# adelacvg/diff-vits

Hardware: AMD Instinct MI355X
Metric: mel_frames_per_sec_50step_dpmsolver (higher is better)
Workload: dtype bf16x3 (bf16 MFMA operands split hi+lo, 3 products, fp32 accumulate / fp32 activations); 1 GPU; B=8/GPU, C=80, T=1024, L=256, 50-step DPM-Solver++(2M) multistep, UNet1DConditionModel (128, 256, 384, 512), seeded random-init weights; global_batch=8, concurrent_sub_batches_per_gpu=1, rccl_world_size=1, parallelism=dp1 (batch-sharded, RCCL broadcast of conditioning + all-gather of mels)

## Files before the change

diff-vits_amd/csrc/engine.hip:

```cpp
#include "../../include/dvits_hip.h"
#include "dv_common.h"

#include <algorithm>
#include <atomic>
#include <cmath>
#include <cstdarg>
#include <cstdio>
#include <cstdlib>
#include <cstring>
#include <functional>
#include <map>
#include <memory>
#include <set>
#include <string>
#include <type_traits>
#include <vector>

static thread_local char g_err[1024] = "";
int dv_fail(int code, const char* fmt, ...) {
  va_list ap;
  va_start(ap, fmt);
  vsnprintf(g_err, sizeof(g_err), fmt, ap);
  va_end(ap);
  return code;
// ... 185 lines not shown
  u->slab = nullptr; u->slab_bytes = 0;
  u->step_ops.clear(); u->cond_ops.clear(); u->probes.clear(); u->step_meta.clear(); u->gemm_store.clear();
  u->pops.clear(); u->step_pop.clear(); u->pops_dev = nullptr; u->psync = nullptr; u->persist_on = false; u->p_begin = u->p_end = 0;
  u->prepared = false; u->cond_set = false; u->flops = 0;
  u->cond_segs.clear(); u->cond_segs_dev = nullptr; u->cond_chunks = 0; u->cond_sig = 0; u->row_cond.clear(); u->cond_gemms.clear();
}

extern "C" int dv_unet_create(const dv_unet_cfg* cfg, dv_unet** out) {
  if (!cfg || !out) return dv_fail(DV_ERR_INVALID, "dv_unet_create: null argument");
  if (cfg->n_levels < 2 || cfg->n_levels > 6) return dv_fail(DV_ERR_INVALID, "n_levels must be 2..6");
  for (int i = 0; i < cfg->n_levels; ++i)
    if (cfg->block_out_channels[i] % 32 != 0 || cfg->block_out_channels[i] <= 0)
      return dv_fail(DV_ERR_INVALID, "block_out_channels[%d]=%d must be a positive multiple of 32", i,
                     cfg->block_out_channels[i]);
  if (cfg->cross_attention_dim % 32 != 0) return dv_fail(DV_ERR_INVALID, "cross_attention_dim must be a multiple of 32");
  if (cfg->num_heads <= 0 || cfg->norm_num_groups <= 0 || cfg->norm_num_groups > 64)
    return dv_fail(DV_ERR_INVALID, "bad num_heads / norm_num_groups");
  for (int i = 0; i < cfg->n_levels; ++i) {
    int c = cfg->block_out_channels[i];
    if (c % cfg->num_heads != 0 || (c / cfg->num_heads) % 4 != 0 || c / cfg->num_heads > 64)
      return dv_fail(DV_ERR_INVALID, "head dim %d/%d must be a multiple of 4 and <= 64", c, cfg->num_heads);
    if (c % cfg->norm_num_groups != 0 || (c / cfg->norm_num_groups) % 4 != 0)
      return dv_fail(DV_ERR_INVALID, "channels per GroupNorm group must be a multiple of 4");
  }
  if (cfg->cross_attention_dim % cfg->add_embed_heads != 0 || cfg->cross_attention_dim / cfg->add_embed_heads > 8)
    return dv_fail(DV_ERR_INVALID, "add_embed_heads must divide cross_attention_dim with <= 8 dims per head");
  dv_unet* u = new dv_unet();
  u->cfg = *cfg;
  *out = u;
  return DV_OK;
}

extern "C" void dv_unet_destroy(dv_unet* u) {
  if (!u) return;
  (void)hipDeviceSynchronize();
  unet_release_prepared(u);
  if (u->gnx_status) (void)hipHostFree(u->gnx_status);
  for (auto& kv : u->w)
    if (kv.second.p) (void)hipFree(kv.second.p);
  delete u;
}

extern "C" int dv_unet_set_weight(dv_unet* u, const char* name, const void* dev_ptr, const int64_t* shape, int32_t ndim) {
  if (!u || !name || !dev_ptr || !shape || ndim < 1 || ndim > 4) return dv_fail(DV_ERR_INVALID, "dv_unet_set_weight: bad argument");
  size_t n = 1;
  std::vector<int64_t> sh(shape, shape + ndim);
  for (auto s : sh) n *= (size_t)s;
  RawW& r = u->w[name];
  if (r.numel != n) {
    if (r.p) (void)hipFree(r.p);
    r.p = nullptr;
    HIPCHK(hipMalloc((void**)&r.p, n * sizeof(float)));
  }
  r.shape = sh;
  r.numel = n;
  HIPCHK(hipMemcpy(r.p, dev_ptr, n * sizeof(float), hipMemcpyDeviceToDevice));
  u->weights_dirty = true;
  return DV_OK;
}

static bool autotune_on() {
  const char* e = getenv("DVITS_GEMM_AUTOTUNE");
  return e && (e[0] == '1' || e[0] == '2');
}

static int autotune_gemms(dv_unet* u, int precision) {
  u->tuned_gemms = u->tuned_changed = 0;
  if (!autotune_on() || u->gemm_store.empty()) return DV_OK;
  HIPCHK(hipDeviceSynchronize());
  hipStream_t st = nullptr;
  hipEvent_t e0, e1;
  HIPCHK(hipEventCreate(&e0)); HIPCHK(hipEventCreate(&e1));
  const size_t flush_bytes = 48u << 20;
  void* flush = nullptr;
  HIPCHK(hipMalloc(&flush, flush_bytes));
  auto time_one = [&](const GemmParams& t, float& best) -> bool {
    if (launch_gemm(t, precision, st) != hipSuccess) { (void)hipGetLastError(); return false; }
    best = 1e30f;
    for (int r = 0; r < 3; ++r) {
      if (hipMemsetAsync(flush, r, flush_bytes, st) != hipSuccess) return false;
      if (hipEventRecord(e0, st) != hipSuccess) return false;
      if (launch_gemm(t, precision, st) != hipSuccess) return false;
      if (hipEventRecord(e1, st) != hipSuccess || hipEventSynchronize(e1) != hipSuccess) return false;
      float ms = 0;
      if (hipEventElapsedTime(&ms, e0, e1) != hipSuccess) return false;
      best = ms < best ? ms : best;
    }
    return true;
  };
  for (auto& up : u->gemm_store) {
    GemmParams* gp = up.get();
    if (!gp->out && !gp->out_hi) continue;
    int cands[12];
    const int n = gemm_candidates(*gp, cands, 12);
    float best = 1e30f;
    int best_tile = gp->force_tile, best_split = gp->sk_split;
    const int heur_split = gp->sk_split;
    {
      float ms;
      if (time_one(*gp, ms)) best = ms * 0.97f;
    }
    for (int c = 0; c < n; ++c)
      for (int sp = 0; sp < (gp->sk_buf ? 2 : 1); ++sp) {
        GemmParams t = *gp;
        t.force_tile = cands[c];
        t.sk_split = sp ? (heur_split > 2 ? heur_split : 2) : 0;
        float ms;
        if (time_one(t, ms) && ms < best) { best = ms; best_tile = cands[c]; best_split = t.sk_split; }
      }
    if (best_tile != gp->force_tile || best_split != heur_split) u->tuned_changed++;
    gp->force_tile = best_tile;
    gp->sk_split = best_split;
    u->tuned_gemms++;
  }
  if (const char* e = getenv("DVITS_GEMM_AUTOTUNE"))
    if (e[0] == '2') fprintf(stderr, "[dvits] GEMM tuner: %d of %d GEMMs moved off the heuristic tile\n", u->tuned_changed, u->tuned_gemms);
  (void)hipFree(flush);
  (void)hipEventDestroy(e0); (void)hipEventDestroy(e1);
  HIPCHK(hipDeviceSynchronize());
  return DV_OK;
}

struct Builder {
  dv_unet* u;
  Arena arena;
  bool dry;
  int B, T, L, prec;
  std::string err;
  hipStream_t pack_stream = nullptr;
  bool fuse_ln = [] { const char* e = getenv("DVITS_FUSE_LN"); return !(e && e[0] == '0'); }();
  bool merge_ff = [] { const char* e = getenv("DVITS_MERGE_FF"); return !(e && e[0] == '0'); }();

  const RawW* raw(const std::string& name) {
    auto it = u->w.find(name);
    if (it == u->w.end()) { if (err.empty()) err = "missing weight: " + name; return nullptr; }
    return &it->second;
  }
  const float* W(const std::string& name) { const RawW* r = raw(name); return r ? r->p : nullptr; }
  bool has(const std::string& name) { return u->w.count(name) != 0; }

  float* alloc(size_t floats) {
    size_t off = arena.alloc(floats * sizeof(float));
    return dry ? reinterpret_cast<float*>(0x1000 + off) : reinterpret_cast<float*>(u->slab + off);
  }
  void release(const void* p) {
    if (u->keep_intermediates) return;
    size_t off = dry ? (reinterpret_cast<size_t>(p) - 0x1000) : (size_t)(reinterpret_cast<const char*>(p) - u->slab);
    arena.release(off);
  }
  const char* cur_kind = "misc";
  const GemmParams* cur_gp = nullptr;
  double cur_flops = 0;
  std::string cur_desc;
  void emit(std::vector<OpFn>& ops, OpFn f, const PersistOp* pop = nullptr) {
    if (dry) return;
    ops.push_back(std::move(f));
    if (&ops == &u->step_ops) {
      u->step_meta.push_back({cur_kind, cur_flops, cur_desc, cur_gp});
      if (pop) { u->step_pop.push_back((int)u->pops.size()); u->pops.push_back(*pop); }
      else u->step_pop.push_back(-1);
    }
    cur_kind = "misc"; cur_flops = 0; cur_desc.clear(); cur_gp = nullptr;
  }
  void emit_launch(std::vector<OpFn>& ops, const char* kind, double flops, std::string desc, OpFn f, const PersistOp* pop = nullptr) {
    cur_kind = kind; cur_flops = flops; cur_desc = std::move(desc);
    if (!dry) u->flops += flops;
    emit(ops, std::move(f), pop);
  }
  static std::string strf(const char* fmt, ...) {
    char buf[128];
    va_list ap;
    va_start(ap, fmt);
    vsnprintf(buf, sizeof(buf), fmt, ap);
    va_end(ap);
    return buf;
  }
  bool persist_gemm(const GemmParams& gin, PersistOp& po) {
    if (prec != DV_PREC_BF16X3 || gin.epi == EPI_STORE_NCT || !gin.w_lo) return false;
    bool k64 = true;
    for (int s2 = 0; s2 < gin.nseg; ++s2) k64 = k64 && gin.seg[s2].c0 % 64 == 0 && gin.seg[s2].c1 % 64 == 0;
    int cfg, bm, bk;
    if (gin.epi == EPI_GEGLU) { if (!k64) return false; cfg = 1; bm = 128; bk = 64; }
    else {
      const bool big = gin.T_out % 128 == 0 && (gin.T_out / 128) * ((gin.N + 127) / 128) >= 24;
      if (big || !k64) { cfg = 0; bm = 128; bk = 32; } else { cfg = 2; bm = 64; bk = 64; }
    }
    if (gin.T_out % bm != 0 || gin.M != B * gin.T_out) return false;
    if (gin.T_out < 1 || (unsigned long long)(gin.M > 0 ? gin.M : 1) * (unsigned long long)gin.T_out >= (1ull << 32)) return false;
    po = PersistOp{};
    po.type = POP_GEMM; po.cfg = cfg; po.g = gin;
    po.g.tout_magic = gemm_tout_magic(gin.T_out);
    if (po.g.Tv_out <= 0) po.g.Tv_out = po.g.T_out;
    if (po.g.Tv_in <= 0) po.g.Tv_in = po.g.T_in;
    for (int s2 = 0; s2 < gin.nseg; ++s2) po.g.seg[s2].nkt = gin.seg[s2].taps * (gin.seg[s2].c0 + gin.seg[s2].c1) / bk;
    return true;
  }
  void probe(const std::string& name, const float* p, int T_, int C_) {
    if (!dry && u->keep_intermediates) u->probes.push_back(Probe{name, const_cast<float*>(p), T_, C_, T_ > 1 ? pitch(T_) : T_});
  }
  void probe_rows(const std::string& name, const float* p, int T_, int C_) {
    if (!dry && u->keep_intermediates) u->probes.push_back(Probe{name, const_cast<float*>(p), T_, C_, T_});
  }

  struct Piece { std::string w; int kind, C, taps, c_pad, k_off, n_off; std::string kscale; int geglu; };
  struct BiasPiece { std::string bias, bias2, foldW, foldBeta; int N, C, n_off, geglu; };

  const PackedW* pack(const std::string& key, int N, int Kp, const std::vector<Piece>& pieces,
                      const std::vector<BiasPiece>& biases) {
    if (dry) { static PackedW dummy; return &dummy; }
    auto it = u->packed.find(key);
    if (it != u->packed.end()) return &it->second;
    PackedW pw;
    pw.N = N; pw.Kp = Kp; pw.N_pad = rup(N, 128);
    const size_t elems = (size_t)pw.N_pad * Kp;
    if (hipMalloc((void**)&pw.hi, elems * 2) != hipSuccess) { err = "hipMalloc(packed weights) failed"; return nullptr; }
    u->owned_w.push_back(pw.hi);
    (void)hipMemsetAsync(pw.hi, 0, elems * 2, pack_stream);
    if (prec == DV_PREC_BF16X3) {
      if (hipMalloc((void**)&pw.lo, elems * 2) != hipSuccess) { err = "hipMalloc(packed weights) failed"; return nullptr; }
      u->owned_w.push_back(pw.lo);
      (void)hipMemsetAsync(pw.lo, 0, elems * 2, pack_stream);
    }
    for (const Piece& pc : pieces) {
      const RawW* r = raw(pc.w);
      if (!r) return nullptr;
      PackSpec s{};
      s.src = r->p; s.N = (int)r->shape[0]; s.kind = pc.kind; s.C = pc.C; s.taps = pc.taps; s.c_pad = pc.c_pad;
      s.k_off = pc.k_off; s.n_off = pc.n_off; s.geglu = pc.geglu;
      s.kscale = pc.kscale.empty() ? nullptr : W(pc.kscale);
      if ((size_t)s.N * s.C * s.taps != r->numel) { err = "weight shape mismatch: " + pc.w; return nullptr; }
      if (launch_pack_weight(s, pw.hi, pw.lo, Kp, pack_stream) != hipSuccess) { err = "pack_weight launch failed"; return nullptr; }
      if (s.kscale) {
        if (!pw.u) {
          if (hipMalloc((void**)&pw.u, (size_t)pw.N_pad * 4) != hipSuccess) { err = "hipMalloc(u) failed"; return nullptr; }
          u->owned_w.push_back(pw.u);
          (void)hipMemsetAsync(pw.u, 0, (size_t)pw.N_pad * 4, pack_stream);
        }
        if (launch_fold_bias(r->p, nullptr, s.kscale, pw.u, s.N, s.C, pc.n_off, pc.geglu, pack_stream) != hipSuccess) {
          err = "fold(u) launch failed"; return nullptr;
        }
      }
    }
    if (!biases.empty()) {
      if (hipMalloc((void**)&pw.bias, (size_t)pw.N_pad * 4) != hipSuccess) { err = "hipMalloc(bias) failed"; return nullptr; }
      u->owned_w.push_back(pw.bias);
      (void)hipMemsetAsync(pw.bias, 0, (size_t)pw.N_pad * 4, pack_stream);
      for (const BiasPiece& bp : biases) {
        const float* b1 = bp.bias.empty() ? nullptr : W(bp.bias);
        const float* fw = bp.foldW.empty() ? nullptr : W(bp.foldW);
        const float* fb = bp.foldBeta.empty() ? nullptr : W(bp.foldBeta);
        if (launch_fold_bias(fw, b1, fb, pw.bias, bp.N, bp.C, bp.n_off, bp.geglu, pack_stream) != hipSuccess) {
          err = "fold_bias launch failed"; return nullptr;
        }
        if (!bp.bias2.empty()) {
          static const float one_one[8] = {1.f, 1.f, 0, 0, 0, 0, 0, 0};
          float* dcoef = nullptr;
          if (hipMalloc((void**)&dcoef, sizeof(one_one)) != hipSuccess) { err = "hipMalloc failed"; return nullptr; }
          u->owned_w.push_back(dcoef);
          (void)hipMemcpyAsync(dcoef, one_one, sizeof(one_one), hipMemcpyHostToDevice, pack_stream);
          (void)launch_lincomb(pw.bias + bp.n_off, pw.bias + bp.n_off, W(bp.bias2), nullptr, nullptr, nullptr, dcoef, bp.N,
                               pack_stream);
        }
      }
    }
    u->packed[key] = pw;
    return &u->packed[key];
  }

  struct Planes { bf16_t* hi = nullptr; bf16_t* lo = nullptr; };
  Planes alloc_planes(size_t elems) {
    Planes pl;
    pl.hi = reinterpret_cast<bf16_t*>(alloc((elems + 1) / 2));
    if (prec == DV_PREC_BF16X3) pl.lo = reinterpret_cast<bf16_t*>(alloc((elems + 1) / 2));
    return pl;
  }
  void release(const Planes& pl) { if (pl.hi) release((const void*)pl.hi); if (pl.lo) release((const void*)pl.lo); }
  void alloc_stat(Act& a, bool want16 = false) {
    if (a.Tp % 32 != 0) {
      if (B == 1) a.stat = alloc((size_t)((a.Tp + 31) / 32) * a.C * 2);
      return;
    }
    if (want16 || stat16_everywhere()) a.stat16 = alloc((size_t)(B * a.Tp / 32) * (a.C / 16) * 2);
    else a.stat = alloc((size_t)(B * a.Tp / 32) * a.C * 2);
  }
  bool pad_on = [] { const char* e = getenv("DVITS_PAD_T"); return !(e && e[0] == '0'); }();
  int pitch(int Tl) const { return (pad_on && Tl % 32 != 0 && stat16_everywhere()) ? rup(Tl, 32) : Tl; }
  bool stat16_everywhere() const {
    const char* e16 = getenv("DVITS_STAT16");
    if ((e16 && e16[0] == '0') || arena.exact) return false;
    const int G = u->cfg.norm_num_groups;
    for (int i = 0; i < u->cfg.n_levels; ++i)
      if (u->cfg.block_out_channels[i] % G != 0 || (u->cfg.block_out_channels[i] / G) % 16 != 0) return false;
    return true;
  }
  void stat_out(GemmParams& g, const Act& a) { g.stats = a.stat; g.stats16 = a.stat16; }
  bool chain_on = [] { const char* e = getenv("DVITS_CHAIN"); return !(e && e[0] == '0'); }();
  int chain_min_rows = [] { const char* e = getenv("DVITS_CHAIN_MIN_ROWS"); return e ? atoi(e) : 128; }();
  bool chain_ok(int Tn, int C) const {
    const int G = u->cfg.norm_num_groups;
    return chain_on && fuse_ln && !arena.exact && prec == DV_PREC_BF16X3 && (C == 128 || C == 256 || C == 384) && Tn % 32 == 0 &&
           B * Tn >= chain_min_rows &&
           G > 0 && G <= 64 && (G & (G - 1)) == 0 && C % G == 0 && (C / G) % 16 == 0 && (Tn / 32) * (C / 16) <= (C / 128) * 2048;
  }
  bool frag(const PackedW* cw) {
    if (dry) return true;
    PackedW* w = const_cast<PackedW*>(cw);
    if (w->fhi) return true;
    const size_t elems = (size_t)w->N_pad * w->Kp;
    if (!w->lo || hipMalloc((void**)&w->fhi, elems * 2) != hipSuccess || hipMalloc((void**)&w->flo, elems * 2) != hipSuccess) {
      err = "hipMalloc(fragment-major weights) failed"; return false;
    }
    u->owned_w.push_back(w->fhi); u->owned_w.push_back(w->flo);
    if (launch_relayout_frag(w->hi, w->fhi, w->N_pad, w->Kp, pack_stream) != hipSuccess ||
        launch_relayout_frag(w->lo, w->flo, w->N_pad, w->Kp, pack_stream) != hipSuccess) { err = "relayout launch failed"; return false; }
    return true;
  }
  static double chain_flops(const ChainParams& cp) { return 2.0 * (double)cp.M * cp.C * cp.C * (1 + cp.passes); }
  void chain(std::vector<OpFn>& ops, const ChainParams& cp, const char* what, double extra_flops = 0.0) {
    const int pr = prec;
    emit_launch(ops, "chain", chain_flops(cp) + extra_flops, strf("%s M=%d C=%d N2=%d", what, cp.M, cp.C, cp.passes * cp.C),
                [cp, pr](hipStream_t st) { return launch_chain2(cp, pr, st); });
  }
  bool sk_fused = [] { const char* e = getenv("DVITS_SPLITK_FUSED"); return !(e && e[0] == '0'); }();
  bool gnx_on = [] { const char* e = getenv("DVITS_GNX"); return !(e && e[0] == '0') && !getenv("HSA_CU_MASK") && !getenv("ROC_GLOBAL_CU_MASK"); }();
  size_t gnx_used = 0;
  int gnx_spin = [] { const char* e = getenv("DVITS_GNX_SPIN"); const int v = e ? atoi(e) : 0; return v != 0 ? v : (1 << 18); }();
  int n_cu = [] { int d = 0, n = 0; if (hipGetDevice(&d) != hipSuccess || hipDeviceGetAttribute(&n, hipDeviceAttributeMultiprocessorCount, d) != hipSuccess) n = 0;
                  const char* e = getenv("DVITS_CU_BUDGET"); const int b = e ? atoi(e) : 0; return b > 0 && b < n ? b : n; }();
  bool gnx_cat_on = [] { const char* e = getenv("DVITS_GNX_CONCAT"); return !(e && e[0] == '0'); }();
  bool handover_ok() const { return gnx_on && u->exclusive && !arena.exact && n_cu > 0; }
  struct Handover { unsigned long long* flags; unsigned* status; };
  Handover handover(size_t n) {
    Handover h{dry ? reinterpret_cast<unsigned long long*>(0x1000) : u->gnx_pool + gnx_used,
               dry ? reinterpret_cast<unsigned*>(0x1000) : u->gnx_status};
    gnx_used += (n + 1) & ~(size_t)1;
    if (!dry) { u->gnx_words = gnx_used; u->gnx_ops++; }
    return h;
  }
  bool gnx_setup(GemmParams& g, const std::string& pre, float eps, const float* tscale, const float* tshift, int ld_t, bool silu,
                 Planes* y, const Act* skip = nullptr, Planes* sk_y = nullptr, Planes* sk_raw = nullptr) {
    if (!handover_ok() || autotune_on() || !g.stats16) return false;
    if (skip && (!gnx_cat_on || !skip->p || !skip->stat16 || skip->Tp != g.T_out || tscale)) return false;
    GemmParams t = g;
    t.B = B;
    t.gnx = GnxParams{};
    t.gnx.groups = u->cfg.norm_num_groups;
    t.gnx.sk_c = skip ? skip->C : 0;
    int k_pad = 0;
    for (int s2 = 0; s2 < t.nseg; ++s2) k_pad += t.seg[s2].taps * (t.seg[s2].c0 + t.seg[s2].c1);
    t.c3_route = conv3_route(t);
    t.sk_split = t.c3_route ? gemm_conv3_split(t, n_cu) : gemm_splitk_plan(t.M, t.N, k_pad, t.epi);
    if (t.sk_split >= 2) {
      if (!sk_fused || ((t.M + 31) / 32) * ((t.N + 31) / 32) > 4096) return false;
      t.sk_buf = reinterpret_cast<float*>(0x1000); t.sk_ticket = reinterpret_cast<unsigned*>(0x1000);
    }
    const int nw = gemm_gnx_plan(t, n_cu);
    if (nw <= 0 || gnx_used + (size_t)nw > dv_unet::GNX_POOL) return false;
    g.gnx = t.gnx;
    gnx_fill(g.gnx, nw, g.M, g.N, pre, eps, tscale, tshift, ld_t, silu, y, skip, sk_y, sk_raw);
    return true;
  }
  void gnx_fill(GnxParams& gx, int nw, int M, int N, const std::string& pre, float eps, const float* tscale, const float* tshift, int ld_t,
                bool silu, Planes* y, const Act* skip, Planes* sk_y, Planes* sk_raw) {
    gx.gamma = W(pre + ".weight"); gx.beta = W(pre + ".bias"); gx.eps = eps;
    gx.tscale = tscale; gx.tshift = tshift; gx.ld_t = ld_t; gx.silu = silu ? 1 : 0;
    gx.spin_max = gnx_spin;
    const Handover h = handover((size_t)nw);
    gx.xchg = h.flags; gx.status = h.status;
    *y = alloc_planes((size_t)M * N);
    gx.y_hi = y->hi; gx.y_lo = y->lo;
    if (skip) {
      gx.sk_x = skip->p; gx.sk_stat16 = skip->stat16;
      *sk_y = alloc_planes((size_t)M * skip->C);
      gx.sk_y_hi = sk_y->hi; gx.sk_y_lo = sk_y->lo;
      if (sk_raw) { *sk_raw = alloc_planes((size_t)M * skip->C); gx.sk_raw_hi = sk_raw->hi; gx.sk_raw_lo = sk_raw->lo; }
    }
  }

  struct NextNorm { std::string pre; bool raw = false; bool set = false; Act skip; float eps = 0.f; bool silu = true; } next_norm;
  void announce_norm(const std::string& pre, bool raw_planes, const Act& skip = Act{}) {
    next_norm.pre = pre; next_norm.raw = raw_planes; next_norm.skip = skip; next_norm.set = true;
    next_norm.eps = u->cfg.norm_eps; next_norm.silu = true;
  }
  void announce_transformer_norm(const std::string& tp, int Tp, int C) {
    if (chain_ok(Tp, C)) return;
    announce_norm(tp + "norm", false);
    next_norm.eps = 1e-6f; next_norm.silu = false;
  }
  bool gnx_offer(GemmParams& g, const NextNorm& nn, Planes* y, Planes* sy, Planes* sr) {
    return gnx_setup(g, nn.pre, nn.eps, nullptr, nullptr, 0, nn.silu, y, nn.skip.C > 0 ? &nn.skip : nullptr, sy, nn.raw ? sr : nullptr);
  }
  static int ff_gnx_plan(const ChainFFParams& fp, int n_cu) { return chain_ff_gnx_plan(fp, n_cu); }
  static int ff_gnx_plan(const FFSplitParams& fp, int n_cu) { return ff_split_gnx_plan(fp, n_cu); }
  template <class FF> bool gnx_offer(FF& fp, const NextNorm& nn, Planes* y, Planes* sy, Planes* sr) {
    const bool cat = nn.skip.C > 0;
    if (!handover_ok() || !gnx_ff_on || !fp.stats16) return false;
    if (cat && (!gnx_cat_on || !nn.skip.p || !nn.skip.stat16 || nn.skip.Tp != fp.T)) return false;
    fp.gnx = GnxParams{};
    fp.gnx.groups = u->cfg.norm_num_groups;
    fp.gnx.sk_c = cat ? nn.skip.C : 0;
    const int nw = ff_gnx_plan(fp, n_cu);
    if (nw <= 0 || gnx_used + (size_t)nw > dv_unet::GNX_POOL) { fp.gnx = GnxParams{}; return false; }
    gnx_fill(fp.gnx, nw, fp.M, fp.C, nn.pre, nn.eps, nullptr, nullptr, 0, nn.silu, y, cat ? &nn.skip : nullptr, sy, nn.raw ? sr : nullptr);
    return true;
  }
  template <class P> void offer_next(P& prod, Act& out) {
    if (!next_norm.set) return;
    const NextNorm nn = next_norm;
    next_norm.set = false;
    Planes y, sy, sr;
    if (!gnx_offer(prod, nn, &y, &sy, &sr)) return;
    const bool cat = nn.skip.C > 0;
    out.n_hi = y.hi; out.n_lo = y.lo; out.n_pre = nn.pre;
    if (cat) { out.sn_hi = sy.hi; out.sn_lo = sy.lo; out.sr_hi = sr.hi; out.sr_lo = sr.lo; }
    const bool fp32_unread = cat && nn.raw && !u->keep_intermediates;
    if (nn.raw && !prod.out_hi) out_planes(prod, out);
    if (fp32_unread && cat_drop_fp32) prod.out = nullptr;
  }
  template <class P> void out_planes(P& prod, Act& out) {
    Planes pl = alloc_planes((size_t)prod.M * out.C);
    out.pl_hi = pl.hi; out.pl_lo = pl.lo; prod.out_hi = pl.hi; prod.out_lo = pl.lo;
  }
  bool ff_split_on = [] { const char* e = getenv("DVITS_FF_SPLIT"); return !(e && e[0] == '0'); }();
  bool chain_ff_on = [] { const char* e = getenv("DVITS_CHAIN_FF"); return !(e && e[0] == '0'); }();
  bool chain_split_on = [] { const char* e = getenv("DVITS_CHAIN_SPLIT"); return !(e && e[0] == '0'); }();
  bool chain_xsplit_on = [] { const char* e = getenv("DVITS_CHAIN_XSPLIT"); return !(e && e[0] == '0'); }();
  bool qkv_split_on = [] { const char* e = getenv("DVITS_QKV_SPLIT"); return !(e && e[0] == '0'); }();
  int qkv_split_min_wg = [] { const char* e = getenv("DVITS_QKV_SPLIT_MIN_WG"); return e ? atoi(e) : 96; }();
  int qkv_split_min_c = [] { const char* e = getenv("DVITS_QKV_SPLIT_MIN_C"); return e ? atoi(e) : 256; }();
  bool qkv_xa_on = [] { const char* e = getenv("DVITS_QKV_XA"); return !(e && e[0] == '0'); }();
  int qkv_xa_min_c = [] { const char* e = getenv("DVITS_QKV_XA_MIN_C"); return e ? atoi(e) : 256; }();
  int ff_split_min_wg = [] { const char* e = getenv("DVITS_FF_SPLIT_MIN_WG"); return e ? atoi(e) : 96; }();
  bool gnx_ff_on = [] { const char* e = getenv("DVITS_GNX_FF"); return !(e && e[0] == '0'); }();
  bool cat_drop_fp32 = [] { const char* e = getenv("DVITS_GNX_CONCAT_KEEP_FP32"); return !(e && e[0] == '1'); }();

  int conv3_min_tiles = [] { const char* e = getenv("DVITS_CONV3_MIN_TILES"); return e ? atoi(e) : 64; }();
  int conv3_route(const GemmParams& g) const {
    if (arena.exact || autotune_on() || prec != DV_PREC_BF16X3) return 0;
    GemmParams t = g;
    t.B = B;
    if (gemm_conv3_up_ok(t)) {
      const int tu = gemm_conv3_row_tiles(t, 128) * (t.N / 64);
      return tu >= (conv3_min_tiles < 64 ? conv3_min_tiles : 96) ? 2 : 0;
    }
    if (!gemm_conv3_shape_ok(t)) return 0;
    return gemm_conv3_row_tiles(t, 64) * (t.N / 64) >= conv3_min_tiles ? 1 : 0;
  }
  bool conv3_takes(const GemmParams& g) const { return conv3_route(g) != 0; }
  void gemm(std::vector<OpFn>& ops, GemmParams g, const PackedW* pw, int k_real) {
    g.w_hi = pw->hi; g.w_lo = pw->lo; g.Kp = pw->Kp; g.N_pad = pw->N_pad;
    if (!g.bias) g.bias = pw->bias;
    g.B = B;
    g.zero_page = u->zero_page;
    const int p = prec;
    const int route = conv3_route(g);
    const bool c3 = route != 0 && (dry || g.Kp == gemm_conv3_k(g)) && frag(pw);
    g.c3_route = c3 ? route : 0;
    if (c3) { g.wf_hi = dry ? reinterpret_cast<const bf16_t*>(0x1000) : pw->fhi; g.wf_lo = dry ? reinterpret_cast<const bf16_t*>(0x1000) : pw->flo; }
    cur_kind = "gemm"; cur_flops = 2.0 * (double)g.M * (double)g.N * (double)k_real;
    {
      char buf[128];
      snprintf(buf, sizeof(buf), "M=%d N=%d K=%d taps=%d nseg=%d epi=%d stride=%d up=%d%s%s%s", g.M, g.N, k_real, g.seg[0].taps,
               g.nseg, g.epi, g.stride, g.up_mode, (g.stats || g.stats16) ? " +stats" : "", c3 ? " resident" : "",
               g.gnx.xchg ? " +gnx" : "");
      cur_desc = buf;
    }
    u->flops += dry ? 0.0 : cur_flops;
    int k_pad = 0;
    for (int s2 = 0; s2 < g.nseg; ++s2) k_pad += g.seg[s2].taps * (g.seg[s2].c0 + g.seg[s2].c1);
    g.sk_split = arena.exact ? 0 : (c3 ? gemm_conv3_split(g, n_cu) : gemm_splitk_plan(g.M, g.N, k_pad, g.epi));
    const bool offer = !arena.exact && autotune_on() && gemm_splitk_plan(64, 64, 1 << 20, EPI_STORE) != 0 && k_pad >= 768 && (g.epi == EPI_STORE || g.epi == EPI_RESIDUAL) &&
                       ((g.M + 63) / 64) * ((g.N + 63) / 64) <= 256;
    if (g.sk_split >= 2 || offer) {
      g.sk_buf = alloc((c3 && g.sk_split == 2 ? gemm_conv3_split_bytes(g) : gemm_splitk_bytes(g.M, g.N, g.sk_split > 2 ? g.sk_split : 2)) / sizeof(float));
      g.sk_ticket = (sk_fused && ((g.M + 31) / 32) * ((g.N + 31) / 32) <= 4096) ? u->sk_tickets : nullptr;
    }
    PersistOp po;
    const bool pok = !dry && persist_gemm(g, po);
    if (dry) emit(ops, OpFn{}, nullptr);
    else {
      u->gemm_store.emplace_back(new GemmParams(g));
      const GemmParams* gp = u->gemm_store.back().get();
      cur_gp = gp;
      if (&ops == &u->cond_ops) u->cond_gemms.push_back(gp);
      dv_unet* uu = u;
      emit(ops, [gp, p, uu](hipStream_t st) {
        if (!uu->io.tp_base || !gp->gnx.xchg || !gp->gnx.tscale) return launch_gemm(*gp, p, st);
        GemmParams g2 = *gp;
        g2.gnx.tscale = uu->io.tp_base + (gp->gnx.tscale - uu->temb.tproj_arena);
        g2.gnx.tshift = uu->io.tp_base + (gp->gnx.tshift - uu->temb.tproj_arena);
        return launch_gemm(g2, p, st);
      }, pok ? &po : nullptr);
    }
    if (g.sk_buf) release((const void*)g.sk_buf);
  }

  static GemmSeg seg(Planes a0, int c0, Planes a1, int c1, int taps, int pad) {
    GemmSeg s{};
    s.a0_hi = a0.hi; s.a0_lo = a0.lo; s.a1_hi = a1.hi; s.a1_lo = a1.lo;
    s.c0 = c0; s.c1 = c1; s.taps = taps; s.pad = pad;
    return s;
  }

  Planes norm_apply(std::vector<OpFn>& ops, Act a0, Act a1, const std::string& pre, float eps, const float* tscale,
                    const float* tshift, int ld_t, bool silu, Planes* raw_out) {
    const int G = u->cfg.norm_num_groups, C = a0.C + a1.C, Tn = a0.T, Tp = a0.Tp;
    GnApplyParams gp{};
    gp.a0 = a0.p; gp.a1 = a1.p; gp.c0 = a0.C; gp.c1 = a1.C;
    gp.gamma = W(pre + ".weight"); gp.beta = W(pre + ".bias"); gp.eps = eps; gp.groups = G;
    gp.tscale = tscale; gp.tshift = tshift; gp.ld_t = ld_t; gp.silu = silu ? 1 : 0;
    gp.B = B; gp.T = Tp; gp.Tv = Tn;
    float* sc = nullptr; float* sh = nullptr;
    const bool fast16 = a0.stat16 && (a1.C == 0 || a1.stat16) && ((a0.C + a1.C) / G) % 16 == 0 && a0.C % 16 == 0;
    const bool fast = fast16 || (a0.stat && (a1.C == 0 || a1.stat));
    if (fast16) { gp.st16_0 = a0.stat16; gp.st16_1 = a1.stat16; }
    else if (fast) { gp.slab0 = a0.stat; gp.slab1 = a1.stat; }
    else {
      const int nchunk = std::max(1, std::min(64, (Tn + 63) / 64));
      double* part = reinterpret_cast<double*>(alloc((size_t)B * nchunk * G * 2 * 2));
      sc = alloc((size_t)B * C); sh = alloc((size_t)B * C);
      const int Bn = B;
      const float* gamma = gp.gamma; const float* beta = gp.beta;
      cur_kind = "gn_partial";
      emit(ops, [=](hipStream_t st) { return launch_gn_partial(a0.p, a0.C, a1.p, a1.C, part, Bn, Tn, G, nchunk, st); });
      cur_kind = "gn_finalize";
      dv_unet* uu = u;
      emit(ops, [=](hipStream_t st) {
        const float* ts = tscale; const float* tb = tshift;
        if (uu->io.tp_base && ts) {
          ts = uu->io.tp_base + (tscale - uu->temb.tproj_arena);
          tb = uu->io.tp_base + (tshift - uu->temb.tproj_arena);
        }
        return launch_gn_finalize(part, nchunk, gamma, beta, ts, tb, ld_t, sc, sh, nullptr, nullptr, Bn, Tn, C, G, eps, st);
      });
      release(part);
      gp.scale_in = sc; gp.shift_in = sh;
    }
    Planes out = alloc_planes((size_t)B * Tp * C);
    gp.out_hi = out.hi; gp.out_lo = out.lo;
    if (raw_out) { *raw_out = alloc_planes((size_t)B * Tp * C); gp.raw_hi = raw_out->hi; gp.raw_lo = raw_out->lo; }
    cur_kind = "gn_apply";
    {
      char buf[96];
      snprintf(buf, sizeof(buf), "T=%d C=%d%s%s", Tn, C, fast16 ? " blockstats" : (fast ? " slab" : " table"), raw_out ? " +raw" : "");
      cur_desc = buf;
    }
    PersistOp po{};
    if (fast) {
      po.type = POP_GN; po.gn = gp;
      po.gn_chunks = std::max(1, std::min(Tp / 4, 64 / G));
      po.gn_rpb = (Tp + po.gn_chunks - 1) / po.gn_chunks;
      po.gn_chunks = (Tp + po.gn_rpb - 1) / po.gn_rpb;
    }
    {
      dv_unet* uu = u;
      emit(ops, [gp, uu](hipStream_t st) {
        if (!uu->io.tp_base || !gp.tscale) return launch_gn_apply(gp, st);
        GnApplyParams g2 = gp;
        g2.tscale = uu->io.tp_base + (gp.tscale - uu->temb.tproj_arena);
        g2.tshift = uu->io.tp_base + (gp.tshift - uu->temb.tproj_arena);
        return launch_gn_apply(g2, st);
      }, (fast && !fast16) ? &po : nullptr);
    }
    if (sc) { release(sc); release(sh); }
    return out;
  }

  Planes ln_apply(std::vector<OpFn>& ops, const float* x, int M, int C) {
    Planes out = alloc_planes((size_t)M * C);
    cur_kind = "ln_apply";
    emit(ops, [=](hipStream_t st) { return launch_ln_apply(x, out.hi, out.lo, M, C, 1e-5f, st); });
    return out;
  }

  Planes split(std::vector<OpFn>& ops, const float* x, size_t n) {
    Planes out = alloc_planes(n);
    cur_kind = "split";
    PersistOp po{};
    po.type = POP_SPLIT; po.sp_in = x; po.sp_hi = out.hi; po.sp_lo = out.lo; po.n4_per_item = (int64_t)(n / 4 / (size_t)B);
    emit(ops, [=](hipStream_t st) { return launch_split(x, out.hi, out.lo, (int64_t)n, st); }, (n % (4 * (size_t)B) == 0) ? &po : nullptr);
    return out;
  }

  GemmParams gp_base(int Tn, int M, int N) {
    GemmParams g{};
    g.nseg = 1; g.T_out = g.T_in = pitch(Tn); g.Tv_out = g.Tv_in = g.T_virt = Tn; g.stride = 1; g.up_mode = UP_NONE;
    g.M = M; g.N = N; g.epi = EPI_STORE; g.ldo = N; g.ldres = N;
    return g;
  }
  GemmParams gp_rows(int rows, int M, int N) {
    GemmParams g = gp_base(rows, M, N);
    g.T_out = g.T_in = rows;
    return g;
  }

  std::map<std::string, int> tproj_off;
  int tproj_total = 0;
  float* tproj = nullptr;

  Act resnet(std::vector<OpFn>& ops, const std::string& p, Act x0, Act x1, int cout, bool want_planes = false,
             bool stat16_out = false) {
    const int cin = x0.C + x1.C, Tn = x0.T, Tp = x0.Tp, M = B * Tp;
    const float eps = u->cfg.norm_eps;
    const bool shortcut = has(p + "conv_shortcut.weight");
    const PackedW* w1 = pack(p + "conv1", cout, 3 * cin, {{p + "conv1.weight", 1, cin, 3, cin, 0, 0, "", 0}},
                             {{p + "conv1.bias", "", "", "", cout, 0, 0, 0}});
    if (!w1) return Act{};
    Act h{};
    h.p = alloc((size_t)M * cout); h.C = cout; h.T = Tn; h.Tp = Tp; alloc_stat(h);
    Planes raw, raw1;
    bool raw_made = false;
    const int toff = tproj_off[p];
    Planes n2x;
    bool gnx1 = false;
    {
      GemmParams g = gp_base(Tn, M, cout);
      g.out = h.p; stat_out(g, h);
      {
        Planes n1, n1b;
        if (x0.n_hi && x0.n_pre == p + "norm1" && (!shortcut || x0.pl_hi) && (x1.C == 0 || (x0.sn_hi && (!shortcut || x0.sr_hi)))) {
          n1.hi = x0.n_hi; n1.lo = x0.n_lo;
          if (shortcut) { raw.hi = x0.pl_hi; raw.lo = x0.pl_lo; }
          if (x1.C) {
            n1b.hi = x0.sn_hi; n1b.lo = x0.sn_lo;
            if (shortcut) { raw1.hi = x0.sr_hi; raw1.lo = x0.sr_lo; }
          }
          g.seg[0] = x1.C ? seg(n1, x0.C, n1b, x1.C, 3, 1) : seg(n1, cin, Planes{}, 0, 3, 1);
        } else {
          if (x0.n_hi) { Planes stale; stale.hi = x0.n_hi; stale.lo = x0.n_lo; release(stale); }
          if (x0.sn_hi) { Planes stale; stale.hi = x0.sn_hi; stale.lo = x0.sn_lo; release(stale); }
          if (x0.sr_hi) { Planes stale; stale.hi = x0.sr_hi; stale.lo = x0.sr_lo; release(stale); }
          n1 = norm_apply(ops, x0, x1, p + "norm1", eps, nullptr, nullptr, 0, true, shortcut ? &raw : nullptr);
          g.seg[0] = seg(n1, cin, Planes{}, 0, 3, 1);
        }
        raw_made = shortcut;
        gnx1 = gnx_setup(g, p + "norm2", eps, tproj + toff, tproj + toff + cout, tproj_total, true, &n2x);
        if (gnx1 && !u->keep_intermediates) g.out = nullptr;
        gemm(ops, g, w1, 3 * cin);
        release(n1);
        if (n1b.hi) release(n1b);
      }
    }
    probe(p + "conv1", h.p, Tn, cout);

    const int K2 = 3 * cout + (shortcut ? cin : 0);
    std::vector<Piece> pcs = {{p + "conv2.weight", 1, cout, 3, cout, 0, 0, "", 0}};
    std::vector<BiasPiece> bps = {{p + "conv2.bias", shortcut ? p + "conv_shortcut.bias" : "", "", "", cout, 0, 0, 0}};
    if (shortcut) pcs.push_back({p + "conv_shortcut.weight", 1, cin, 1, cin, 3 * cout, 0, "", 0});
    const PackedW* w2 = pack(p + "conv2", cout, K2, pcs, bps);
    if (!w2) return Act{};
    Act out{};
    out.p = alloc((size_t)M * cout); out.C = cout; out.T = Tn; out.Tp = Tp; alloc_stat(out, stat16_out);
    {
      GemmParams g = gp_base(Tn, M, cout);
      if (!shortcut) { g.epi = EPI_RESIDUAL; g.res = x0.p; g.ldres = cout; }
      g.out = out.p; stat_out(g, out);
      if (want_planes) out_planes(g, out);
      const bool offered = next_norm.set;
      {
        Planes n2 = gnx1 ? n2x : norm_apply(ops, h, Act{}, p + "norm2", eps, tproj + toff, tproj + toff + cout, tproj_total, true, nullptr);
        g.seg[0] = seg(n2, cout, Planes{}, 0, 3, 1);
        g.nseg = 1;
        if (shortcut) { g.seg[1] = raw1.hi ? seg(raw, x0.C, raw1, x1.C, 1, 0) : seg(raw, cin, Planes{}, 0, 1, 0); g.nseg = 2; }
        if (offered) offer_next(g, out);
        gemm(ops, g, w2, K2);
        release(n2);
      }
    }
    release_act(h);
    if (raw_made) release(raw);
    if (raw1.hi) release(raw1);
    probe(p.substr(0, p.size() - 1), out.p, Tn, cout);
    return out;
  }

  std::map<std::string, float*> cross_kv;
  std::set<std::string> kv_read;
  float* mask_bias = nullptr;
  struct XFrag { bf16_t* kf_hi = nullptr; bf16_t* kf_lo = nullptr; bf16_t* vf_hi = nullptr; bf16_t* vf_lo = nullptr; };
  std::map<std::string, XFrag> cross_frag;
  float* xbias = nullptr;
  bool xa_on = [] { const char* e = getenv("DVITS_CHAIN_XATTN"); return !(e && e[0] == '0'); }();
  bool xa_ok(int Tn, int C) const {
    const int H = u->cfg.num_heads;
    return xa_on && chain_ok(Tn, C) && H == 8 && C % H == 0 && (C / H == 16 || C / H == 32);
  }

  Planes attention(std::vector<OpFn>& ops, const float* q, int ldq, const float* k, const float* v, int ldkv, const float* bias,
                   int Tq, int Tk, int C, int Tk_pitch = 0) {
    Planes o = alloc_planes((size_t)B * Tq * C);
    AttnParams a{};
    a.Tk_pitch = Tk_pitch;
    a.q = q; a.k = k; a.v = v; a.bias = bias; a.o = nullptr; a.o_hi = o.hi; a.o_lo = o.lo;
    a.ldq = ldq; a.ldk = ldkv; a.ldv = ldkv; a.ldo = C;
    a.B = B; a.H = u->cfg.num_heads; a.Tq = Tq; a.Tk = Tk; a.d = C / u->cfg.num_heads;
    a.scale = 1.0f / sqrtf((float)a.d);
    a.nsplit = prec == DV_PREC_BF16X3 ? 3 : 1;
    PersistOp po{};
    po.type = POP_ATTN; po.cfg = (a.d + 15) / 16 * 16; po.a = a;
    emit_launch(ops, "attn", 4.0 * B * a.H * (double)Tq * Tk * a.d, strf("Tq=%d Tk=%d d=%d H=%d", Tq, Tk, a.d, a.H),
                [a](hipStream_t st) { return launch_attention(a, st); }, (prec == DV_PREC_BF16X3 && a.d % 4 == 0 && a.d <= 64) ? &po : nullptr);
    return o;
  }

  Planes attention_frag(std::vector<OpFn>& ops, AttnFragParams a, int Tq, int Tk, int C) {
    Planes o = alloc_planes((size_t)B * Tq * C);
    a.o = nullptr; a.o_hi = o.hi; a.o_lo = o.lo; a.ldo = C;
    a.B = B; a.H = u->cfg.num_heads; a.Tq = Tq; a.Tk = Tk; a.d = C / u->cfg.num_heads;
    a.scale = 1.0f / sqrtf((float)a.d);
    a.nsplit = prec == DV_PREC_BF16X3 ? 3 : 1;
    emit_launch(ops, "attn", 4.0 * B * a.H * (double)Tq * Tk * a.d, strf("Tq=%d Tk=%d d=%d H=%d frag", Tq, Tk, a.d, a.H),
                [a](hipStream_t st) { return launch_attention_frag(a, st); });
    return o;
  }
  bool attn_frag_on = [] { const char* e = getenv("DVITS_ATTN_FRAG"); return !(e && e[0] == '0'); }();
  Planes cross_attention_frag(std::vector<OpFn>& ops, const std::string& p, const float* q2, int Tn, int C) {
    const XFrag& xf = cross_frag[p];
    const int H = u->cfg.num_heads, dh = C / H, nT = (L + 31) / 32, KSq = dh / 16, NBv = (dh + 31) / 32;
    AttnFragParams a{};
    a.q = q2; a.ldq = C;
    a.kf_hi = xf.kf_hi; a.kf_lo = xf.kf_lo; a.vf_hi = xf.vf_hi; a.vf_lo = xf.vf_lo;
    a.k_b = H * nT * KSq; a.k_h = nT * KSq; a.k_t = KSq;
    a.v_b = H * nT * 2 * NBv; a.v_h = nT * 2 * NBv; a.v_t = 2 * NBv; a.v_kb = NBv; a.v_nb = 1; a.self_layout = 0;
    a.bias = xbias; a.bias_ld = nT * 32;
    return attention_frag(ops, a, Tn, L, C);
  }

  struct LnIn { Planes pl; float* stat = nullptr; };
  LnIn ln_planes(int M, int C) {
    LnIn in;
    in.pl = alloc_planes((size_t)M * C);
    in.stat = alloc((size_t)M * (C / 32) * 2);
    return in;
  }
  LnIn ln_produce(GemmParams& g, int M, int C) {
    if (!fuse_ln) return LnIn{};
    LnIn in = ln_planes(M, C);
    g.out_hi = in.pl.hi; g.out_lo = in.pl.lo; g.rowstat_out = in.stat;
    return in;
  }
  void ln_consume(std::vector<OpFn>& ops, GemmParams& g, LnIn& in, const float* x32, const PackedW* w, int M, int C) {
    if (!fuse_ln) in.pl = ln_apply(ops, x32, M, C);
    else { g.ln_stat = in.stat; g.ln_nblk = C / 32; g.ln_u = w->u; g.ln_eps = 1e-5f; }
    g.seg[0] = seg(in.pl, C, Planes{}, 0, 1, 0);
  }
  void ln_release(LnIn& in) { release(in.pl); if (in.stat) release(in.stat); }

  bool qkv_split(std::vector<OpFn>& ops, ChainParams cp, std::string desc, double extra_flops = 0.0) {
    if (!qkv_split_supported(cp, prec)) return false;
    const Handover h = handover((size_t)qkv_split_flags(cp));
    cp.nsplit = 1; cp.qs_flags = h.flags; cp.qs_status = h.status; cp.qs_spin = gnx_spin;
    const int pr = prec;
    emit_launch(ops, "chain", chain_flops(cp) + extra_flops, std::move(desc), [cp, pr](hipStream_t st) { return launch_qkv_split(cp, pr, st); });
    return true;
  }

  struct Xf {
    std::string p, tb;
    Act x;
    int C, Tn, Tp, M;
    const PackedW *w_in, *w_qkv, *w_o1, *w_q2, *w_o2, *w_gg, *w_ff, *w_out;
    bool merged_ffproj;
  };

  Act transformer(std::vector<OpFn>& ops, const std::string& p, Act x, bool want_planes = false) {
    const int C = x.C;
    const std::string tb = p + "transformer_blocks.0.";
    Xf b{p, tb, x, C, x.T, x.Tp, B * x.Tp};
    b.w_in = pack(p + "proj_in", C, C, {{p + "proj_in.weight", 1, C, 1, C, 0, 0, "", 0}},
                  {{p + "proj_in.bias", "", "", "", C, 0, 0, 0}});
    b.w_qkv = pack(tb + "qkv1", 3 * C, C,
                   {{tb + "attn1.to_q.weight", 0, C, 1, C, 0, 0, tb + "norm1.weight", 0},
                    {tb + "attn1.to_k.weight", 0, C, 1, C, 0, C, tb + "norm1.weight", 0},
                    {tb + "attn1.to_v.weight", 0, C, 1, C, 0, 2 * C, tb + "norm1.weight", 0}},
                   {{"", "", tb + "attn1.to_q.weight", tb + "norm1.bias", C, C, 0, 0},
                    {"", "", tb + "attn1.to_k.weight", tb + "norm1.bias", C, C, C, 0},
                    {"", "", tb + "attn1.to_v.weight", tb + "norm1.bias", C, C, 2 * C, 0}});
    b.w_o1 = pack(tb + "out1", C, C, {{tb + "attn1.to_out.0.weight", 0, C, 1, C, 0, 0, "", 0}},
                  {{tb + "attn1.to_out.0.bias", "", "", "", C, 0, 0, 0}});
    b.w_q2 = pack(tb + "q2", C, C, {{tb + "attn2.to_q.weight", 0, C, 1, C, 0, 0, tb + "norm2.weight", 0}},
                  {{"", "", tb + "attn2.to_q.weight", tb + "norm2.bias", C, C, 0, 0}});
    b.w_o2 = pack(tb + "out2", C, C, {{tb + "attn2.to_out.0.weight", 0, C, 1, C, 0, 0, "", 0}},
                  {{tb + "attn2.to_out.0.bias", "", "", "", C, 0, 0, 0}});
    b.w_gg = pack(tb + "geglu", 8 * C, C, {{tb + "ff.net.0.proj.weight", 0, C, 1, C, 0, 0, tb + "norm3.weight", 1}},
                  {{tb + "ff.net.0.proj.bias", "", tb + "ff.net.0.proj.weight", tb + "norm3.bias", 8 * C, C, 0, 1}});
    b.merged_ffproj = merge_ff && fuse_ln && !u->keep_intermediates;
    b.w_ff = b.merged_ffproj ? b.w_gg : pack(tb + "ffout", C, 4 * C, {{tb + "ff.net.2.weight", 0, 4 * C, 1, 4 * C, 0, 0, "", 0}},
                                             {{tb + "ff.net.2.bias", "", "", "", C, 0, 0, 0}});
    b.w_out = b.merged_ffproj ? b.w_gg : pack(p + "proj_out", C, C, {{p + "proj_out.weight", 1, C, 1, C, 0, 0, "", 0}},
                                              {{p + "proj_out.bias", "", "", "", C, 0, 0, 0}});
    if (!b.w_in || !b.w_qkv || !b.w_o1 || !b.w_q2 || !b.w_o2 || !b.w_gg || !b.w_ff || !b.w_out) return Act{};

    float* h3 = nullptr;
    LnIn l3;
    if (chain_ok(b.Tp, C) && x.stat16) {
      if (!(frag(b.w_in) && frag(b.w_qkv) && frag(b.w_o1) && frag(b.w_q2))) return Act{};
      float* h = nullptr;
      const Planes ao = xf_head(ops, b, h);
      if (!xf_tail(ops, b, h, ao, h3, l3)) return Act{};
    } else h3 = xf_attention_gemms(ops, b, l3);
    return xf_ff(ops, b, h3, l3, want_planes);
  }

  Planes xf_head(std::vector<OpFn>& ops, const Xf& b, float*& h) {
    const int C = b.C, Tn = b.Tn, Tp = b.Tp, M = b.M;
    h = alloc((size_t)M * C);
    const int dh = C / u->cfg.num_heads;
    const bool sa_frag = attn_frag_on && !arena.exact && C % u->cfg.num_heads == 0 && dh % 16 == 0 && dh <= 64;
    float* qkv = alloc((size_t)M * (sa_frag ? 1 : 3) * C);
    Planes kf, vf;
    if (sa_frag) { kf = alloc_planes((size_t)M * C); vf = alloc_planes((size_t)M * C); }
    ChainParams cp{};
    cp.M = M; cp.C = C; cp.T = Tp; cp.Tv = Tn; cp.amode = 1;
    cp.x = b.x.p; cp.stat16 = b.x.stat16; cp.gamma = W(b.p + "norm.weight"); cp.beta = W(b.p + "norm.bias"); cp.gn_eps = 1e-6f;
    cp.groups = u->cfg.norm_num_groups;
    cp.w1_hi = b.w_in->fhi; cp.w1_lo = b.w_in->flo; cp.Kp1 = b.w_in->Kp; cp.b1 = b.w_in->bias; cp.res = nullptr; cp.out1 = h;
    cp.w2_hi = b.w_qkv->fhi; cp.w2_lo = b.w_qkv->flo; cp.Kp2 = b.w_qkv->Kp; cp.b2 = b.w_qkv->bias; cp.u2 = b.w_qkv->u;
    cp.passes = 3; cp.out2 = qkv; cp.ldo2 = sa_frag ? C : 3 * C; cp.ln_eps = 1e-5f;
    if (sa_frag) { cp.sa_kf_hi = kf.hi; cp.sa_kf_lo = kf.lo; cp.sa_vf_hi = vf.hi; cp.sa_vf_lo = vf.lo; }
    {
      const int rbs = M / 32, cus = n_cu > 0 ? n_cu : 256;
      cp.nsplit = !chain_split_on ? 1 : (rbs * 3 <= cus ? 3 : (rbs * 2 <= cus ? 2 : 1));
    }
    const int n_qflags = qkv_split_flags(cp);
    const bool split = qkv_split_on && C >= qkv_split_min_c && sa_frag && handover_ok() && !autotune_on() &&
                       n_qflags <= n_cu && n_qflags >= qkv_split_min_wg && gnx_used + (size_t)n_qflags <= dv_unet::GNX_POOL &&
                       qkv_split(ops, cp, strf("norm+proj_in+LN+q|Kfrag|Vfrag (%d wg / 64 rows) M=%d C=%d N2=%d", C / 64, M, C, 3 * C));
    if (!split) chain(ops, cp, sa_frag ? "norm+proj_in+LN+q|Kfrag|Vfrag" : "norm+proj_in+LN+qkv");
    probe(b.p + "proj_in", h, Tn, C);
    Planes ao;
    if (sa_frag) {
      AttnFragParams a{};
      a.q = qkv; a.ldq = C;
      a.kf_hi = kf.hi; a.kf_lo = kf.lo; a.vf_hi = vf.hi; a.vf_lo = vf.lo;
      const int nT = Tp / 32;
      a.k_b = nT * (C / 16); a.k_h = dh / 16; a.k_t = C / 16;
      a.v_b = nT * (C / 32) * 2; a.v_h = 0; a.v_t = (C / 32) * 2; a.v_kb = 1; a.v_nb = 2; a.self_layout = 1;
      a.bias = nullptr; a.bias_ld = 0;
      ao = attention_frag(ops, a, Tp, Tn, C);
      release(kf); release(vf);
    } else ao = attention(ops, qkv, 3 * C, qkv + C, qkv + 2 * C, 3 * C, nullptr, Tp, Tn, C, Tp);
    release(qkv);
    return ao;
  }

  bool xf_tail(std::vector<OpFn>& ops, const Xf& b, float* h, Planes ao, float*& h3, LnIn& l3) {
    const int C = b.C, M = b.M;
    if (xa_ok(b.Tp, C) && cross_frag.count(b.p)) {
      if (!frag(b.w_o2)) return false;
      float* h2 = alloc((size_t)M * C);
      h3 = alloc((size_t)M * C);
      l3 = ln_planes(M, C);
      xf_xattn_chain(ops, b, h, ao, h2, h3, l3);
      release(ao); release(h);
      probe(b.tb + "attn1", h2, b.Tn, C);
      release(h2);
      probe(b.tb + "attn2", h3, b.Tn, C);
      return true;
    }
    float* h2 = alloc((size_t)M * C);
    float* q2 = alloc((size_t)M * C);
    ChainParams cp = tail_chain(b, h, ao, h2);
    cp.out2 = q2;
    {
      const int rbs = M / 32, cus = n_cu > 0 ? n_cu : 256, nsg = C / 128;
      cp.nsplit = (chain_split_on && nsg >= 2 && rbs * nsg <= cus) ? nsg : 1;
    }
    const int n_qflags = qkv_split_flags(cp);
    const bool split = qkv_split_on && C >= qkv_split_min_c && handover_ok() && !autotune_on() &&
                       n_qflags <= n_cu && n_qflags >= qkv_split_min_wg && gnx_used + (size_t)n_qflags <= dv_unet::GNX_POOL &&
                       qkv_split(ops, cp, strf("to_out+res+LN+to_q (%d wg / 64 rows) M=%d C=%d N2=%d", C / 64, M, C, C));
    if (!split) chain(ops, cp, "to_out+res+LN+to_q");
    release(ao); release(h);
    probe(b.tb + "attn1", h2, b.Tn, C);
    h3 = cross_attention_out(ops, b, q2, h2, l3);
    return true;
  }
  ChainParams tail_chain(const Xf& b, float* h, Planes ao, float* h2) {
    ChainParams cp{};
    cp.M = b.M; cp.C = b.C; cp.T = b.Tp; cp.Tv = b.Tn; cp.amode = 0;
    cp.a_hi = ao.hi; cp.a_lo = ao.lo;
    cp.w1_hi = b.w_o1->fhi; cp.w1_lo = b.w_o1->flo; cp.Kp1 = b.w_o1->Kp; cp.b1 = b.w_o1->bias; cp.res = h; cp.out1 = h2;
    cp.w2_hi = b.w_q2->fhi; cp.w2_lo = b.w_q2->flo; cp.Kp2 = b.w_q2->Kp; cp.b2 = b.w_q2->bias; cp.u2 = b.w_q2->u;
    cp.passes = 1; cp.out2 = nullptr; cp.ldo2 = b.C; cp.ln_eps = 1e-5f;
    return cp;
  }
  void xf_xattn_chain(std::vector<OpFn>& ops, const Xf& b, float* h, Planes ao, float* h2, float* h3, const LnIn& l3) {
    const int C = b.C, Tp = b.Tp, M = b.M;
    const XFrag& xf = cross_frag[b.p];
    ChainParams cp = tail_chain(b, h, ao, h2);
    cp.xa_kf_hi = xf.kf_hi; cp.xa_kf_lo = xf.kf_lo; cp.xa_vf_hi = xf.vf_hi; cp.xa_vf_lo = xf.vf_lo; cp.xa_bias = xbias;
    cp.xa_nT = (L + 31) / 32; cp.xa_d = C / u->cfg.num_heads;
    cp.xa_qscale = (1.0f / sqrtf((float)cp.xa_d)) * 1.44269504088896340736f;
    cp.w3_hi = b.w_o2->fhi; cp.w3_lo = b.w_o2->flo; cp.b3 = b.w_o2->bias;
    cp.out3 = h3; cp.out3_hi = l3.pl.hi; cp.out3_lo = l3.pl.lo; cp.rowstat3 = l3.stat;
    {
      const int rbs = M / 32, cus = n_cu > 0 ? n_cu : 256;
      if (chain_xsplit_on && C == 256 && rbs * 2 <= cus && rbs <= 4096 && (dry || u->sk_tickets)) {
        cp.nsplit = 2;
        cp.xs_buf = alloc((size_t)rbs * 2 * C * 32);
        cp.xs_ticket = dry ? reinterpret_cast<unsigned*>(0x1000) : u->sk_tickets;
      }
    }
    ChainParams cq = cp;
    cq.nsplit = 1; cq.xs_buf = nullptr; cq.xs_ticket = nullptr;
    const double xattn_flops = 4.0 * B * u->cfg.num_heads * (double)Tp * L * cp.xa_d + 2.0 * (double)M * C * C;
    const int n_wg = (M / 64) * (C / 64);
    bool split_xa = qkv_split_on && qkv_xa_on && C >= qkv_xa_min_c && handover_ok() && !autotune_on() &&
                    Tp % 64 == 0 && (M / 64) % 8 == 0 && n_wg <= n_cu && n_wg >= qkv_split_min_wg && u->cfg.num_heads == 8 &&
                    gnx_used + (size_t)2 * n_wg <= dv_unet::GNX_POOL;
    Planes oxa;
    if (split_xa) {
      oxa = alloc_planes((size_t)M * C);
      cq.qs_o_hi = oxa.hi; cq.qs_o_lo = oxa.lo;
      split_xa = qkv_split(ops, cq, strf("to_out+res+LN+to_q+xattn+to_out+res (%d wg / 64 rows) M=%d C=%d", C / 64, M, C), xattn_flops);
      if (!split_xa) release(oxa);
    }
    if (!split_xa)
      chain(ops, cp, cp.nsplit == 2 ? "to_out+res+LN+to_q+xattn(2 wg)+to_out+res" : "to_out+res+LN+to_q+xattn+to_out+res", xattn_flops);
    if (cp.xs_buf) release(cp.xs_buf);
    if (split_xa) release(oxa);
  }

  float* xf_attention_gemms(std::vector<OpFn>& ops, const Xf& b, LnIn& l3) {
    const int C = b.C, Tn = b.Tn, Tp = b.Tp, M = b.M;
    float* h = alloc((size_t)M * C);
    LnIn l1;
    {
      GemmParams g = gp_base(Tn, M, C);
      g.out = h; l1 = ln_produce(g, M, C);
      Planes gn;
      if (b.x.n_hi && b.x.n_pre == b.p + "norm") { gn.hi = b.x.n_hi; gn.lo = b.x.n_lo; }
      else gn = norm_apply(ops, b.x, Act{}, b.p + "norm", 1e-6f, nullptr, nullptr, 0, false, nullptr);
      g.seg[0] = seg(gn, C, Planes{}, 0, 1, 0);
      gemm(ops, g, b.w_in, C);
      release(gn);
    }
    probe(b.p + "proj_in", h, Tn, C);

    float* qkv = alloc((size_t)M * 3 * C);
    {
      GemmParams g = gp_base(Tn, M, 3 * C);
      g.out = qkv; ln_consume(ops, g, l1, h, b.w_qkv, M, C); gemm(ops, g, b.w_qkv, C);
    }
    ln_release(l1);
    Planes ao = attention(ops, qkv, 3 * C, qkv + C, qkv + 2 * C, 3 * C, nullptr, Tp, Tn, C, Tp);
    release(qkv);
    float* h2 = alloc((size_t)M * C);
    LnIn l2;
    {
      GemmParams g = gp_base(Tn, M, C); g.seg[0] = seg(ao, C, Planes{}, 0, 1, 0);
      g.epi = EPI_RESIDUAL; g.res = h; g.out = h2; l2 = ln_produce(g, M, C);
      gemm(ops, g, b.w_o1, C);
    }
    release(ao); release(h);
    probe(b.tb + "attn1", h2, Tn, C);

    float* q2 = alloc((size_t)M * C);
    {
      GemmParams g = gp_base(Tn, M, C);
      g.out = q2; ln_consume(ops, g, l2, h2, b.w_q2, M, C); gemm(ops, g, b.w_q2, C);
    }
    ln_release(l2);
    return cross_attention_out(ops, b, q2, h2, l3);
  }
  float* cross_attention_out(std::vector<OpFn>& ops, const Xf& b, float* q2, float* h2, LnIn& l3) {
    const int C = b.C, Tp = b.Tp, M = b.M;
    float* kv = cross_kv[b.p];
    Planes ao;
    if (attn_frag_on && !arena.exact && cross_frag.count(b.p)) ao = cross_attention_frag(ops, b.p, q2, Tp, C);
    else { ao = attention(ops, q2, C, kv, kv + C, 2 * C, mask_bias, Tp, L, C); kv_read.insert(b.p); }
    release(q2);
    float* h3 = alloc((size_t)M * C);
    {
      GemmParams g = gp_base(b.Tn, M, C); g.seg[0] = seg(ao, C, Planes{}, 0, 1, 0);
      g.epi = EPI_RESIDUAL; g.res = h2; g.out = h3; l3 = ln_produce(g, M, C);
      gemm(ops, g, b.w_o2, C);
    }
    release(ao); release(h2);
    probe(b.tb + "attn2", h3, b.Tn, C);
    return h3;
  }

  Act xf_ff(std::vector<OpFn>& ops, const Xf& b, float* h3, LnIn& l3, bool want_planes) {
    const int C = b.C, Tp = b.Tp, M = b.M;
    const bool one_launch = b.merged_ffproj && chain_on && !arena.exact && l3.stat && b.x.stat16;
    ChainFFParams cf{};
    cf.M = M; cf.C = C; cf.T = Tp; cf.Tv = b.Tn;
    FFSplitParams fs{};
    fs.M = M; fs.C = C; fs.T = Tp; fs.Tv = b.Tn; fs.nspl = C == 256 ? 4 : 8;
    fs.rows = ff_split_rows(C, M, Tp, fs.nspl, n_cu);
    const int ff_wg = (M / fs.rows) * fs.nspl;
    const size_t n_flags = (size_t)ff_wg * 8;
    if (one_launch && chain_ff_on && chain_ff_supported(cf, prec)) return ff_launch(ops, b, cf, h3, l3, want_planes);
    else if (one_launch && ff_split_on && handover_ok() && !autotune_on() && (C == 256 || C == 384 || C == 512) &&
             ff_split_supported(fs, prec) && (ff_wg <= n_cu || gemm_handover_rounds()) && ff_wg >= ff_split_min_wg &&
             gnx_used + n_flags <= dv_unet::GNX_POOL)
      return ff_launch(ops, b, fs, h3, l3, want_planes);
    else return xf_ff_gemms(ops, b, h3, l3, want_planes);
  }
  const PackedW* ffproj_weight(const Xf& b) {
    const int C = b.C;
    const std::string &p = b.p, &tb = b.tb;
    const std::string mw = tb + "__ffproj.weight", mb = tb + "__ffproj.bias";
    if (!dry && !u->packed.count(p + "ffproj")) {
      const float* Wo = W(p + "proj_out.weight"); const float* W2 = W(tb + "ff.net.2.weight");
      const float* bo = W(p + "proj_out.bias"); const float* b2 = W(tb + "ff.net.2.bias");
      float* dw = derived(mw, {C, 4 * C});
      float* db = derived(mb, {C});
      if (!Wo || !W2 || !bo || !b2 || !dw || !db) return nullptr;
      (void)launch_matmul_f32(Wo, W2, dw, C, C, 4 * C, pack_stream);
      (void)launch_fold_bias(Wo, bo, b2, db, C, C, 0, 0, pack_stream);
    }
    return pack(p + "ffproj", C, 5 * C, {{p + "proj_out.weight", 1, C, 1, C, 0, 0, "", 0}, {mw, 0, 4 * C, 1, 4 * C, C, 0, "", 0}},
                {{mb, "", "", "", C, 0, 0, 0}});
  }
  template <class FF> Act ff_launch(std::vector<OpFn>& ops, const Xf& b, FF fp, float* h3, LnIn& l3, bool want_planes) {
    constexpr bool split = std::is_same<FF, FFSplitParams>::value;
    const int C = b.C, M = b.M;
    const PackedW* w_m = ffproj_weight(b);
    if (!w_m || !frag(b.w_gg) || !frag(w_m)) return Act{};
    Act out{};
    out.p = alloc((size_t)M * C); out.C = C; out.T = b.Tn; out.Tp = b.Tp; alloc_stat(out, true);
    fp.a_hi = l3.pl.hi; fp.a_lo = l3.pl.lo; fp.rowstat = l3.stat; fp.ln_eps = 1e-5f;
    fp.wg_hi = b.w_gg->fhi; fp.wg_lo = b.w_gg->flo; fp.bg = b.w_gg->bias; fp.ug = b.w_gg->u;
    fp.wm_hi = w_m->fhi; fp.wm_lo = w_m->flo; fp.bm = w_m->bias;
    fp.res = b.x.p; fp.out = out.p; fp.stats16 = out.stat16;
    if constexpr (split) {
      const Handover ho = handover((size_t)(M / fp.rows) * fp.nspl * 8);
      fp.flags = ho.flags; fp.status = ho.status; fp.spin_max = gnx_spin;
      fp.xbuf = alloc(ff_split_xbuf_floats(M, C, fp.nspl, fp.rows));
    }
    if (want_planes) out_planes(fp, out);
    offer_next(fp, out);
    const double flops = 2.0 * (double)M * C * (8.0 * C + 5.0 * C);
    const char* gnx = fp.gnx.xchg ? "+gnx" : "";
    const int pr = prec;
    if constexpr (split) {
      emit_launch(ops, "chain", flops, strf("LN+GEGLU+ffproj+res%s (%d wg / %d rows) M=%d C=%d", gnx, fp.nspl, fp.rows, M, C),
                  [fp, pr](hipStream_t st) { return launch_ff_split(fp, pr, st); });
      release(fp.xbuf);
    } else {
      emit_launch(ops, "chain", flops, strf("LN+GEGLU+ffproj+res%s M=%d C=%d", gnx, M, C),
                  [fp, pr](hipStream_t st) { return launch_chain_ff(fp, pr, st); });
    }
    ln_release(l3);
    release(h3);
    probe(b.p.substr(0, b.p.size() - 1), out.p, b.Tn, C);
    return out;
  }
  Act xf_ff_gemms(std::vector<OpFn>& ops, const Xf& b, float* h3, LnIn& l3, bool want_planes) {
    const int C = b.C, Tn = b.Tn, Tp = b.Tp, M = b.M;
    Planes gg = alloc_planes((size_t)M * 4 * C);
    {
      GemmParams g = gp_base(Tn, M, 8 * C);
      g.epi = EPI_GEGLU; g.out_hi = gg.hi; g.out_lo = gg.lo; g.ldo = 4 * C; ln_consume(ops, g, l3, h3, b.w_gg, M, C); gemm(ops, g, b.w_gg, C);
    }
    if (b.merged_ffproj) {
      const PackedW* w_m = ffproj_weight(b);
      if (!w_m) return Act{};
      Act out{};
      out.p = alloc((size_t)M * C); out.C = C; out.T = Tn; out.Tp = Tp; alloc_stat(out);
      {
        GemmParams g = gp_base(Tn, M, C);
        g.seg[0] = seg(l3.pl, C, Planes{}, 0, 1, 0);
        g.seg[1] = seg(gg, 4 * C, Planes{}, 0, 1, 0); g.nseg = 2;
        g.epi = EPI_RESIDUAL; g.res = b.x.p; g.out = out.p; stat_out(g, out);
        if (want_planes) out_planes(g, out);
        offer_next(g, out);
        gemm(ops, g, w_m, 5 * C);
      }
      ln_release(l3);
      release(gg); release(h3);
      probe(b.p.substr(0, b.p.size() - 1), out.p, Tn, C);
      return out;
    }
    ln_release(l3);
    Planes h4 = alloc_planes((size_t)M * C);
    float* h4f = u->keep_intermediates ? alloc((size_t)M * C) : nullptr;
    {
      GemmParams g = gp_base(Tn, M, C); g.seg[0] = seg(gg, 4 * C, Planes{}, 0, 1, 0);
      g.epi = EPI_RESIDUAL; g.res = h3; g.out = h4f; g.out_hi = h4.hi; g.out_lo = h4.lo; gemm(ops, g, b.w_ff, 4 * C);
    }
    release(gg); release(h3);
    if (h4f) probe(b.tb + "ff", h4f, Tn, C);

    Act out{};
    out.p = alloc((size_t)M * C); out.C = C; out.T = Tn; out.Tp = Tp; alloc_stat(out);
    {
      GemmParams g = gp_base(Tn, M, C); g.seg[0] = seg(h4, C, Planes{}, 0, 1, 0);
      g.epi = EPI_RESIDUAL; g.res = b.x.p; g.out = out.p; stat_out(g, out);
      if (want_planes) out_planes(g, out);
      offer_next(g, out);
      gemm(ops, g, b.w_out, C);
    }
    release(h4);
    probe(b.p.substr(0, b.p.size() - 1), out.p, Tn, C);
    return out;
  }

  Act resample(std::vector<OpFn>& ops, const std::string& p, Act x, bool down, int T_target) {
    const int C = x.C;
    const PackedW* w = pack(p + "conv", C, 3 * C, {{p + "conv.weight", 1, C, 3, C, 0, 0, "", 0}},
                            {{p + "conv.bias", "", "", "", C, 0, 0, 0}});
    if (!w) return Act{};
    Planes xs;
    if (x.pl_hi) { xs.hi = x.pl_hi; xs.lo = x.pl_lo; }
    else xs = split(ops, x.p, (size_t)B * x.Tp * C);
    GemmParams g = gp_base(x.T, 0, C);
    g.seg[0] = seg(xs, C, Planes{}, 0, 3, 1);
    g.T_in = x.Tp; g.Tv_in = x.T;
    int T_new;
    if (down) { g.T_virt = x.T; g.stride = 2; g.up_mode = UP_NONE; T_new = (x.T + 2 - 3) / 2 + 1; }
    else {
      g.stride = 1; T_new = g.T_virt = T_target;
      if (u->force_up && T_target != 2 * x.T) { g.up_mode = UP_SIZE; g.up_scale = (float)x.T / (float)T_target; }
      else g.up_mode = UP_X2;
    }
    g.Tv_out = T_new; g.T_out = pitch(T_new);
    Act out{};
    out.p = alloc((size_t)B * g.T_out * C); out.C = C; out.T = T_new; out.Tp = g.T_out; alloc_stat(out);
    g.M = B * g.T_out; g.out = out.p; stat_out(g, out);
    offer_next(g, out);
    gemm(ops, g, w, 3 * C);
    release(xs);
    probe(p.substr(0, p.size() - 1), out.p, T_new, C);
    return out;
  }

  void release_act(const Act& a) { if (a.p) release(a.p); if (a.stat) release(a.stat); if (a.stat16) release(a.stat16); }

  int build() {
    const dv_unet_cfg& c = u->cfg;
    const int n = c.n_levels, lpb = c.layers_per_block, E = c.block_out_channels[0] * 4, D = c.cross_attention_dim;
    const int C0 = c.block_out_channels[0];
    std::vector<OpFn>& S = u->step_ops;
    std::vector<OpFn>& K = u->cond_ops;
    dv_unet* uu = u;
    const int Bn = B, Ln = L, Tn = T;

    std::vector<std::pair<std::string, int>> resnets;
    for (int i = 0; i < n; ++i)
      for (int j = 0; j < lpb; ++j) resnets.push_back({"down_blocks." + std::to_string(i) + ".resnets." + std::to_string(j) + ".", c.block_out_channels[i]});
    resnets.push_back({"mid_block.resnets.0.", c.block_out_channels[n - 1]});
    resnets.push_back({"mid_block.resnets.1.", c.block_out_channels[n - 1]});
    for (int i = 0; i < n; ++i)
      for (int j = 0; j < lpb + 1; ++j) resnets.push_back({"up_blocks." + std::to_string(i) + ".resnets." + std::to_string(j) + ".", c.block_out_channels[n - 1 - i]});
    tproj_total = 0;
    for (auto& r : resnets) { tproj_off[r.first] = tproj_total; tproj_total += 2 * r.second; }

    float* Wt = nullptr; float* bt = nullptr;
    if (!dry) {
      if (hipMalloc((void**)&Wt, (size_t)tproj_total * E * 4) != hipSuccess || hipMalloc((void**)&bt, (size_t)tproj_total * 4) != hipSuccess)
        return dv_fail(DV_ERR_HIP, "hipMalloc(time_emb_proj table) failed");
      u->owned.push_back(Wt); u->owned.push_back(bt);
      for (auto& r : resnets) {
        const RawW* w = raw(r.first + "time_emb_proj.weight");
        const RawW* b = raw(r.first + "time_emb_proj.bias");
        if (!w || !b) break;
        if (w->numel != (size_t)2 * r.second * E) { err = "shape mismatch: " + r.first + "time_emb_proj.weight"; break; }
        (void)hipMemcpyAsync(Wt + (size_t)tproj_off[r.first] * E, w->p, w->numel * 4, hipMemcpyDeviceToDevice, pack_stream);
        (void)hipMemcpyAsync(bt + tproj_off[r.first], b->p, b->numel * 4, hipMemcpyDeviceToDevice, pack_stream);
      }
      if (!u->zero_page) {
        void* z = nullptr;
        if (hipMalloc(&z, DV_ZERO_PAGE_BYTES) != hipSuccess) return dv_fail(DV_ERR_HIP, "hipMalloc(zero page) failed");
        (void)hipMemsetAsync(z, 0, DV_ZERO_PAGE_BYTES, pack_stream);
        u->owned.push_back(z);
        u->zero_page = reinterpret_cast<bf16_t*>(z);
      }
      if (!u->gnx_pool) {
        void* z = nullptr;
        if (hipMalloc(&z, dv_unet::GNX_POOL * 8) != hipSuccess) return dv_fail(DV_ERR_HIP, "hipMalloc(GroupNorm exchange words) failed");
        (void)hipMemsetAsync(z, 0xff, dv_unet::GNX_POOL * 8, pack_stream);
        u->owned.push_back(z);
        u->gnx_pool = reinterpret_cast<unsigned long long*>(z);
      }
      if (!u->gnx_status) {
        if (hipHostMalloc((void**)&u->gnx_status, 64, hipHostMallocMapped) != hipSuccess) return dv_fail(DV_ERR_HIP, "hipHostMalloc(status word) failed");
        *u->gnx_status = 0;
      }
      if (!u->sk_tickets) {
        void* z = nullptr;
        if (hipMalloc(&z, 4096 * sizeof(unsigned)) != hipSuccess) return dv_fail(DV_ERR_HIP, "hipMalloc(split-K tickets) failed");
        (void)hipMemsetAsync(z, 0, 4096 * sizeof(unsigned), pack_stream);
        u->owned.push_back(z);
        u->sk_tickets = reinterpret_cast<unsigned*>(z);
      }
    }

    float* aug_emb = alloc((size_t)B * E);
    mask_bias = alloc((size_t)B * L);
    std::vector<std::pair<std::string, int>> xformers;
    for (int i = 0; i < n - 1; ++i)
      for (int j = 0; j < lpb; ++j) xformers.push_back({"down_blocks." + std::to_string(i) + ".attentions." + std::to_string(j) + ".", c.block_out_channels[i]});
    xformers.push_back({"mid_block.attentions.0.", c.block_out_channels[n - 1]});
    for (int i = 1; i < n; ++i)
      for (int j = 0; j < lpb + 1; ++j) xformers.push_back({"up_blocks." + std::to_string(i) + ".attentions." + std::to_string(j) + ".", c.block_out_channels[n - 1 - i]});
    for (auto& x : xformers) cross_kv[x.first] = alloc((size_t)B * L * 2 * x.second);
    {
      const int H = c.num_heads, nT = (L + 31) / 32;
      xbias = alloc((size_t)B * nT * 32);
      int lvl_T = T;
      std::map<int, int> T_of_C;
      for (int i = 0; i < n; ++i) { T_of_C[c.block_out_channels[i]] = pitch(lvl_T); lvl_T = (lvl_T + 2 - 3) / 2 + 1; }
      for (auto& x : xformers) {
        const int C = x.second;
        const bool frag_attn = attn_frag_on && !arena.exact && prec == DV_PREC_BF16X3 && C % H == 0 && (C / H) % 16 == 0 && C / H <= 64;
        if (!xa_ok(T_of_C[C], C) && !frag_attn) continue;
        const int d = C / H, KSq = d / 16, NBv = (d + 31) / 32;
        const size_t kel = (size_t)B * H * nT * KSq * 64 * 8, vel = (size_t)B * H * nT * 2 * NBv * 64 * 8;
        XFrag xf;
        xf.kf_hi = reinterpret_cast<bf16_t*>(alloc((kel + 1) / 2)); xf.kf_lo = reinterpret_cast<bf16_t*>(alloc((kel + 1) / 2));
        xf.vf_hi = reinterpret_cast<bf16_t*>(alloc((vel + 1) / 2)); xf.vf_lo = reinterpret_cast<bf16_t*>(alloc((vel + 1) / 2));
        cross_frag[x.first] = xf;
      }
    }

    {
      float* mb = mask_bias;
      emit(K, [=](hipStream_t st) {
        return uu->io.mask ? launch_copy_f32(uu->io.mask, mb, (int64_t)Bn * Ln, st) : launch_fill_f32(mb, 0.f, (int64_t)Bn * Ln, st);
      });
      const std::string a = "add_embedding.";
      float* seq = alloc((size_t)B * (L + 1) * D);
      const float* n1w = W(a + "norm1.weight"); const float* n1b = W(a + "norm1.bias");
      emit(K, [=](hipStream_t st) { return launch_layernorm_rows_into(uu->io.enc, n1w, n1b, seq, Bn * Ln, D, 1e-5f, Ln, Ln + 1, 1, st); });
      const float* pos = W(a + "pool.positional_embedding");
      emit(K, [=](hipStream_t st) { return launch_mean_token(seq, pos, Bn, Ln, D, st); });
      const PackedW* wkv = pack(a + "pool.kv", 2 * D, D,
                                {{a + "pool.k_proj.weight", 0, D, 1, D, 0, 0, "", 0}, {a + "pool.v_proj.weight", 0, D, 1, D, 0, D, "", 0}},
                                {{a + "pool.k_proj.bias", "", "", "", D, 0, 0, 0}, {a + "pool.v_proj.bias", "", "", "", D, 0, D, 0}});
      if (!wkv) return dv_fail(DV_ERR_MISSING_WEIGHT, "%s", err.c_str());
      Planes seqs = split(K, seq, (size_t)B * (L + 1) * D);
      float* kvp = alloc((size_t)B * (L + 1) * 2 * D);
      {
        GemmParams g = gp_rows(L + 1, B * (L + 1), 2 * D);
        g.seg[0] = seg(seqs, D, Planes{}, 0, 1, 0);
        g.out = kvp;
        gemm(K, g, wkv, D);
      }
      float* qp = alloc((size_t)B * D);
      const float* wq = W(a + "pool.q_proj.weight"); const float* bq = W(a + "pool.q_proj.bias");
      emit(K, [=](hipStream_t st) { return launch_small_linear(seq, (Ln + 1) * D, wq, bq, nullptr, qp, D, Bn, D, D, 0, 0, st); });
      float* pooled = alloc((size_t)B * D);
      const int heads = c.add_embed_heads;
      emit(K, [=](hipStream_t st) { return launch_pool_attn(qp, kvp, pooled, Bn, Ln + 1, D, heads, st); });
      float* pe = alloc((size_t)B * E);
      const float* wp = W(a + "proj.weight"); const float* bp = W(a + "proj.bias");
      emit(K, [=](hipStream_t st) { return launch_small_linear(pooled, D, wp, bp, nullptr, pe, E, Bn, D, E, 0, 0, st); });
      const float* n2w = W(a + "norm2.weight"); const float* n2b = W(a + "norm2.bias");
      emit(K, [=](hipStream_t st) { return launch_layernorm_rows(pe, n2w, n2b, aug_emb, Bn, E, 1e-5f, st); });
      release(seq); release(seqs); release(kvp); release(qp); release(pooled); release(pe);
      Planes encs = alloc_planes((size_t)B * L * D);
      emit(K, [=](hipStream_t st) { return launch_split(uu->io.enc, encs.hi, encs.lo, (int64_t)Bn * Ln * D, st); });
      for (auto& x : xformers) {
        const std::string tb = x.first + "transformer_blocks.0.";
        const int C = x.second;
        const PackedW* w = pack(tb + "kv2", 2 * C, D,
                                {{tb + "attn2.to_k.weight", 0, D, 1, D, 0, 0, "", 0}, {tb + "attn2.to_v.weight", 0, D, 1, D, 0, C, "", 0}}, {});
        if (!w) return dv_fail(DV_ERR_MISSING_WEIGHT, "%s", err.c_str());
        GemmParams g = gp_rows(L, B * L, 2 * C);
        g.seg[0] = seg(encs, D, Planes{}, 0, 1, 0);
        g.out = cross_kv[x.first];
        gemm(K, g, w, D);
        if (cross_frag.count(x.first)) {
          const XFrag xf = cross_frag[x.first];
          const float* kvp2 = cross_kv[x.first];
          const int H = c.num_heads;
          emit(K, [=](hipStream_t st) { return launch_kv_frag(kvp2, xf.kf_hi, xf.kf_lo, xf.vf_hi, xf.vf_lo, Bn, Ln, C, H, st); });
        }
      }
      {
        float* xb = xbias; const float* mbp = mask_bias; const int nT = (L + 31) / 32;
        emit(K, [=](hipStream_t st) { return launch_xbias(mbp, xb, Bn, Ln, nT, st); });
      }
      release(encs);
    }

    u->flops = 0;
    tproj = alloc((size_t)B * tproj_total);
    float* emb = alloc((size_t)B * E);
    {
      float* tsin = alloc((size_t)B * C0);
      float* h1 = alloc((size_t)B * E);
      const int temb_begin = (int)S.size();
      emit(S, [=](hipStream_t st) { return launch_timestep_sincos(uu->io.t, tsin, Bn, C0, st); });
      const float* w1 = W("time_embedding.linear_1.weight"); const float* b1 = W("time_embedding.linear_1.bias");
      const float* w2 = W("time_embedding.linear_2.weight"); const float* b2 = W("time_embedding.linear_2.bias");
      if (Bn <= 16) {
        float* w1T = nullptr; float* w2T = nullptr;
        if (!dry) {
          if (hipMalloc((void**)&w1T, (size_t)E * C0 * 4) != hipSuccess || hipMalloc((void**)&w2T, (size_t)E * E * 4) != hipSuccess)
            return dv_fail(DV_ERR_HIP, "hipMalloc(time_embedding^T) failed");
          u->owned.push_back(w1T); u->owned.push_back(w2T);
          (void)launch_transpose_f32(w1, w1T, E, C0, pack_stream);
          (void)launch_transpose_f32(w2, w2T, E, E, pack_stream);
        }
        emit(S, [=](hipStream_t st) { return launch_small_linear_t(tsin, C0, w1T, b1, nullptr, h1, E, Bn, C0, E, 0, 1, st); });
        emit(S, [=](hipStream_t st) { return launch_small_linear_t(h1, E, w2T, b2, aug_emb, emb, E, Bn, E, E, 0, 0, st); });
        if (!dry) { u->temb.w1T = w1T; u->temb.w2T = w2T; u->temb.b1 = b1; u->temb.b2 = b2; u->temb.aug_emb = aug_emb; }
      } else {
        emit(S, [=](hipStream_t st) { return launch_small_linear(tsin, C0, w1, b1, nullptr, h1, E, Bn, C0, E, 0, 1, st); });
        emit(S, [=](hipStream_t st) { return launch_small_linear(h1, E, w2, b2, aug_emb, emb, E, Bn, E, E, 0, 0, st); });
      }
      float* tp = tproj; const int tt = tproj_total;
      if (Bn <= 16) {
        float* WtT = nullptr;
        if (!dry) {
          if (hipMalloc((void**)&WtT, (size_t)tt * E * 4) != hipSuccess) return dv_fail(DV_ERR_HIP, "hipMalloc(time_emb_proj^T) failed");
          u->owned.push_back(WtT);
          (void)launch_transpose_f32(Wt, WtT, tt, E, pack_stream);
        }
        emit(S, [=](hipStream_t st) { return launch_small_linear_t(emb, E, WtT, bt, nullptr, tp, tt, Bn, E, tt, 1, 0, st); });
        if (!dry && !arena.exact) {
          u->temb.WtT = WtT; u->temb.bt = bt; u->temb.C0 = C0; u->temb.E = E; u->temb.tt = tt; u->temb.tproj_arena = tp;
          u->temb.begin = temb_begin; u->temb.end = (int)S.size(); u->temb.ok = true;
        }
      } else {
        emit(S, [=](hipStream_t st) { return launch_small_linear(emb, E, Wt, bt, nullptr, tp, tt, Bn, E, tt, 1, 0, st); });
      }
      release(tsin); release(h1);
      probe("emb", emb, 1, E);
    }
    const int cin = c.in_channels, cpad = cin > 64 ? rup(cin, 64) : rup(cin, 32);
    const int Tp0 = pitch(T);
    Planes xin = alloc_planes((size_t)B * Tp0 * cpad);
    emit(S, [=](hipStream_t st) {
      return launch_pack_input(uu->io.x, uu->io.cx, uu->io.cond, cin - uu->io.cx, xin.hi, xin.lo, cpad, Bn, Tn, st, uu->gnx_pool, uu->gnx_words, Tp0);
    });
    const PackedW* wci = pack("conv_in", C0, 3 * cpad, {{"conv_in.weight", 1, cin, 3, cpad, 0, 0, "", 0}},
                              {{"conv_in.bias", "", "", "", C0, 0, 0, 0}});
    if (!wci) return dv_fail(DV_ERR_MISSING_WEIGHT, "%s", err.c_str());
    Act h{};
    h.p = alloc((size_t)B * Tp0 * C0); h.C = C0; h.T = T; h.Tp = Tp0; alloc_stat(h);
    {
      GemmParams g = gp_base(T, B * Tp0, C0);
      g.seg[0] = seg(xin, cpad, Planes{}, 0, 3, 1);
      g.out = h.p; stat_out(g, h);
      announce_norm("down_blocks.0.resnets.0.norm1", has("down_blocks.0.resnets.0.conv_shortcut.weight"));
      offer_next(g, h);
      gemm(S, g, wci, 3 * cin);
    }
    release(xin);
    probe("conv_in", h.p, T, C0);

    auto skip_of = [](Act a) { a.pl_hi = a.pl_lo = a.n_hi = a.n_lo = a.sn_hi = a.sn_lo = a.sr_hi = a.sr_lo = nullptr; a.n_pre.clear(); return a; };
    auto announce_resnet = [&](const std::string& rp) { announce_norm(rp + "norm1", has(rp + "conv_shortcut.weight")); };
    std::vector<Act> skips{skip_of(h)};
    auto announce_up = [&](int i, int j) {
      const std::string rp = "up_blocks." + std::to_string(i) + ".resnets." + std::to_string(j) + ".";
      if (!skips.empty()) announce_norm(rp + "norm1", has(rp + "conv_shortcut.weight"), skips.back());
    };
    for (int i = 0; i < n; ++i) {
      const std::string bp = "down_blocks." + std::to_string(i) + ".";
      const bool attn = i < n - 1;
      for (int j = 0; j < lpb; ++j) {
        const bool feeds_resampler = i < n - 1 && j == lpb - 1;
        const std::string next_rp = j + 1 < lpb ? bp + "resnets." + std::to_string(j + 1) + "." : (i == n - 1 ? std::string("mid_block.resnets.0.") : std::string());
        if (!attn && !next_rp.empty()) announce_resnet(next_rp);
        if (attn) announce_transformer_norm(bp + "attentions." + std::to_string(j) + ".", h.Tp, c.block_out_channels[i]);
        Act r = resnet(S, bp + "resnets." + std::to_string(j) + ".", h, Act{}, c.block_out_channels[i], feeds_resampler && !attn,
                       attn && chain_ok(h.Tp, c.block_out_channels[i]));
        next_norm.set = false;
        if (!r.p) return dv_fail(DV_ERR_MISSING_WEIGHT, "%s", err.c_str());
        if (attn) {
          if (!next_rp.empty()) announce_resnet(next_rp);
          Act a = transformer(S, bp + "attentions." + std::to_string(j) + ".", r, feeds_resampler);
          next_norm.set = false;
          if (!a.p) return dv_fail(DV_ERR_MISSING_WEIGHT, "%s", err.c_str());
          release_act(r);
          r = a;
        }
        h = r;
        skips.push_back(skip_of(h));
      }
      if (i < n - 1) {
        announce_resnet("down_blocks." + std::to_string(i + 1) + ".resnets.0.");
        h = resample(S, bp + "downsamplers.0.", h, true, 0);
        next_norm.set = false;
        if (!h.p) return dv_fail(DV_ERR_MISSING_WEIGHT, "%s", err.c_str());
        skips.push_back(skip_of(h));
      }
    }
    {
      announce_transformer_norm("mid_block.attentions.0.", h.Tp, h.C);
      Act r0 = resnet(S, "mid_block.resnets.0.", h, Act{}, h.C, false, chain_ok(h.Tp, h.C));
      next_norm.set = false;
      if (!r0.p) return dv_fail(DV_ERR_MISSING_WEIGHT, "%s", err.c_str());
      announce_resnet("mid_block.resnets.1.");
      Act a = transformer(S, "mid_block.attentions.0.", r0);
      next_norm.set = false;
      if (!a.p) return dv_fail(DV_ERR_MISSING_WEIGHT, "%s", err.c_str());
      release_act(r0);
      announce_up(0, 0);
      h = resnet(S, "mid_block.resnets.1.", a, Act{}, a.C);
      next_norm.set = false;
      if (!h.p) return dv_fail(DV_ERR_MISSING_WEIGHT, "%s", err.c_str());
      release_act(a);
    }
    for (int i = 0; i < n; ++i) {
      const std::string bp = "up_blocks." + std::to_string(i) + ".";
      const bool attn = i > 0, last = i == n - 1;
      const int cout = c.block_out_channels[n - 1 - i];
      for (int j = 0; j < lpb + 1; ++j) {
        Act sk = skips.back();
        skips.pop_back();
        const bool feeds_resampler = !last && j == lpb;
        const bool final_op = last && j == lpb;
        if (final_op && !attn) announce_norm("conv_norm_out", false);
        if (j < lpb && !attn) announce_up(i, j + 1);
        if (attn) announce_transformer_norm(bp + "attentions." + std::to_string(j) + ".", h.Tp, cout);
        Act r = resnet(S, bp + "resnets." + std::to_string(j) + ".", h, sk, cout, feeds_resampler && !attn, attn && chain_ok(h.Tp, cout));
        next_norm.set = false;
        if (!r.p) return dv_fail(DV_ERR_MISSING_WEIGHT, "%s", err.c_str());
        release_act(h);
        release_act(sk);
        if (attn) {
          if (final_op) announce_norm("conv_norm_out", false);
          if (j < lpb) announce_up(i, j + 1);
          Act a = transformer(S, bp + "attentions." + std::to_string(j) + ".", r, feeds_resampler);
          next_norm.set = false;
          if (!a.p) return dv_fail(DV_ERR_MISSING_WEIGHT, "%s", err.c_str());
          release_act(r);
          r = a;
        }
        h = r;
      }
      if (!last) {
        announce_up(i + 1, 0);
        Act up = resample(S, bp + "upsamplers.0.", h, false, skips.back().T);
        next_norm.set = false;
        if (!up.p) return dv_fail(DV_ERR_MISSING_WEIGHT, "%s", err.c_str());
        release_act(h);
        h = up;
      }
    }
    {
      const int co = c.out_channels;
      const PackedW* wo = pack("conv_out", co, 3 * C0, {{"conv_out.weight", 1, C0, 3, C0, 0, 0, "", 0}},
                               {{"conv_out.bias", "", "", "", co, 0, 0, 0}});
      if (!wo) return dv_fail(DV_ERR_MISSING_WEIGHT, "%s", err.c_str());
      GemmParams g = gp_base(T, B * Tp0, co);
      Planes nf;
      if (h.n_hi && h.n_pre == "conv_norm_out") {
        nf.hi = h.n_hi; nf.lo = h.n_lo;
        g.seg[0] = seg(nf, C0, Planes{}, 0, 3, 1);
      } else {
        nf = norm_apply(S, h, Act{}, "conv_norm_out", c.norm_eps, nullptr, nullptr, 0, true, nullptr);
        g.seg[0] = seg(nf, C0, Planes{}, 0, 3, 1);
      }
      g.epi = EPI_STORE_NCT; g.ldo = co;
      g.w_hi = wo->hi; g.w_lo = wo->lo; g.Kp = wo->Kp; g.N_pad = wo->N_pad; g.bias = wo->bias; g.B = B;
      g.zero_page = u->zero_page;
      const int pr = prec;
      emit_launch(S, "gemm", 2.0 * g.M * (double)co * 3 * C0, "conv_out (NCT store)",
                  [g, pr, uu](hipStream_t st) { GemmParams gg = g; gg.out = uu->io.y; return launch_gemm(gg, pr, st); });
      if (nf.hi) release(nf);
      release_act(h);
    }
    if (!err.empty()) return dv_fail(DV_ERR_MISSING_WEIGHT, "%s", err.c_str());
    if (!dry) {
      const int H = c.num_heads, nT = (L + 31) / 32;
      auto add = [&](int kind, int idx, const void* base, size_t bytes) {
        u->cond_segs.push_back(dv_unet::CondSeg{kind, idx, const_cast<char*>(static_cast<const char*>(base)), bytes});
      };
      add(1, 0, aug_emb, (size_t)E * 4);
      if (!kv_read.empty()) add(2, 0, mask_bias, (size_t)L * 4);
      if (!cross_frag.empty()) add(3, 0, xbias, (size_t)nT * 32 * 4);
      for (int i = 0; i < (int)xformers.size(); ++i) {
        const std::string& p = xformers[i].first;
        const int C = xformers[i].second;
        if (kv_read.count(p)) add(4, i, cross_kv[p], (size_t)L * 2 * C * 4);
        if (cross_frag.count(p)) {
          const XFrag& xf = cross_frag[p];
          const int d = C / H, KSq = d / 16, NBv = (d + 31) / 32;
          const size_t kb = (size_t)H * nT * KSq * 64 * 8 * sizeof(bf16_t), vb = (size_t)H * nT * 2 * NBv * 64 * 8 * sizeof(bf16_t);
          add(5, i, xf.kf_hi, kb); add(6, i, xf.kf_lo, kb); add(7, i, xf.vf_hi, vb); add(8, i, xf.vf_lo, vb);
        }
      }
    }
    return DV_OK;
  }

  float* derived(const std::string& name, const std::vector<int64_t>& shape) {
    if (dry) return nullptr;
    size_t n = 1;
    for (auto v : shape) n *= (size_t)v;
    RawW& r = u->w[name];
    if (r.numel != n) {
      if (r.p) (void)hipFree(r.p);
      r.p = nullptr;
      if (hipMalloc((void**)&r.p, n * 4) != hipSuccess) { err = "hipMalloc(derived weight) failed"; return nullptr; }
    }
    r.shape = shape; r.numel = n;
    return r.p;
  }

  void const_vec(const std::string& name, int n, float value) {
    if (dry || u->w.count(name)) return;
    RawW r;
    if (hipMalloc((void**)&r.p, (size_t)n * 4) != hipSuccess) { err = "hipMalloc(const) failed"; return; }
    r.shape = {n}; r.numel = (size_t)n;
    (void)launch_fill_f32(r.p, value, n, pack_stream);
    u->w[name] = r;
  }

  int build_penc() {
    const dv_penc_cfg& c = u->pcfg;
    const int H = c.hidden_channels, Cin = c.in_channels, Cout = c.out_channels, Ln = T, M = B * Ln, Bn = B;
    const int cpad = rup(Cin, 32), KS9 = c.ffn_kernel;
    std::vector<OpFn>& S = u->step_ops;
    dv_unet* uu = u;
    if (!dry && !u->zero_page) {
      void* z = nullptr;
      if (hipMalloc(&z, DV_ZERO_PAGE_BYTES) != hipSuccess) return dv_fail(DV_ERR_HIP, "hipMalloc(zero page) failed");
      (void)hipMemsetAsync(z, 0, DV_ZERO_PAGE_BYTES, pack_stream);
      u->owned.push_back(z);
      u->zero_page = reinterpret_cast<bf16_t*>(z);
    }

    float* keep = alloc((size_t)M);
    float* kbias = alloc((size_t)M);
    emit(S, [=](hipStream_t st) { return launch_copy_f32(uu->io.mask, keep, (int64_t)Bn * Ln, st); });
    Planes p0 = alloc_planes((size_t)M * cpad);
    {
      const float* g0 = W("pre.layer_norm.weight"); const float* b0 = W("pre.layer_norm.bias");
      emit(S, [=](hipStream_t st) {
        return launch_prompt_pre(uu->io.x, keep, g0, b0, p0.hi, p0.lo, kbias, Bn, Cin, Ln, cpad, 1e-5f, st);
      });
    }
    const PackedW* w_pre = pack("pre", H, cpad, {{"pre.conv.weight", 0, Cin, 1, cpad, 0, 0, "", 0}},
                                {{"pre.conv.bias", "", "", "", H, 0, 0, 0}});
    if (!w_pre) return dv_fail(DV_ERR_MISSING_WEIGHT, "%s", err.c_str());
    float* x = alloc((size_t)M * H);
    LnIn lin;
    {
      GemmParams g = gp_rows(Ln, M, H); g.seg[0] = seg(p0, cpad, Planes{}, 0, 1, 0);
      g.out = x; g.rowmask = keep; lin = ln_produce(g, M, H); gemm(S, g, w_pre, Cin);
    }
    release(p0);
    probe_rows("pre", x, Ln, H);

    const_vec("__const.ffn_scale", 4 * H, 1.0f / sqrtf((float)KS9));
    for (int i = 0; i < c.n_layers; ++i) {
      const std::string p = "layers." + std::to_string(i) + ".op.";
      const PackedW* w_qkv = pack(p + "qkv", 3 * H, H, {{p + "self_attn.in_proj_weight", 0, H, 1, H, 0, 0, p + "layer_norm1.weight", 0}},
                                  {{"", "", p + "self_attn.in_proj_weight", p + "layer_norm1.bias", 3 * H, H, 0, 0}});
      const PackedW* w_o = pack(p + "out", H, H, {{p + "self_attn.out_proj.weight", 0, H, 1, H, 0, 0, "", 0}}, {});
      std::vector<Piece> f1;
      for (int j = 0; j < KS9; ++j) f1.push_back({p + "ffn.ffn_1." + std::to_string(j) + ".weight", 0, H, 1, H, H * j, 0, "", 0});
      const PackedW* w_f1 = pack(p + "ffn1", 4 * H, KS9 * H, f1, {{p + "ffn.ffn_1.0.bias", "", "", "", 4 * H, 0, 0, 0}});
      const PackedW* w_f2 = pack(p + "ffn2", H, 4 * H, {{p + "ffn.ffn_2.weight", 0, 4 * H, 1, 4 * H, 0, 0, "__const.ffn_scale", 0}},
                                 {{p + "ffn.ffn_2.bias", "", "", "", H, 0, 0, 0}});
      if (!w_qkv || !w_o || !w_f1 || !w_f2) return dv_fail(DV_ERR_MISSING_WEIGHT, "%s", err.c_str());

      float* qkv = alloc((size_t)M * 3 * H);
      {
        GemmParams g = gp_rows(Ln, M, 3 * H);
        g.out = qkv; ln_consume(S, g, lin, x, w_qkv, M, H); gemm(S, g, w_qkv, H);
      }
      ln_release(lin);
      Planes ao = attention(S, qkv, 3 * H, qkv + H, qkv + 2 * H, 3 * H, kbias, Ln, Ln, H);
      release(qkv);
      float* x2 = alloc((size_t)M * H);
      {
        GemmParams g = gp_rows(Ln, M, H); g.seg[0] = seg(ao, H, Planes{}, 0, 1, 0);
        g.epi = EPI_RESIDUAL; g.res = x; g.out = x2; g.rowmask = keep; gemm(S, g, w_o, H);
      }
      release(ao); release(x);
      probe_rows("layer" + std::to_string(i) + ".attn", x2, Ln, H);

      Planes n2 = alloc_planes((size_t)M * H);
      {
        const float* g2 = W(p + "layer_norm2.weight"); const float* b2 = W(p + "layer_norm2.bias");
        const float* xin = x2;
        cur_kind = "ln_apply";
        emit(S, [=](hipStream_t st) { return launch_ln_affine(xin, g2, b2, nullptr, nullptr, n2.hi, n2.lo, Bn * Ln, H, 1e-5f, st); });
      }
      Planes hh = alloc_planes((size_t)M * 4 * H);
      {
        GemmParams g = gp_rows(Ln, M, 4 * H);
        g.seg[0] = seg(n2, H, Planes{}, 0, 1, 0);
        if (KS9 > 1) { g.seg[1] = seg(n2, H, Planes{}, 0, KS9 - 1, (KS9 - 1) / 2 - 1); g.nseg = 2; }
        g.relu = 1; g.out_hi = hh.hi; g.out_lo = hh.lo;
        gemm(S, g, w_f1, KS9 * H);
      }
      release(n2);
      if (!dry && u->keep_intermediates)
        u->probes.push_back(Probe{"layer" + std::to_string(i) + ".ffn1", nullptr, Ln, 4 * H, Ln, hh.hi, hh.lo, 1.0f / sqrtf((float)KS9)});
      float* x3 = alloc((size_t)M * H);
      {
        GemmParams g = gp_rows(Ln, M, H); g.seg[0] = seg(hh, 4 * H, Planes{}, 0, 1, 0);
        g.epi = EPI_RESIDUAL; g.res = x2; g.out = x3; g.rowmask = keep; lin = ln_produce(g, M, H); gemm(S, g, w_f2, 4 * H);
      }
      release(hh); release(x2);
      x = x3;
      probe_rows("layer" + std::to_string(i), x, Ln, H);
    }

    const PackedW* w_op = pack("out_proj", Cout, H, {{"out_proj.conv.weight", 0, H, 1, H, 0, 0, "out_proj.layer_norm.weight", 0}},
                               {{"out_proj.conv.bias", "", "out_proj.conv.weight", "out_proj.layer_norm.bias", Cout, H, 0, 0}});
    if (!w_op) return dv_fail(DV_ERR_MISSING_WEIGHT, "%s", err.c_str());
    float* z = alloc((size_t)M * Cout);
    {
      GemmParams g = gp_rows(Ln, M, Cout);
      g.out = z; g.rowmask = keep; ln_consume(S, g, lin, x, w_op, M, H); gemm(S, g, w_op, H);
    }
    ln_release(lin); release(x);
    probe_rows("out_proj", z, Ln, Cout);
    if (has("layer_norm.weight")) {
      const float* gl = W("layer_norm.weight"); const float* bl = W("layer_norm.bias");
      cur_kind = "ln_apply";
      emit(S, [=](hipStream_t st) { return launch_ln_affine(z, gl, bl, keep, uu->io.y, nullptr, nullptr, Bn * Ln, Cout, 1e-5f, st); });
    } else {
      emit(S, [=](hipStream_t st) { return launch_copy_f32(z, uu->io.y, (int64_t)Bn * Ln * Cout, st); });
    }
    release(z);
    if (!err.empty()) return dv_fail(DV_ERR_MISSING_WEIGHT, "%s", err.c_str());
    return DV_OK;
  }
};

static int cond_table_finish(dv_unet* u);
extern "C" int dv_unet_prepare(dv_unet* u, int32_t B, int32_t T, int32_t L, int32_t precision, int32_t force_upsample_size) {
  if (!u) return dv_fail(DV_ERR_INVALID, "dv_unet_prepare: null handle");
  if (B <= 0 || T <= 0 || L <= 0) return dv_fail(DV_ERR_INVALID, "dv_unet_prepare: B, T, L must be positive");
  if (precision != DV_PREC_BF16X3 && precision != DV_PREC_BF16) return dv_fail(DV_ERR_INVALID, "unknown precision %d", precision);
  {
    int t = T;
    for (int i = 0; i < u->cfg.n_levels - 1; ++i) t = (t + 2 - 3) / 2 + 1;
    if (t < 1) return dv_fail(DV_ERR_INVALID, "T=%d too short for %d levels", T, u->cfg.n_levels);
  }
  HIPCHK(hipDeviceSynchronize());
  HIPCHK(gemm_init());
  gemm_env_refresh();
  HIPCHK(attn_init());
  HIPCHK(chain_init());
  HIPCHK(ff_split_init());
  HIPCHK(qkv_split_init());
  unet_release_prepared(u, !u->weights_dirty && u->packed_prec == precision);
  u->packed_prec = precision;
  u->B = B; u->T = T; u->L = L; u->precision = precision; u->force_up = force_upsample_size;
  const char* keep = getenv("DVITS_KEEP_INTERMEDIATES");
  u->keep_intermediates = keep && keep[0] == '1';

  const bool persist_env = [] { const char* e = getenv("DVITS_PERSIST"); return e && e[0] == '1'; }();
  size_t need = 0;
  {
    Builder b{};
    b.u = u; b.dry = true; b.B = B; b.T = T; b.L = L; b.prec = precision;
    b.arena.reuse = !u->keep_intermediates;
    b.arena.exact = persist_env;
    int rc = b.build();
    if (rc != DV_OK) return rc;
    need = b.arena.high;
  }
  HIPCHK(hipMalloc((void**)&u->slab, need + 256));
  u->slab_bytes = need;
  {
    Builder b{};
    b.u = u; b.dry = false; b.B = B; b.T = T; b.L = L; b.prec = precision;
    b.arena.reuse = !u->keep_intermediates;
    b.arena.exact = persist_env;
    int rc = b.build();
    if (rc != DV_OK) { unet_release_prepared(u); return rc; }
  }
  if (!persist_env) {
    int rc = autotune_gemms(u, precision);
    if (rc != DV_OK) { unet_release_prepared(u); return rc; }
  }
  {
    const char* pe = getenv("DVITS_PERSIST");
    const int n = (int)u->step_ops.size();
    int best0 = 0, best1 = 0;
    for (int i = 0; i < n;) {
      if (u->step_pop[i] < 0) { ++i; continue; }
      int j = i;
      while (j < n && u->step_pop[j] >= 0) ++j;
      if (j - i > best1 - best0) { best0 = i; best1 = j; }
      i = j;
    }
    if (pe && pe[0] == '1' && best1 - best0 >= 8 && persist_init() == hipSuccess) {
      const int np = best1 - best0;
      HIPCHK(hipMalloc((void**)&u->pops_dev, (size_t)np * sizeof(PersistOp)));
      u->owned.push_back(u->pops_dev);
      HIPCHK(hipMemcpy(u->pops_dev, u->pops.data() + u->step_pop[best0], (size_t)np * sizeof(PersistOp), hipMemcpyHostToDevice));
      HIPCHK(hipMalloc((void**)&u->psync, sizeof(PersistSync)));
      u->owned.push_back(u->psync);
      HIPCHK(hipMemset(u->psync, 0, sizeof(PersistSync)));
      u->p_begin = best0; u->p_end = best1; u->persist_on = true;
    }
  }
  if (int rc = cond_table_finish(u)) { unet_release_prepared(u); return rc; }
  HIPCHK(hipDeviceSynchronize());
  u->prepared = true;
  u->weights_dirty = false;
  u->generation = ++g_generation;
  return DV_OK;
}

struct dv_penc { dv_unet core; };

extern "C" int dv_penc_create(const dv_penc_cfg* cfg, dv_penc** out) {
  if (!cfg || !out) return dv_fail(DV_ERR_INVALID, "dv_penc_create: null argument");
  if (cfg->in_channels <= 0 || cfg->in_channels > 512) return dv_fail(DV_ERR_INVALID, "in_channels must be 1..512");
  if (cfg->hidden_channels <= 0 || cfg->hidden_channels % 32 != 0 || cfg->hidden_channels > 512)
    return dv_fail(DV_ERR_INVALID, "hidden_channels must be a positive multiple of 32, <= 512");
  if (cfg->out_channels <= 0 || cfg->out_channels % 4 != 0 || cfg->out_channels > 2048)
    return dv_fail(DV_ERR_INVALID, "out_channels must be a positive multiple of 4");
  if (cfg->n_layers < 0 || cfg->n_layers > 64) return dv_fail(DV_ERR_INVALID, "n_layers out of range");
  if (cfg->num_heads <= 0 || cfg->hidden_channels % cfg->num_heads != 0 || (cfg->hidden_channels / cfg->num_heads) % 4 != 0 ||
      cfg->hidden_channels / cfg->num_heads > 64)
    return dv_fail(DV_ERR_INVALID, "head dim must be a multiple of 4 and <= 64");
  if (cfg->ffn_kernel < 1 || cfg->ffn_kernel % 2 != 1) return dv_fail(DV_ERR_INVALID, "ffn_kernel must be odd ('SAME' padding)");
  dv_penc* p = new dv_penc();
// ... 681 lines not shown
```

diff-vits_amd/csrc/kernels_qkv.hip:

```cpp
#include "dv_common.h"
#include "dv_device.h"

#include <cstdlib>
#include <type_traits>

typedef __attribute__((ext_vector_type(8))) __bf16 bf16x8;
typedef __attribute__((ext_vector_type(16))) float f32x16;

#ifdef DV_GEMM_TRACE
__device__ unsigned long long g_qkv_trace[1024 * 16];
__device__ int g_qkv_sel = 0;
#define DV_QTRACE(i) do { if (threadIdx.x == 0 && blockIdx.x < 1024 && (g_qkv_sel == 0 || g_qkv_sel == C)) g_qkv_trace[blockIdx.x * 16 + (i)] = __builtin_amdgcn_s_memtime(); } while (0)
extern "C" int dv_debug_qkv_trace_select(int c) {
  hipError_t e = hipMemcpyToSymbol(HIP_SYMBOL(g_qkv_sel), &c, sizeof(c));
  void* d = nullptr;
  if (e == hipSuccess) e = hipGetSymbolAddress(&d, HIP_SYMBOL(g_qkv_trace));
  return (int)(e != hipSuccess ? e : hipMemset(d, 0, sizeof(g_qkv_trace)));
}
extern "C" int dv_debug_qkv_trace(unsigned long long* host, int n_wg) {
  return (int)hipMemcpyFromSymbol(host, HIP_SYMBOL(g_qkv_trace), (size_t)n_wg * 16 * sizeof(unsigned long long));
}
#else
#define DV_QTRACE(i) do {} while (0)
#endif

namespace {

constexpr int NWV = 8, NT = 64 * NWV, BM = 64, BN = 64;
constexpr int CHP = BM * 128;
__device__ __forceinline__ int swz(int row) { return (row >> 1) & 7; }
__device__ __forceinline__ unsigned pk(float lo, float hi) { return dv_cvt_pk_bf16(lo, hi); }
struct BFrag { bf16x8 h, l; };

template <int C>
struct QGeom {
  static constexpr int NSPL = C / BN;
  static constexpr int KS = C / 16, U = KS / 4;
  static constexpr int DEPTH = U < 6 ? U : 6;
  static constexpr int A_CH = C / 64, A_PL = A_CH * CHP;
  static constexpr bool ONE = 2 * A_PL + 65536 + 8192 <= 160 * 1024;
  static constexpr int RED = ONE ? 65536 : 32768;
  static constexpr int SMEM = 2 * A_PL + RED;
  static constexpr int D3 = 3 * U < 9 ? 3 * U : 9;
  static constexpr int JT = C / 32;
  static constexpr int ENT_MAX = RED / 8;
  static_assert(C % 128 == 0 && KS % 4 == 0 && SMEM + 8192 <= 160 * 1024, "geometry");
};

template <int C, int MODE>
__global__ __launch_bounds__(NT) void k_qkv_split(const ChainParams p) {
  using G = QGeom<C>;
  extern __shared__ __attribute__((aligned(1024))) char smem[];
  char* const a_reg = smem;
  char* const red_reg = smem + 2 * G::A_PL;
  __shared__ __attribute__((aligned(16))) float s_gscale[C], s_gshift[C];
  __shared__ __attribute__((aligned(16))) float2 s_ln[BM];
  asm volatile("" ::"s"(p.M), "s"(p.gamma), "s"(p.w1_lo), "s"(p.out1), "s"(p.u2), "s"(p.sa_kf_hi), "s"(p.sa_vf_lo), "s"(p.qs_flags));
  DV_QTRACE(0);
  const int tid = threadIdx.x, lane = tid & 63, wave = __builtin_amdgcn_readfirstlane(tid >> 6);
  const int l31 = lane & 31, lh = lane >> 5;
  const int cf = wave & 1, kq = wave >> 1;
  const int fg = wave >> 1;
  const bool xl = p.qs_xcd != 0;
  int rb, s;
  if (xl) { const int x = (int)blockIdx.x & 7, i = (int)blockIdx.x >> 3, rbl = i / G::NSPL; s = i - rbl * G::NSPL; rb = rbl * 8 + x; }
  else { rb = (int)blockIdx.x / G::NSPL; s = (int)blockIdx.x - rb * G::NSPL; }
  const int m0 = rb * BM;
  unsigned xcc = 0;
  asm volatile("s_getreg_b32 %0, hwreg(HW_REG_XCC_ID)" : "=s"(xcc));
  xcc &= 0xfu;
  const int r_row = tid >> 3, r_e8 = tid & 7;

  auto load_unit = [&](const bf16_t* wf_hi, const bf16_t* wf_lo, int nf, int j) {
    const size_t e = ((size_t)(nf * G::KS + kq * G::U + j) * 64 + lane) * 8;
    BFrag f;
    f.h = *reinterpret_cast<const bf16x8*>(wf_hi + e);
    f.l = *reinterpret_cast<const bf16x8*>(wf_lo + e);
    return f;
  };
  BFrag bq[G::DEPTH];
  auto job_prologue = [&](const bf16_t* wf_hi, const bf16_t* wf_lo, int nf) __attribute__((always_inline)) {
#pragma unroll
    for (int j = 0; j < G::DEPTH; ++j) bq[j] = load_unit(wf_hi, wf_lo, nf, j);
    __builtin_amdgcn_sched_barrier(0);
  };
  f32x16 acc[2];
  auto job_loop = [&](const bf16_t* wf_hi, const bf16_t* wf_lo, int nf, auto swap_tag) __attribute__((always_inline)) {
    constexpr bool SWAP = decltype(swap_tag)::value;
#pragma unroll
    for (int rf = 0; rf < 2; ++rf)
#pragma unroll
      for (int r = 0; r < 16; ++r) acc[rf][r] = 0.f;
    auto read_a = [&](int u, bf16x8 (&h)[2], bf16x8 (&l)[2]) {
      const int c16 = (kq * G::U + u) * 2 + lh;
#pragma unroll
      for (int rf = 0; rf < 2; ++rf) {
        const int row = rf * 32 + l31;
        const int off = (c16 >> 3) * CHP + row * 128 + (((c16 & 7) ^ swz(row)) << 4);
        h[rf] = *reinterpret_cast<const bf16x8*>(a_reg + off);
        l[rf] = *reinterpret_cast<const bf16x8*>(a_reg + G::A_PL + off);
      }
    };
    bf16x8 ah[2][2], al[2][2];
    read_a(0, ah[0], al[0]);
#pragma unroll
    for (int u = 0; u < G::U; ++u) {
      const int cur = u & 1;
      if (u + 1 < G::U) read_a(u + 1, ah[cur ^ 1], al[cur ^ 1]);
      const BFrag f = bq[u % G::DEPTH];
      if (SWAP) {
        acc[0] = __builtin_amdgcn_mfma_f32_32x32x16_bf16(al[cur][0], f.h, acc[0], 0, 0, 0);
        acc[1] = __builtin_amdgcn_mfma_f32_32x32x16_bf16(al[cur][1], f.h, acc[1], 0, 0, 0);
        acc[0] = __builtin_amdgcn_mfma_f32_32x32x16_bf16(ah[cur][0], f.l, acc[0], 0, 0, 0);
        acc[1] = __builtin_amdgcn_mfma_f32_32x32x16_bf16(ah[cur][1], f.l, acc[1], 0, 0, 0);
        acc[0] = __builtin_amdgcn_mfma_f32_32x32x16_bf16(ah[cur][0], f.h, acc[0], 0, 0, 0);
        acc[1] = __builtin_amdgcn_mfma_f32_32x32x16_bf16(ah[cur][1], f.h, acc[1], 0, 0, 0);
      } else {
        acc[0] = __builtin_amdgcn_mfma_f32_32x32x16_bf16(f.h, al[cur][0], acc[0], 0, 0, 0);
        acc[1] = __builtin_amdgcn_mfma_f32_32x32x16_bf16(f.h, al[cur][1], acc[1], 0, 0, 0);
        acc[0] = __builtin_amdgcn_mfma_f32_32x32x16_bf16(f.l, ah[cur][0], acc[0], 0, 0, 0);
        acc[1] = __builtin_amdgcn_mfma_f32_32x32x16_bf16(f.l, ah[cur][1], acc[1], 0, 0, 0);
        acc[0] = __builtin_amdgcn_mfma_f32_32x32x16_bf16(f.h, ah[cur][0], acc[0], 0, 0, 0);
        acc[1] = __builtin_amdgcn_mfma_f32_32x32x16_bf16(f.h, ah[cur][1], acc[1], 0, 0, 0);
      }
      __builtin_amdgcn_sched_barrier(0);
      if (u + G::DEPTH < G::U) bq[u % G::DEPTH] = load_unit(wf_hi, wf_lo, nf, u + G::DEPTH);
      __builtin_amdgcn_sched_barrier(0);
    }
  };
  float4* const red4 = reinterpret_cast<float4*>(red_reg);
  auto pieces = [&](const f32x16& a0, const f32x16& a1, float4 (&v)[2]) __attribute__((always_inline)) {
    if constexpr (G::ONE) {
      __syncthreads();
#pragma unroll
      for (int g = 0; g < 4; ++g) {
        red4[((((cf * 4 + kq) * 2 + 0) * 4 + g) << 6) + lane] = make_float4(a0[4 * g], a0[4 * g + 1], a0[4 * g + 2], a0[4 * g + 3]);
        red4[((((cf * 4 + kq) * 2 + 1) * 4 + g) << 6) + lane] = make_float4(a1[4 * g], a1[4 * g + 1], a1[4 * g + 2], a1[4 * g + 3]);
      }
      __syncthreads();
#pragma unroll
      for (int rf = 0; rf < 2; ++rf) {
        float4 t = red4[((((cf * 4 + 0) * 2 + rf) * 4 + fg) << 6) + lane];
#pragma unroll
        for (int k = 1; k < 4; ++k) {
          const float4 w = red4[((((cf * 4 + k) * 2 + rf) * 4 + fg) << 6) + lane];
          t.x += w.x; t.y += w.y; t.z += w.z; t.w += w.w;
        }
        v[rf] = t;
      }
    } else {
#pragma unroll
      for (int rf = 0; rf < 2; ++rf) {
        __syncthreads();
#pragma unroll
        for (int g = 0; g < 4; ++g)
          red4[(((cf * 4 + kq) * 4 + g) << 6) + lane] = rf == 0 ? make_float4(a0[4 * g], a0[4 * g + 1], a0[4 * g + 2], a0[4 * g + 3])
                                                                 : make_float4(a1[4 * g], a1[4 * g + 1], a1[4 * g + 2], a1[4 * g + 3]);
        __syncthreads();
        float4 t = red4[(((cf * 4 + 0) * 4 + fg) << 6) + lane];
#pragma unroll
        for (int k = 1; k < 4; ++k) {
          const float4 w = red4[(((cf * 4 + k) * 4 + fg) << 6) + lane];
          t.x += w.x; t.y += w.y; t.z += w.z; t.w += w.w;
        }
        v[rf] = t;
      }
    }
  };
  auto put_planes = [&](int j, float v0, float v1, float v2, float v3) __attribute__((always_inline)) {
    const int ch = 4 * (r_e8 + 8 * j);
    uint2 hw, lw;
    hw.x = pk(v0, v1); hw.y = pk(v2, v3);
    lw.x = pk(v0 - __uint_as_float(hw.x << 16), v1 - __uint_as_float(hw.x & 0xffff0000u));
    lw.y = pk(v2 - __uint_as_float(hw.y << 16), v3 - __uint_as_float(hw.y & 0xffff0000u));
    const int off = (ch >> 6) * CHP + r_row * 128 + ((((ch & 63) >> 3) ^ swz(r_row)) << 4) + ((ch & 7) >> 2) * 8;
    *reinterpret_cast<uint2*>(a_reg + off) = hw;
    *reinterpret_cast<uint2*>(a_reg + G::A_PL + off) = lw;
  };

  float4 rv[G::JT];
  const float4 b1v = *reinterpret_cast<const float4*>(p.b1 + s * BN + cf * 32 + 8 * fg + 4 * lh);
  float4 rres[2];
  float4 h2v[2];
  if constexpr (MODE >= 1) {
    const int ncol_ = s * BN + cf * 32 + 8 * fg + 4 * lh;
#pragma unroll
    for (int rf = 0; rf < 2; ++rf)
      rres[rf] = p.res ? *reinterpret_cast<const float4*>(p.res + (size_t)(m0 + rf * 32 + l31) * C + ncol_) : make_float4(0.f, 0.f, 0.f, 0.f);
    const unsigned a_base = (unsigned)(size_t)a_reg;
    const int d_row = wave * 8 + (lane >> 3), d_slot = lane & 7;
#pragma unroll
    for (int c = 0; c < G::A_CH; ++c) {
      const size_t e = (size_t)(m0 + d_row) * C + c * 64 + ((d_slot ^ swz(d_row)) << 3);
      const unsigned dst = a_base + (unsigned)(c * CHP + wave * 1024);
      glds16(p.a_hi + e, dst);
      glds16(p.a_lo + e, dst + G::A_PL);
    }
    job_prologue(p.w1_hi, p.w1_lo, s * 2 + cf);
    DV_QTRACE(10);
    wait_vmcnt<2 * G::DEPTH>();
  } else {
  const int T = p.T, b_item = m0 / T, Tv = p.Tv > 0 ? p.Tv : T;
  {
    const float* xr = p.x + (size_t)(m0 + r_row) * C + 4 * r_e8;
#pragma unroll
    for (int j = 0; j < G::JT; ++j) rv[j] = *reinterpret_cast<const float4*>(xr + 32 * j);
  }
  job_prologue(p.w1_hi, p.w1_lo, s * 2 + cf);
  DV_QTRACE(10);
  {
    const int Gn = p.groups, cg = C / Gn, nvb = cg >> 4, RB = T >> 5, nblk = C >> 4, n_ent = RB * nblk;
    const int cc = min(tid, C - 1);
    const float pg = p.gamma[cc], pb = p.beta[cc];
    float2* s_ent = reinterpret_cast<float2*>(red_reg);
    for (int e0 = 0; e0 < n_ent; e0 += 2 * NT) {
      float2 ev[2];
#pragma unroll
      for (int k = 0; k < 2; ++k) {
        const int e = min(e0 + k * NT + tid, n_ent - 1);
        ev[k] = reinterpret_cast<const float2*>(p.stat16)[(size_t)b_item * n_ent + e];
      }
#pragma unroll
      for (int k = 0; k < 2; ++k) {
        const int e = e0 + k * NT + tid;
        if (e < n_ent) s_ent[e] = ev[k];
      }
    }
    __syncthreads();
    DV_QTRACE(11);
    const int lpg = 64 / Gn, g = lane / lpg, sub = lane - g * lpg;
    const double inv_last = 1.0 / (double)(16 * min(32, Tv - 32 * (RB - 1)));
    double s1 = 0, q = 0;
    for (int i0 = sub; i0 < RB * nvb; i0 += 4 * lpg) {
#pragma unroll
      for (int k = 0; k < 4; ++k) {
        const int i = i0 + k * lpg, rbk = i / nvb;
        const float2 v = s_ent[min(rbk * nblk + g * nvb + (i - rbk * nvb), n_ent - 1)];
        if (i < RB * nvb) { s1 += (double)v.x; q += (double)v.y + (double)v.x * (double)v.x * (rbk == RB - 1 ? inv_last : (1.0 / 512.0)); }
      }
    }
    for (int o = lpg >> 1; o > 0; o >>= 1) { s1 += __shfl_xor(s1, o); q += __shfl_xor(q, o); }
    const double n = (double)cg * (double)Tv, mean_d = s1 / n;
    double var = q / n - mean_d * mean_d;
    var = var > 0 ? var : 0;
    const float mean = (float)mean_d, rstd = 1.0f / sqrtf((float)var + p.gn_eps);
    const int src_lane = cc / cg * lpg;
    const float gm = __shfl(mean, src_lane), gr = __shfl(rstd, src_lane);
    if (tid < C) { const float a = gr * pg; s_gscale[tid] = a; s_gshift[tid] = pb - gm * a; }
    __syncthreads();
    DV_QTRACE(12);
  }
#pragma unroll
  for (int j = 0; j < G::JT; ++j) {
    const int ch = 4 * (r_e8 + 8 * j);
    const float4 sc = *reinterpret_cast<const float4*>(s_gscale + ch);
    const float4 sh = *reinterpret_cast<const float4*>(s_gshift + ch);
    put_planes(j, fmaf(rv[j].x, sc.x, sh.x), fmaf(rv[j].y, sc.y, sh.y), fmaf(rv[j].z, sc.z, sh.z), fmaf(rv[j].w, sc.w, sh.w));
  }
  }
  DV_QTRACE(1);
  __syncthreads();
  DV_QTRACE(2);

  job_loop(p.w1_hi, p.w1_lo, s * 2 + cf, std::false_type{});
  DV_QTRACE(3);
  const int ncol = s * BN + cf * 32 + 8 * fg + 4 * lh;
  {
    const float4 b4 = b1v;
    float4 pv[2];
    pieces(acc[0], acc[1], pv);
#pragma unroll
    for (int rf = 0; rf < 2; ++rf) {
      float4 v = pv[rf];
      v.x += b4.x; v.y += b4.y; v.z += b4.z; v.w += b4.w;
      if constexpr (MODE >= 1) {
        const float4 r4 = rf == 0 ? rres[0] : rres[1];
        v.x += r4.x; v.y += r4.y; v.z += r4.z; v.w += r4.w;
        if (rf == 0) h2v[0] = v; else h2v[1] = v;
      }
      float4* const dst = reinterpret_cast<float4*>(p.out1 + (size_t)(m0 + rf * 32 + l31) * C + ncol);
      if (xl) *dst = v; else st_handover16(dst, v);
    }
  }
  asm volatile("s_waitcnt vmcnt(0)" ::: "memory");
  __syncthreads();
  if (tid == 0) {
    const unsigned long long fv = 1ull + xcc;
    if (xl) *reinterpret_cast<volatile unsigned long long*>(p.qs_flags + (size_t)rb * G::NSPL + s) = fv;
    else __hip_atomic_store(p.qs_flags + (size_t)rb * G::NSPL + s, fv, __ATOMIC_RELAXED, __HIP_MEMORY_SCOPE_SYSTEM);
  }
  const int nfq = s * 2 + cf, nfk = C / 32 + s * 2 + cf, nfv = 2 * (C / 32) + s * 2 + cf;
  BFrag b3[MODE == 0 ? G::D3 : 1];
  auto load_unit3 = [&](int j) {
    const int u = j / 3, ps = j - 3 * u;
    return load_unit(p.w2_hi, p.w2_lo, ps == 0 ? nfq : (ps == 1 ? nfk : nfv), u);
  };
  if constexpr (MODE == 0) {
#pragma unroll
    for (int j = 0; j < G::D3; ++j) b3[j] = load_unit3(j);
    __builtin_amdgcn_sched_barrier(0);
  } else job_prologue(p.w2_hi, p.w2_lo, nfq);
  DV_QTRACE(4);
  const float4 uq = *reinterpret_cast<const float4*>(p.u2 + ncol), bq4 = *reinterpret_cast<const float4*>(p.b2 + ncol);
  float4 uk = uq, bk4 = bq4;
  float uvv = 0.f, bvv = 0.f;
  if constexpr (MODE == 0) {
    uk = *reinterpret_cast<const float4*>(p.u2 + C + ncol); bk4 = *reinterpret_cast<const float4*>(p.b2 + C + ncol);
    const int vch = s * BN + cf * 32 + l31;
    uvv = p.u2[2 * C + vch]; bvv = p.b2[2 * C + vch];
  }

  auto wait_flags = [&](const unsigned long long* fl, unsigned code) __attribute__((always_inline)) {
    for (int spins = 0;; ++spins) {
      bool ok = true;
      unsigned long long fv = 0;
      if (lane < G::NSPL) {
        if (xl) asm volatile("global_load_dwordx2 %0, %1, off sc1\n\ts_waitcnt vmcnt(0)" : "=v"(fv) : "v"(fl + lane) : "memory");
        else fv = __hip_atomic_load(fl + lane, __ATOMIC_RELAXED, __HIP_MEMORY_SCOPE_SYSTEM);
        ok = fv != ~0ull;
      }
      if (__all(ok)) {
        if (xl && __any(lane < G::NSPL && fv != 1ull + xcc)) {
          if (lane == 0) {
            p.qs_status[1] = (unsigned)(size_t)p.qs_flags; p.qs_status[2] = blockIdx.x; p.qs_status[3] = 0xc2u; p.qs_status[4] = xcc;
            __hip_atomic_store(p.qs_status, 1u, __ATOMIC_RELAXED, __HIP_MEMORY_SCOPE_SYSTEM);
          }
        }
        break;
      }
      const bool lost = (spins & 63) == 63 && __hip_atomic_load(p.qs_status, __ATOMIC_RELAXED, __HIP_MEMORY_SCOPE_SYSTEM) != 0u;
      if (lost) break;
      if (spins > p.qs_spin) {
        if (lane == 0) {
          p.qs_status[1] = (unsigned)(size_t)p.qs_flags; p.qs_status[2] = blockIdx.x; p.qs_status[3] = code; p.qs_status[4] = (unsigned)__builtin_popcountll(__ballot(!ok));
          __hip_atomic_store(p.qs_status, 1u, __ATOMIC_RELAXED, __HIP_MEMORY_SCOPE_SYSTEM);
        }
        break;
      }
      __builtin_amdgcn_s_sleep(1);
    }
    asm volatile("" ::: "memory");
  };
  wait_flags(p.qs_flags + (size_t)rb * G::NSPL, 0xc1u);
  DV_QTRACE(5);
  {
    const float4* hr = reinterpret_cast<const float4*>(p.out1 + (size_t)(m0 + r_row) * C + 4 * r_e8);
    if (xl) {
      if constexpr (G::JT == 4)
        asm volatile("global_load_dwordx4 %0, %4, off sc1\n\tglobal_load_dwordx4 %1, %4, off offset:128 sc1\n\t"
                     "global_load_dwordx4 %2, %4, off offset:256 sc1\n\tglobal_load_dwordx4 %3, %4, off offset:384 sc1\n\t"
                     "s_waitcnt vmcnt(0)"
                     : "=&v"(rv[0]), "=&v"(rv[1]), "=&v"(rv[2]), "=&v"(rv[3]) : "v"(hr) : "memory");
      else if constexpr (G::JT == 8)
        asm volatile("global_load_dwordx4 %0, %8, off sc1\n\tglobal_load_dwordx4 %1, %8, off offset:128 sc1\n\t"
                     "global_load_dwordx4 %2, %8, off offset:256 sc1\n\tglobal_load_dwordx4 %3, %8, off offset:384 sc1\n\t"
                     "global_load_dwordx4 %4, %8, off offset:512 sc1\n\tglobal_load_dwordx4 %5, %8, off offset:640 sc1\n\t"
                     "global_load_dwordx4 %6, %8, off offset:768 sc1\n\tglobal_load_dwordx4 %7, %8, off offset:896 sc1\n\t"
                     "s_waitcnt vmcnt(0)"
                     : "=&v"(rv[0]), "=&v"(rv[1]), "=&v"(rv[2]), "=&v"(rv[3]), "=&v"(rv[4]), "=&v"(rv[5]), "=&v"(rv[6]), "=&v"(rv[7]) : "v"(hr) : "memory");
      else
        asm volatile("global_load_dwordx4 %0, %12, off sc1\n\tglobal_load_dwordx4 %1, %12, off offset:128 sc1\n\t"
                     "global_load_dwordx4 %2, %12, off offset:256 sc1\n\tglobal_load_dwordx4 %3, %12, off offset:384 sc1\n\t"
                     "global_load_dwordx4 %4, %12, off offset:512 sc1\n\tglobal_load_dwordx4 %5, %12, off offset:640 sc1\n\t"
                     "global_load_dwordx4 %6, %12, off offset:768 sc1\n\tglobal_load_dwordx4 %7, %12, off offset:896 sc1\n\t"
                     "global_load_dwordx4 %8, %12, off offset:1024 sc1\n\tglobal_load_dwordx4 %9, %12, off offset:1152 sc1\n\t"
                     "global_load_dwordx4 %10, %12, off offset:1280 sc1\n\tglobal_load_dwordx4 %11, %12, off offset:1408 sc1\n\t"
                     "s_waitcnt vmcnt(0)"
                     : "=&v"(rv[0]), "=&v"(rv[1]), "=&v"(rv[2]), "=&v"(rv[3]), "=&v"(rv[4]), "=&v"(rv[5]), "=&v"(rv[6]), "=&v"(rv[7]),
                       "=&v"(rv[8 % G::JT]), "=&v"(rv[9 % G::JT]), "=&v"(rv[10 % G::JT]), "=&v"(rv[11 % G::JT])
                     : "v"(hr) : "memory");
    } else {
#pragma unroll
      for (int j = 0; j < G::JT; ++j) rv[j] = ld_handover16(hr + 8 * j);
    }
    float s1 = 0.f;
#pragma unroll
    for (int j = 0; j < G::JT; ++j) s1 += (rv[j].x + rv[j].y) + (rv[j].z + rv[j].w);
    s1 += __shfl_xor(s1, 1); s1 += __shfl_xor(s1, 2); s1 += __shfl_xor(s1, 4);
    const float mean = s1 * (1.0f / (float)C);
    float m2 = 0.f;
#pragma unroll
    for (int j = 0; j < G::JT; ++j) {
      const float d0 = rv[j].x - mean, d1 = rv[j].y - mean, d2 = rv[j].z - mean, d3 = rv[j].w - mean;
      m2 = fmaf(d0, d0, m2); m2 = fmaf(d1, d1, m2); m2 = fmaf(d2, d2, m2); m2 = fmaf(d3, d3, m2);
    }
    m2 += __shfl_xor(m2, 1); m2 += __shfl_xor(m2, 2); m2 += __shfl_xor(m2, 4);
    if (r_e8 == 0) s_ln[r_row] = make_float2(mean, 1.0f / sqrtf(m2 * (1.0f / (float)C) + p.ln_eps));
#pragma unroll
    for (int j = 0; j < G::JT; ++j) put_planes(j, rv[j].x, rv[j].y, rv[j].z, rv[j].w);
  }
  __syncthreads();
  DV_QTRACE(6);

  auto finish_q = [&](const float4 (&pv)[2]) __attribute__((always_inline)) {
#pragma unroll
    for (int rf = 0; rf < 2; ++rf) {
      const float4 v = pv[rf];
      const float2 st = s_ln[rf * 32 + l31];
      float4 o;
      o.x = st.y * (v.x - st.x * uq.x) + bq4.x; o.y = st.y * (v.y - st.x * uq.y) + bq4.y;
      o.z = st.y * (v.z - st.x * uq.z) + bq4.z; o.w = st.y * (v.w - st.x * uq.w) + bq4.w;
      dv_st16(p.out2 + (size_t)(m0 + rf * 32 + l31) * p.ldo2 + ncol, o);
    }
  };
  if constexpr (MODE == 1) {
    job_loop(p.w2_hi, p.w2_lo, nfq, std::false_type{});
    float4 pv[2];
    pieces(acc[0], acc[1], pv);
    finish_q(pv);
    DV_QTRACE(7); DV_QTRACE(8); DV_QTRACE(9);
    return;
  } else if constexpr (MODE == 2) {
    constexpr int d = C / 8, KSq = d / 16, HS = BN / d, KP = (2 * HS < NWV) ? 2 : 1;
    static_assert(C <= 256 && 2 * HS * KP == NWV, "MODE 2 geometry");
    job_loop(p.w2_hi, p.w2_lo, nfq, std::false_type{});
    job_prologue(p.w3_hi, p.w3_lo, s * 2 + cf);
    {
      float4 pv[2];
      pieces(acc[0], acc[1], pv);
#pragma unroll
      for (int rf = 0; rf < 2; ++rf) {
        const float4 v = pv[rf];
        const float2 st = s_ln[rf * 32 + l31];
        const float q0 = (st.y * (v.x - st.x * uq.x) + bq4.x) * p.xa_qscale, q1 = (st.y * (v.y - st.x * uq.y) + bq4.y) * p.xa_qscale;
        const float q2 = (st.y * (v.z - st.x * uq.z) + bq4.z) * p.xa_qscale, q3 = (st.y * (v.w - st.x * uq.w) + bq4.w) * p.xa_qscale;
        uint2 hw, lw;
        hw.x = pk(q0, q1); hw.y = pk(q2, q3);
        lw.x = pk(q0 - __uint_as_float(hw.x << 16), q1 - __uint_as_float(hw.x & 0xffff0000u));
        lw.y = pk(q2 - __uint_as_float(hw.y << 16), q3 - __uint_as_float(hw.y & 0xffff0000u));
        const int nl = cf * 32 + 8 * fg + 4 * lh, row = rf * 32 + l31;
        const int off = row * 128 + (((nl >> 3) ^ swz(row)) << 4) + ((nl & 7) >> 2) * 8;
        *reinterpret_cast<uint2*>(a_reg + off) = hw;
        *reinterpret_cast<uint2*>(a_reg + G::A_PL + off) = lw;
      }
    }
    const int job = KP == 2 ? (wave & 3) : wave, jh = job >> 1, jrf = job & 1, kh = KP == 2 ? wave >> 2 : 0;
    const int head = s * HS + jh, nT = p.xa_nT;
    const int b_item = m0 / p.T;
    const size_t bh = (size_t)b_item * 8 + head;
    const bf16x8* kfh = reinterpret_cast<const bf16x8*>(p.xa_kf_hi) + bh * nT * KSq * 64 + lane;
    const bf16x8* kfl = reinterpret_cast<const bf16x8*>(p.xa_kf_lo) + bh * nT * KSq * 64 + lane;
    const bf16x8* vfh = reinterpret_cast<const bf16x8*>(p.xa_vf_hi) + bh * nT * 2 * 64 + lane;
    const bf16x8* vfl = reinterpret_cast<const bf16x8*>(p.xa_vf_lo) + bh * nT * 2 * 64 + lane;
    const float* kbias = p.xa_bias + (size_t)b_item * nT * 32 + 4 * lh;
    struct KVT { bf16x8 kh[KSq], kl[KSq], vh[2], vl[2]; float4 bv[4]; };
    auto load_kv = [&](int t) {
      KVT f;
      const int tc = min(t, nT - 1);
#pragma unroll
      for (int ks = 0; ks < KSq; ++ks) { f.kh[ks] = kfh[(size_t)(tc * KSq + ks) * 64]; f.kl[ks] = kfl[(size_t)(tc * KSq + ks) * 64]; }
#pragma unroll
      for (int kb = 0; kb < 2; ++kb) { f.vh[kb] = vfh[(size_t)(tc * 2 + kb) * 64]; f.vl[kb] = vfl[(size_t)(tc * 2 + kb) * 64]; }
#pragma unroll
      for (int g = 0; g < 4; ++g) f.bv[g] = *reinterpret_cast<const float4*>(kbias + tc * 32 + 8 * g);
      return f;
    };
    KVT cur = load_kv(kh);
    __builtin_amdgcn_sched_barrier(0);
    __syncthreads();
    bf16x8 qh[KSq], ql[KSq];
#pragma unroll
    for (int ks = 0; ks < KSq; ++ks) {
      const int c16 = ((jh * d + ks * 16) >> 3) + lh, row = jrf * 32 + l31;
      const int off = row * 128 + ((c16 ^ swz(row)) << 4);
      qh[ks] = *reinterpret_cast<const bf16x8*>(a_reg + off);
      ql[ks] = *reinterpret_cast<const bf16x8*>(a_reg + G::A_PL + off);
    }
    f32x16 o;
#pragma unroll
    for (int r = 0; r < 16; ++r) o[r] = 0.f;
    float m_run = -1e30f, l_run = 0.f;
    DV_QTRACE(7);
    for (int t = kh; t < nT; t += KP) {
      __builtin_amdgcn_sched_barrier(0);
      KVT nxt = load_kv(t + KP);
      __builtin_amdgcn_sched_barrier(0);
      f32x16 sc;
#pragma unroll
      for (int g = 0; g < 4; ++g) { sc[4 * g] = cur.bv[g].x; sc[4 * g + 1] = cur.bv[g].y; sc[4 * g + 2] = cur.bv[g].z; sc[4 * g + 3] = cur.bv[g].w; }
#pragma unroll
      for (int ks = 0; ks < KSq; ++ks) {
        sc = __builtin_amdgcn_mfma_f32_32x32x16_bf16(cur.kl[ks], qh[ks], sc, 0, 0, 0);
        sc = __builtin_amdgcn_mfma_f32_32x32x16_bf16(cur.kh[ks], ql[ks], sc, 0, 0, 0);
        sc = __builtin_amdgcn_mfma_f32_32x32x16_bf16(cur.kh[ks], qh[ks], sc, 0, 0, 0);
      }
      float tmax = m_run;
#pragma unroll
      for (int r = 0; r < 16; ++r) tmax = fmaxf(tmax, sc[r]);
      const float m_new = pair_max32(tmax);
      const float alpha = __builtin_amdgcn_exp2f(m_run - m_new);
      m_run = m_new;
      float psum = 0.f;
#pragma unroll
      for (int r = 0; r < 16; ++r) { sc[r] = __builtin_amdgcn_exp2f(sc[r] - m_new); psum += sc[r]; }
      l_run = l_run * alpha + psum;
      if (__any(alpha != 1.0f)) {
#pragma unroll
        for (int r = 0; r < 16; ++r) o[r] *= alpha;
      }
#pragma unroll
      for (int kb = 0; kb < 2; ++kb) {
        typedef unsigned u32x4 __attribute__((ext_vector_type(4)));
        u32x4 hw, lw;
        if (DV_ATTN_PF16) {
#pragma unroll
          for (int e = 0; e < 4; ++e) hw[e] = dv_cvt_pk_f16(sc[kb * 8 + 2 * e], sc[kb * 8 + 2 * e + 1]);
          const dv_f16x8 ph16 = __builtin_bit_cast(dv_f16x8, hw);
          o = __builtin_amdgcn_mfma_f32_32x32x16_f16(__builtin_bit_cast(dv_f16x8, cur.vl[kb]), ph16, o, 0, 0, 0);
          o = __builtin_amdgcn_mfma_f32_32x32x16_f16(__builtin_bit_cast(dv_f16x8, cur.vh[kb]), ph16, o, 0, 0, 0);
          continue;
        }
#pragma unroll
        for (int e = 0; e < 4; ++e) {
          const float x0 = sc[kb * 8 + 2 * e], x1 = sc[kb * 8 + 2 * e + 1];
          const unsigned h2 = pk(x0, x1);
          hw[e] = h2;
          lw[e] = pk(x0 - __uint_as_float(h2 << 16), x1 - __uint_as_float(h2 & 0xffff0000u));
        }
        const bf16x8 ph = __builtin_bit_cast(bf16x8, hw), pl = __builtin_bit_cast(bf16x8, lw);
        o = __builtin_amdgcn_mfma_f32_32x32x16_bf16(cur.vl[kb], ph, o, 0, 0, 0);
        o = __builtin_amdgcn_mfma_f32_32x32x16_bf16(cur.vh[kb], pl, o, 0, 0, 0);
        o = __builtin_amdgcn_mfma_f32_32x32x16_bf16(cur.vh[kb], ph, o, 0, 0, 0);
      }
      cur = nxt;
    }
    if constexpr (KP == 2) {
      float* mg = reinterpret_cast<float*>(red_reg);
      __syncthreads();
      if (kh == 1) {
        float* q = mg + (size_t)job * 18 * 64 + lane;
        q[0] = m_run; q[64] = l_run;
#pragma unroll
        for (int r = 0; r < 16; ++r) q[(2 + r) * 64] = o[r];
      }
      __syncthreads();
      if (kh == 0) {
        const float* q = mg + (size_t)job * 18 * 64 + lane;
        const float m1 = q[0], l1 = q[64];
        const float mm = fmaxf(m_run, m1);
        const float a0 = __builtin_amdgcn_exp2f(m_run - mm), a1 = __builtin_amdgcn_exp2f(m1 - mm);
        l_run = l_run * a0 + l1 * a1;
#pragma unroll
        for (int r = 0; r < 16; ++r) o[r] = o[r] * a0 + q[(2 + r) * 64] * a1;
      }
    }
    DV_QTRACE(8);
    if (kh == 0) {
      const float inv = 1.0f / pair_sum32(l_run);
      const size_t ro = (size_t)(m0 + jrf * 32 + l31) * C + head * d + 4 * lh;
#pragma unroll
      for (int g = 0; g < 4; ++g) {
        if (8 * g < d) {
          const float v0 = o[4 * g] * inv, v1 = o[4 * g + 1] * inv, v2 = o[4 * g + 2] * inv, v3 = o[4 * g + 3] * inv;
          uint2 hw, lw;
          hw.x = pk(v0, v1); hw.y = pk(v2, v3);
          lw.x = pk(v0 - __uint_as_float(hw.x << 16), v1 - __uint_as_float(hw.x & 0xffff0000u));
          lw.y = pk(v2 - __uint_as_float(hw.y << 16), v3 - __uint_as_float(hw.y & 0xffff0000u));
          *reinterpret_cast<uint2*>(p.qs_o_hi + ro + 8 * g) = hw;
          *reinterpret_cast<uint2*>(p.qs_o_lo + ro + 8 * g) = lw;
        }
      }
    }
    asm volatile("s_waitcnt vmcnt(0)" ::: "memory");
    __syncthreads();
    const unsigned long long* fl2 = p.qs_flags + (size_t)(p.M / BM) * G::NSPL + (size_t)rb * G::NSPL;
    if (tid == 0) *reinterpret_cast<volatile unsigned long long*>(const_cast<unsigned long long*>(fl2) + s) = 1ull + xcc;
    const float4 b3v = *reinterpret_cast<const float4*>(p.b3 + ncol);
    wait_flags(fl2, 0xc3u);
    {
      const unsigned a_base = (unsigned)(size_t)a_reg;
      const int d_row = wave * 8 + (lane >> 3), d_slot = lane & 7;
#pragma unroll
      for (int c = 0; c < G::A_CH; ++c) {
        const size_t e = (size_t)(m0 + d_row) * C + c * 64 + ((d_slot ^ swz(d_row)) << 3);
        const unsigned dst = a_base + (unsigned)(c * CHP + wave * 1024);
        glds16_sc1(p.qs_o_hi + e, dst);
        glds16_sc1(p.qs_o_lo + e, dst + G::A_PL);
      }
      asm volatile("s_waitcnt vmcnt(0)" ::: "memory");
    }
    __syncthreads();
    DV_QTRACE(9);
    job_loop(p.w3_hi, p.w3_lo, s * 2 + cf, std::false_type{});
    {
      float4 pv[2];
      pieces(acc[0], acc[1], pv);
      __shared__ float2 s_rp[2 * 32 * 2 * 4];
#pragma unroll
      for (int rf = 0; rf < 2; ++rf) {
        const float4 r4 = rf == 0 ? h2v[0] : h2v[1];
        float4 v = pv[rf];
        v.x += b3v.x + r4.x; v.y += b3v.y + r4.y; v.z += b3v.z + r4.z; v.w += b3v.w + r4.w;
        const size_t ob = (size_t)(m0 + rf * 32 + l31) * C + ncol;
        dv_st16(p.out3 + ob, v);
        uint2 hw, lw;
        hw.x = pk(v.x, v.y); hw.y = pk(v.z, v.w);
        lw.x = pk(v.x - __uint_as_float(hw.x << 16), v.y - __uint_as_float(hw.x & 0xffff0000u));
        lw.y = pk(v.z - __uint_as_float(hw.y << 16), v.w - __uint_as_float(hw.y & 0xffff0000u));
        dv_st8(p.out3_hi + ob, hw);
        dv_st8(p.out3_lo + ob, lw);
        const float a = pair_sum32((v.x + v.y) + (v.z + v.w));
        const float mb = a * (1.0f / 8.0f);
        const float q = pair_sum32((v.x - mb) * (v.x - mb) + (v.y - mb) * (v.y - mb) + (v.z - mb) * (v.z - mb) + (v.w - mb) * (v.w - mb));
        if (lh == 0) s_rp[((rf * 32 + l31) * 2 + cf) * 4 + fg] = make_float2(a, q);
      }
      __syncthreads();
      if (tid < 2 * BM) {
        const int row = tid >> 1, f = tid & 1;
        float s1 = 0.f;
#pragma unroll
        for (int k = 0; k < 4; ++k) s1 += s_rp[(row * 2 + f) * 4 + k].x;
        const float mean = s1 * (1.0f / 32.0f);
        float m2 = 0.f;
#pragma unroll
        for (int k = 0; k < 4; ++k) {
          const float2 t2 = s_rp[(row * 2 + f) * 4 + k];
          const float dm = t2.x * (1.0f / 8.0f) - mean;
          m2 += t2.y + 8.0f * dm * dm;
        }
        reinterpret_cast<float2*>(p.rowstat3)[(size_t)(m0 + row) * (C / 32) + s * 2 + f] = make_float2(s1, m2);
      }
    }
    DV_QTRACE(13);
    return;
  } else {
    f32x16 aq[2], ak[2], av[2];
#pragma unroll
    for (int rf = 0; rf < 2; ++rf)
#pragma unroll
      for (int r = 0; r < 16; ++r) { aq[rf][r] = 0.f; ak[rf][r] = 0.f; av[rf][r] = 0.f; }
    {
      auto read_a = [&](int u, bf16x8 (&h)[2], bf16x8 (&l)[2]) {
        const int c16 = (kq * G::U + u) * 2 + lh;
#pragma unroll
        for (int rf = 0; rf < 2; ++rf) {
          const int row = rf * 32 + l31;
          const int off = (c16 >> 3) * CHP + row * 128 + (((c16 & 7) ^ swz(row)) << 4);
          h[rf] = *reinterpret_cast<const bf16x8*>(a_reg + off);
          l[rf] = *reinterpret_cast<const bf16x8*>(a_reg + G::A_PL + off);
        }
      };
      bf16x8 ah[2][2], al[2][2];
      read_a(0, ah[0], al[0]);
#pragma unroll
      for (int j = 0; j < 3 * G::U; ++j) {
        const int u = j / 3, ps = j - 3 * u, cur = u & 1;
        if (ps == 0 && u + 1 < G::U) read_a(u + 1, ah[cur ^ 1], al[cur ^ 1]);
        const BFrag f = b3[j % G::D3];
        if (ps == 2) {
#pragma unroll
          for (int rf = 0; rf < 2; ++rf) av[rf] = __builtin_amdgcn_mfma_f32_32x32x16_bf16(al[cur][rf], f.h, av[rf], 0, 0, 0);
#pragma unroll
          for (int rf = 0; rf < 2; ++rf) av[rf] = __builtin_amdgcn_mfma_f32_32x32x16_bf16(ah[cur][rf], f.l, av[rf], 0, 0, 0);
#pragma unroll
          for (int rf = 0; rf < 2; ++rf) av[rf] = __builtin_amdgcn_mfma_f32_32x32x16_bf16(ah[cur][rf], f.h, av[rf], 0, 0, 0);
        } else if (ps == 1) {
#pragma unroll
          for (int rf = 0; rf < 2; ++rf) ak[rf] = __builtin_amdgcn_mfma_f32_32x32x16_bf16(f.h, al[cur][rf], ak[rf], 0, 0, 0);
#pragma unroll
          for (int rf = 0; rf < 2; ++rf) ak[rf] = __builtin_amdgcn_mfma_f32_32x32x16_bf16(f.l, ah[cur][rf], ak[rf], 0, 0, 0);
#pragma unroll
          for (int rf = 0; rf < 2; ++rf) ak[rf] = __builtin_amdgcn_mfma_f32_32x32x16_bf16(f.h, ah[cur][rf], ak[rf], 0, 0, 0);
        } else {
#pragma unroll
          for (int rf = 0; rf < 2; ++rf) aq[rf] = __builtin_amdgcn_mfma_f32_32x32x16_bf16(f.h, al[cur][rf], aq[rf], 0, 0, 0);
#pragma unroll
          for (int rf = 0; rf < 2; ++rf) aq[rf] = __builtin_amdgcn_mfma_f32_32x32x16_bf16(f.l, ah[cur][rf], aq[rf], 0, 0, 0);
#pragma unroll
          for (int rf = 0; rf < 2; ++rf) aq[rf] = __builtin_amdgcn_mfma_f32_32x32x16_bf16(f.h, ah[cur][rf], aq[rf], 0, 0, 0);
        }
        __builtin_amdgcn_sched_barrier(0);
        if (j + G::D3 < 3 * G::U) b3[j % G::D3] = load_unit3(j + G::D3);
        __builtin_amdgcn_sched_barrier(0);
      }
    }
    DV_QTRACE(7);
    float4 pv[2];
    pieces(aq[0], aq[1], pv);
    finish_q(pv);
    pieces(ak[0], ak[1], pv);
#pragma unroll
    for (int rf = 0; rf < 2; ++rf) {
      const float4 v = pv[rf];
      const float2 st = s_ln[rf * 32 + l31];
      const float o0 = st.y * (v.x - st.x * uk.x) + bk4.x, o1 = st.y * (v.y - st.x * uk.y) + bk4.y;
      const float o2 = st.y * (v.z - st.x * uk.z) + bk4.z, o3 = st.y * (v.w - st.x * uk.w) + bk4.w;
      uint2 hw, lw;
      hw.x = pk(o0, o1); hw.y = pk(o2, o3);
      lw.x = pk(o0 - __uint_as_float(hw.x << 16), o1 - __uint_as_float(hw.x & 0xffff0000u));
      lw.y = pk(o2 - __uint_as_float(hw.y << 16), o3 - __uint_as_float(hw.y & 0xffff0000u));
      const size_t eo = (((size_t)((m0 >> 5) + rf) * (C / 16) + (ncol >> 4)) * 64 + (fg & 1) * 32 + l31) * 8 + lh * 4;
      dv_st8(p.sa_kf_hi + eo, hw);
      dv_st8(p.sa_kf_lo + eo, lw);
    }
    DV_QTRACE(8);
    pieces(av[0], av[1], pv);
#pragma unroll
    for (int rf = 0; rf < 2; ++rf) {
      const float4 v = pv[rf];
      const float4 s01 = *reinterpret_cast<const float4*>(&s_ln[rf * 32 + 8 * fg + 4 * lh]);
      const float4 s23 = *reinterpret_cast<const float4*>(&s_ln[rf * 32 + 8 * fg + 4 * lh + 2]);
      const float x0 = s01.y * (v.x - s01.x * uvv) + bvv, x1 = s01.w * (v.y - s01.z * uvv) + bvv;
      const float x2 = s23.y * (v.z - s23.x * uvv) + bvv, x3 = s23.w * (v.w - s23.z * uvv) + bvv;
      uint2 hw, lw;
      if (DV_ATTN_PF16) {
        dv_split_pk_f16(x0, x1, hw.x, lw.x);
        dv_split_pk_f16(x2, x3, hw.y, lw.y);
      } else {
        hw.x = pk(x0, x1); hw.y = pk(x2, x3);
        lw.x = pk(x0 - __uint_as_float(hw.x << 16), x1 - __uint_as_float(hw.x & 0xffff0000u));
        lw.y = pk(x2 - __uint_as_float(hw.y << 16), x3 - __uint_as_float(hw.y & 0xffff0000u));
      }
      const size_t eo = (((((size_t)((m0 >> 5) + rf) * (C / 32) + s * 2 + cf) * 2 + (fg >> 1)) * 64 + lane) * 8) + (fg & 1) * 4;
      dv_st8(p.sa_vf_hi + eo, hw);
      dv_st8(p.sa_vf_lo + eo, lw);
    }
    DV_QTRACE(9);
  }
}

template <int C>
hipError_t qkv_init_one() {
  hipError_t e = hipFuncSetAttribute(reinterpret_cast<const void*>(k_qkv_split<C, 0>), hipFuncAttributeMaxDynamicSharedMemorySize, QGeom<C>::SMEM);
  if (e == hipSuccess) e = hipFuncSetAttribute(reinterpret_cast<const void*>(k_qkv_split<C, 1>), hipFuncAttributeMaxDynamicSharedMemorySize, QGeom<C>::SMEM);
  if constexpr (C <= 256) {
    if (e == hipSuccess) e = hipFuncSetAttribute(reinterpret_cast<const void*>(k_qkv_split<C, 2>), hipFuncAttributeMaxDynamicSharedMemorySize, QGeom<C>::SMEM);
  }
  return e;
}
template <int C>
hipError_t qkv_launch_one(const ChainParams& pin, hipStream_t st) {
  ChainParams p = pin;
  p.qs_xcd = qkv_split_xcd_local(p.M) ? 1 : 0;
  if (p.amode == 1) hipLaunchKernelGGL((k_qkv_split<C, 0>), dim3((p.M / BM) * QGeom<C>::NSPL), dim3(NT), QGeom<C>::SMEM, st, p);
  else if (!p.xa_kf_hi) hipLaunchKernelGGL((k_qkv_split<C, 1>), dim3((p.M / BM) * QGeom<C>::NSPL), dim3(NT), QGeom<C>::SMEM, st, p);
  else {
    if constexpr (C <= 256) {
      if (!p.qs_xcd) return hipErrorInvalidValue;
      hipLaunchKernelGGL((k_qkv_split<C, 2>), dim3((p.M / BM) * QGeom<C>::NSPL), dim3(NT), QGeom<C>::SMEM, st, p);
    } else return hipErrorInvalidValue;
  }
  return hipGetLastError();
}

}

bool qkv_split_xcd_local(int M) {
  static const bool xcd_on = [] { const char* e = getenv("DVITS_QKV_XCD"); return !(e && e[0] == '0'); }();
  return xcd_on && (M / BM) % 8 == 0;
}
hipError_t qkv_split_init() {
  hipError_t e = qkv_init_one<128>();
  if (e == hipSuccess) e = qkv_init_one<256>();
  return e != hipSuccess ? e : qkv_init_one<384>();
}
bool qkv_split_supported(const ChainParams& p, int precision) {
  if (precision != 0 || !p.out1 || (p.ldo2 & 3) != 0) return false;
  if (p.C != 128 && p.C != 256 && p.C != 384) return false;
  if (p.T % BM != 0 || p.M % p.T != 0 || p.Tv < 0 || p.Tv > p.T || (p.Tv > 0 && p.Tv <= p.T - 32)) return false;
  if (p.amode == 1) {
    if (p.passes != 3 || !p.sa_kf_hi || !p.sa_kf_lo || !p.sa_vf_hi || !p.sa_vf_lo || p.res || p.xa_kf_hi || !p.out2 || p.ldo2 < p.C) return false;
    const int G = p.groups;
    if (G <= 0 || G > 64 || (G & (G - 1)) != 0 || p.C % G != 0 || (p.C / G) % 16 != 0) return false;
    if ((p.T / 32) * (p.C / 16) > 2 * 4 * 4 * 64 * 16 / 8) return false;
    return true;
  }
  if (p.amode != 0 || p.passes != 1 || !p.a_hi || !p.a_lo || p.sa_kf_hi) return false;
  if (!p.xa_kf_hi) return p.out2 && p.ldo2 >= p.C;
  return p.C <= 256 && p.xa_kf_lo && p.xa_vf_hi && p.xa_vf_lo && p.xa_bias && p.xa_nT > 0 && p.xa_d == p.C / 8 && p.w3_hi && p.w3_lo && p.b3 &&
         p.out3 && p.out3_hi && p.out3_lo && p.rowstat3 && p.qs_o_hi && p.qs_o_lo && qkv_split_xcd_local(p.M);
}
int qkv_split_flags(const ChainParams& p) { return (p.M / BM) * (p.C / BN) * (p.xa_kf_hi ? 2 : 1); }
hipError_t launch_qkv_split(const ChainParams& p, int precision, hipStream_t st) {
  if (!qkv_split_supported(p, precision)) return hipErrorInvalidValue;
  if ((p.amode == 1 && (!p.x || !p.stat16 || !p.gamma || !p.beta)) || !p.w1_hi || !p.w1_lo || !p.b1 || !p.w2_hi || !p.w2_lo || !p.b2 || !p.u2 ||
      !p.qs_flags || !p.qs_status)
    return hipErrorInvalidValue;
  if (!gemm_handover_rounds()) {
    static const int n_cu = [] { int d = 0, n = 0; (void)hipGetDevice(&d); (void)hipDeviceGetAttribute(&n, hipDeviceAttributeMultiprocessorCount, d); return n; }();
    if ((p.M / BM) * (p.C / BN) > n_cu) return hipErrorInvalidValue;
  }
  if (p.C == 128) return qkv_launch_one<128>(p, st);
  if (p.C == 256) return qkv_launch_one<256>(p, st);
  return qkv_launch_one<384>(p, st);
}
```

Measured before the change: 67500 mel-frames/s.

## Extend column-split fused transformer head kernel to C=512 with 32-row blocks

```diff
diff --git a/diff-vits_amd/csrc/engine.hip b/diff-vits_amd/csrc/engine.hip
--- a/diff-vits_amd/csrc/engine.hip
+++ b/diff-vits_amd/csrc/engine.hip
@@ -511,6 +511,17 @@
            B * Tn >= chain_min_rows &&
            G > 0 && G <= 64 && (G & (G - 1)) == 0 && C % G == 0 && (C / G) % 16 == 0 && (Tn / 32) * (C / 16) <= (C / 128) * 2048;
   }
+  int split32_wgs(int Tn, int C) const { ChainParams cp{}; cp.M = B * Tn; cp.C = C; return qkv_split_flags(cp); }
+  bool split32_ok(int Tn, int C) const {
+    const int G = u->cfg.norm_num_groups, H = u->cfg.num_heads;
+    if (C != 512 || C > qkv_split_max_c || C < qkv_split_min_c || !chain_on || !fuse_ln || arena.exact || prec != DV_PREC_BF16X3) return false;
+    if (!attn_frag_on || H <= 0 || C % H != 0 || (C / H) % 16 != 0 || C / H > 64) return false;
+    if (!handover_ok() || autotune_on() || Tn % 32 != 0) return false;
+    if (!(G > 0 && G <= 64 && (G & (G - 1)) == 0 && C % G == 0 && (C / G) % 16 == 0 && (Tn / 32) * (C / 16) <= 4096)) return false;
+    const int n_wg = split32_wgs(Tn, C);
+    return n_wg <= n_cu && n_wg >= qkv_split_min_wg;
+  }
+  bool xf_own_norm(int Tn, int C) const { return chain_ok(Tn, C) || split32_ok(Tn, C); }
   bool frag(const PackedW* cw) {
     if (dry) return true;
     PackedW* w = const_cast<PackedW*>(cw);
@@ -592,7 +603,7 @@
     next_norm.eps = u->cfg.norm_eps; next_norm.silu = true;
   }
   void announce_transformer_norm(const std::string& tp, int Tp, int C) {
-    if (chain_ok(Tp, C)) return;
+    if (xf_own_norm(Tp, C)) return;
     announce_norm(tp + "norm", false);
     next_norm.eps = 1e-6f; next_norm.silu = false;
   }
@@ -637,6 +648,7 @@
   bool qkv_split_on = [] { const char* e = getenv("DVITS_QKV_SPLIT"); return !(e && e[0] == '0'); }();
   int qkv_split_min_wg = [] { const char* e = getenv("DVITS_QKV_SPLIT_MIN_WG"); return e ? atoi(e) : 96; }();
   int qkv_split_min_c = [] { const char* e = getenv("DVITS_QKV_SPLIT_MIN_C"); return e ? atoi(e) : 256; }();
+  int qkv_split_max_c = [] { const char* e = getenv("DVITS_QKV_SPLIT_MAX_C"); return e ? atoi(e) : 512; }();
   bool qkv_xa_on = [] { const char* e = getenv("DVITS_QKV_XA"); return !(e && e[0] == '0'); }();
   int qkv_xa_min_c = [] { const char* e = getenv("DVITS_QKV_XA_MIN_C"); return e ? atoi(e) : 256; }();
   int ff_split_min_wg = [] { const char* e = getenv("DVITS_FF_SPLIT_MIN_WG"); return e ? atoi(e) : 96; }();
@@ -1002,10 +1014,13 @@
 
     float* h3 = nullptr;
     LnIn l3;
-    if (chain_ok(b.Tp, C) && x.stat16) {
+    const bool split32 = !chain_ok(b.Tp, C) && split32_ok(b.Tp, C) &&
+                         gnx_used + 2 * (((size_t)split32_wgs(b.Tp, C) + 1) & ~(size_t)1) <= dv_unet::GNX_POOL;
+    if ((chain_ok(b.Tp, C) || split32) && x.stat16) {
       if (!(frag(b.w_in) && frag(b.w_qkv) && frag(b.w_o1) && frag(b.w_q2))) return Act{};
       float* h = nullptr;
       const Planes ao = xf_head(ops, b, h);
+      if (!ao.hi) return Act{};
       if (!xf_tail(ops, b, h, ao, h3, l3)) return Act{};
     } else h3 = xf_attention_gemms(ops, b, l3);
     return xf_ff(ops, b, h3, l3, want_planes);
@@ -1032,9 +1047,12 @@
       cp.nsplit = !chain_split_on ? 1 : (rbs * 3 <= cus ? 3 : (rbs * 2 <= cus ? 2 : 1));
     }
     const int n_qflags = qkv_split_flags(cp);
-    const bool split = qkv_split_on && C >= qkv_split_min_c && sa_frag && handover_ok() && !autotune_on() &&
+    const bool chained = chain_ok(Tp, C);
+    const int q_rows = M * (C / 64) / n_qflags;
+    const bool split = (qkv_split_on || !chained) && C >= qkv_split_min_c && C <= qkv_split_max_c && sa_frag && handover_ok() && !autotune_on() &&
                        n_qflags <= n_cu && n_qflags >= qkv_split_min_wg && gnx_used + (size_t)n_qflags <= dv_unet::GNX_POOL &&
-                       qkv_split(ops, cp, strf("norm+proj_in+LN+q|Kfrag|Vfrag (%d wg / 64 rows) M=%d C=%d N2=%d", C / 64, M, C, 3 * C));
+                       qkv_split(ops, cp, strf(chained ? "norm+proj_in+LN+q|Kfrag|Vfrag (%d wg / %d rows) M=%d C=%d N2=%d" : "norm+proj_in+LN+q|Kfrag|Vfrag [%d wg / %d rows] M=%d C=%d N2=%d", C / 64, q_rows, M, C, 3 * C));
+    if (!split && !chained) { err = "the column-split block head refused a shape its planner admitted"; return Planes{}; }
     if (!split) chain(ops, cp, sa_frag ? "norm+proj_in+LN+q|Kfrag|Vfrag" : "norm+proj_in+LN+qkv");
     probe(b.p + "proj_in", h, Tn, C);
     Planes ao;
@@ -1076,12 +1094,19 @@
       cp.nsplit = (chain_split_on && nsg >= 2 && rbs * nsg <= cus) ? nsg : 1;
     }
     const int n_qflags = qkv_split_flags(cp);
-    const bool split = qkv_split_on && C >= qkv_split_min_c && handover_ok() && !autotune_on() &&
+    const bool chained = chain_ok(b.Tp, C);
+    const int q_rows = M * (C / 64) / n_qflags;
+    const bool split = (qkv_split_on || !chained) && C >= qkv_split_min_c && C <= qkv_split_max_c && handover_ok() && !autotune_on() &&
                        n_qflags <= n_cu && n_qflags >= qkv_split_min_wg && gnx_used + (size_t)n_qflags <= dv_unet::GNX_POOL &&
-                       qkv_split(ops, cp, strf("to_out+res+LN+to_q (%d wg / 64 rows) M=%d C=%d N2=%d", C / 64, M, C, C));
-    if (!split) chain(ops, cp, "to_out+res+LN+to_q");
-    release(ao); release(h);
-    probe(b.tb + "attn1", h2, b.Tn, C);
+                       qkv_split(ops, cp, strf(chained ? "to_out+res+LN+to_q (%d wg / %d rows) M=%d C=%d N2=%d" : "to_out+res+LN+to_q [%d wg / %d rows] M=%d C=%d N2=%d", C / 64, q_rows, M, C, C));
+    if (!split && !chained) {
+      release(q2); release(h2);
+      q2 = xf_out1_q2(ops, b, h, ao, h2);
+    } else {
+      if (!split) chain(ops, cp, "to_out+res+LN+to_q");
+      release(ao); release(h);
+      probe(b.tb + "attn1", h2, b.Tn, C);
+    }
     h3 = cross_attention_out(ops, b, q2, h2, l3);
     return true;
   }
@@ -1155,7 +1180,13 @@
     ln_release(l1);
     Planes ao = attention(ops, qkv, 3 * C, qkv + C, qkv + 2 * C, 3 * C, nullptr, Tp, Tn, C, Tp);
     release(qkv);
-    float* h2 = alloc((size_t)M * C);
+    float* h2 = nullptr;
+    float* q2 = xf_out1_q2(ops, b, h, ao, h2);
+    return cross_attention_out(ops, b, q2, h2, l3);
+  }
+  float* xf_out1_q2(std::vector<OpFn>& ops, const Xf& b, float* h, Planes ao, float*& h2) {
+    const int C = b.C, Tn = b.Tn, M = b.M;
+    h2 = alloc((size_t)M * C);
     LnIn l2;
     {
       GemmParams g = gp_base(Tn, M, C); g.seg[0] = seg(ao, C, Planes{}, 0, 1, 0);
@@ -1171,7 +1202,7 @@
       g.out = q2; ln_consume(ops, g, l2, h2, b.w_q2, M, C); gemm(ops, g, b.w_q2, C);
     }
     ln_release(l2);
-    return cross_attention_out(ops, b, q2, h2, l3);
+    return q2;
   }
   float* cross_attention_out(std::vector<OpFn>& ops, const Xf& b, float* q2, float* h2, LnIn& l3) {
     const int C = b.C, Tp = b.Tp, M = b.M;
@@ -1570,7 +1601,7 @@
         if (!attn && !next_rp.empty()) announce_resnet(next_rp);
         if (attn) announce_transformer_norm(bp + "attentions." + std::to_string(j) + ".", h.Tp, c.block_out_channels[i]);
         Act r = resnet(S, bp + "resnets." + std::to_string(j) + ".", h, Act{}, c.block_out_channels[i], feeds_resampler && !attn,
-                       attn && chain_ok(h.Tp, c.block_out_channels[i]));
+                       attn && xf_own_norm(h.Tp, c.block_out_channels[i]));
         next_norm.set = false;
         if (!r.p) return dv_fail(DV_ERR_MISSING_WEIGHT, "%s", err.c_str());
         if (attn) {
@@ -1594,7 +1625,7 @@
     }
     {
       announce_transformer_norm("mid_block.attentions.0.", h.Tp, h.C);
-      Act r0 = resnet(S, "mid_block.resnets.0.", h, Act{}, h.C, false, chain_ok(h.Tp, h.C));
+      Act r0 = resnet(S, "mid_block.resnets.0.", h, Act{}, h.C, false, xf_own_norm(h.Tp, h.C));
       next_norm.set = false;
       if (!r0.p) return dv_fail(DV_ERR_MISSING_WEIGHT, "%s", err.c_str());
       announce_resnet("mid_block.resnets.1.");
@@ -1620,7 +1651,7 @@
         if (final_op && !attn) announce_norm("conv_norm_out", false);
         if (j < lpb && !attn) announce_up(i, j + 1);
         if (attn) announce_transformer_norm(bp + "attentions." + std::to_string(j) + ".", h.Tp, cout);
-        Act r = resnet(S, bp + "resnets." + std::to_string(j) + ".", h, sk, cout, feeds_resampler && !attn, attn && chain_ok(h.Tp, cout));
+        Act r = resnet(S, bp + "resnets." + std::to_string(j) + ".", h, sk, cout, feeds_resampler && !attn, attn && xf_own_norm(h.Tp, cout));
         next_norm.set = false;
         if (!r.p) return dv_fail(DV_ERR_MISSING_WEIGHT, "%s", err.c_str());
         release_act(h);
diff --git a/diff-vits_amd/csrc/kernels_qkv.hip b/diff-vits_amd/csrc/kernels_qkv.hip
--- a/diff-vits_amd/csrc/kernels_qkv.hip
+++ b/diff-vits_amd/csrc/kernels_qkv.hip
@@ -27,24 +27,30 @@
 namespace {
 
 constexpr int NWV = 8, NT = 64 * NWV, BM = 64, BN = 64;
-constexpr int CHP = BM * 128;
 __device__ __forceinline__ int swz(int row) { return (row >> 1) & 7; }
 __device__ __forceinline__ unsigned pk(float lo, float hi) { return dv_cvt_pk_bf16(lo, hi); }
 struct BFrag { bf16x8 h, l; };
 
-template <int C>
+constexpr int qrows(int c) { return c <= 384 ? 64 : 32; }
+template <int C, int ROWS = qrows(C)>
 struct QGeom {
+  static constexpr int RB = ROWS, NRF = RB / 32;
+  static constexpr int CHP = RB * 128;
+  static constexpr int TPR = NT / RB;
   static constexpr int NSPL = C / BN;
   static constexpr int KS = C / 16, U = KS / 4;
   static constexpr int DEPTH = U < 6 ? U : 6;
   static constexpr int A_CH = C / 64, A_PL = A_CH * CHP;
-  static constexpr bool ONE = 2 * A_PL + 65536 + 8192 <= 160 * 1024;
-  static constexpr int RED = ONE ? 65536 : 32768;
+  static constexpr bool ONE = 2 * A_PL + NRF * 32768 + 8192 <= 160 * 1024;
+  static constexpr int RED = ONE ? NRF * 32768 : 32768;
   static constexpr int SMEM = 2 * A_PL + RED;
   static constexpr int D3 = 3 * U < 9 ? 3 * U : 9;
-  static constexpr int JT = C / 32;
+  static constexpr int JT = C / (4 * TPR);
   static constexpr int ENT_MAX = RED / 8;
+  static constexpr int NRG = RB / 8;
+  static constexpr int DMA_CH = A_CH * NRG / NWV;
   static_assert(C % 128 == 0 && KS % 4 == 0 && SMEM + 8192 <= 160 * 1024, "geometry");
+  static_assert((RB == 32 || RB == 64) && NWV % NRG == 0 && (A_CH * NRG) % NWV == 0 && JT * 4 * TPR == C, "row passes");
 };
 
 template <int C, int MODE>
@@ -54,7 +60,7 @@
   char* const a_reg = smem;
   char* const red_reg = smem + 2 * G::A_PL;
   __shared__ __attribute__((aligned(16))) float s_gscale[C], s_gshift[C];
-  __shared__ __attribute__((aligned(16))) float2 s_ln[BM];
+  __shared__ __attribute__((aligned(16))) float2 s_ln[G::RB];
   asm volatile("" ::"s"(p.M), "s"(p.gamma), "s"(p.w1_lo), "s"(p.out1), "s"(p.u2), "s"(p.sa_kf_hi), "s"(p.sa_vf_lo), "s"(p.qs_flags));
   DV_QTRACE(0);
   const int tid = threadIdx.x, lane = tid & 63, wave = __builtin_amdgcn_readfirstlane(tid >> 6);
@@ -65,11 +71,12 @@
   int rb, s;
   if (xl) { const int x = (int)blockIdx.x & 7, i = (int)blockIdx.x >> 3, rbl = i / G::NSPL; s = i - rbl * G::NSPL; rb = rbl * 8 + x; }
   else { rb = (int)blockIdx.x / G::NSPL; s = (int)blockIdx.x - rb * G::NSPL; }
-  const int m0 = rb * BM;
+  const int m0 = rb * G::RB;
   unsigned xcc = 0;
   asm volatile("s_getreg_b32 %0, hwreg(HW_REG_XCC_ID)" : "=s"(xcc));
   xcc &= 0xfu;
-  const int r_row = tid >> 3, r_e8 = tid & 7;
+  constexpr int CHP = G::CHP, NRF = G::NRF, TPR = G::TPR;
+  const int r_row = tid / TPR, r_e8 = tid & (TPR - 1);
 
   auto load_unit = [&](const bf16_t* wf_hi, const bf16_t* wf_lo, int nf, int j) {
     const size_t e = ((size_t)(nf * G::KS + kq * G::U + j) * 64 + lane) * 8;
@@ -84,24 +91,24 @@
     for (int j = 0; j < G::DEPTH; ++j) bq[j] = load_unit(wf_hi, wf_lo, nf, j);
     __builtin_amdgcn_sched_barrier(0);
   };
-  f32x16 acc[2];
+  f32x16 acc[NRF];
   auto job_loop = [&](const bf16_t* wf_hi, const bf16_t* wf_lo, int nf, auto swap_tag) __attribute__((always_inline)) {
     constexpr bool SWAP = decltype(swap_tag)::value;
 #pragma unroll
-    for (int rf = 0; rf < 2; ++rf)
+    for (int rf = 0; rf < NRF; ++rf)
 #pragma unroll
       for (int r = 0; r < 16; ++r) acc[rf][r] = 0.f;
-    auto read_a = [&](int u, bf16x8 (&h)[2], bf16x8 (&l)[2]) {
+    auto read_a = [&](int u, bf16x8 (&h)[NRF], bf16x8 (&l)[NRF]) {
       const int c16 = (kq * G::U + u) * 2 + lh;
 #pragma unroll
-      for (int rf = 0; rf < 2; ++rf) {
+      for (int rf = 0; rf < NRF; ++rf) {
         const int row = rf * 32 + l31;
         const int off = (c16 >> 3) * CHP + row * 128 + (((c16 & 7) ^ swz(row)) << 4);
         h[rf] = *reinterpret_cast<const bf16x8*>(a_reg + off);
         l[rf] = *reinterpret_cast<const bf16x8*>(a_reg + G::A_PL + off);
       }
     };
-    bf16x8 ah[2][2], al[2][2];
+    bf16x8 ah[2][NRF], al[2][NRF];
     read_a(0, ah[0], al[0]);
 #pragma unroll
     for (int u = 0; u < G::U; ++u) {
@@ -109,19 +116,19 @@
       if (u + 1 < G::U) read_a(u + 1, ah[cur ^ 1], al[cur ^ 1]);
       const BFrag f = bq[u % G::DEPTH];
       if (SWAP) {
-        acc[0] = __builtin_amdgcn_mfma_f32_32x32x16_bf16(al[cur][0], f.h, acc[0], 0, 0, 0);
-        acc[1] = __builtin_amdgcn_mfma_f32_32x32x16_bf16(al[cur][1], f.h, acc[1], 0, 0, 0);
-        acc[0] = __builtin_amdgcn_mfma_f32_32x32x16_bf16(ah[cur][0], f.l, acc[0], 0, 0, 0);
-        acc[1] = __builtin_amdgcn_mfma_f32_32x32x16_bf16(ah[cur][1], f.l, acc[1], 0, 0, 0);
-        acc[0] = __builtin_amdgcn_mfma_f32_32x32x16_bf16(ah[cur][0], f.h, acc[0], 0, 0, 0);
-        acc[1] = __builtin_amdgcn_mfma_f32_32x32x16_bf16(ah[cur][1], f.h, acc[1], 0, 0, 0);
+#pragma unroll
+        for (int rf = 0; rf < NRF; ++rf) acc[rf] = __builtin_amdgcn_mfma_f32_32x32x16_bf16(al[cur][rf], f.h, acc[rf], 0, 0, 0);
+#pragma unroll
+        for (int rf = 0; rf < NRF; ++rf) acc[rf] = __builtin_amdgcn_mfma_f32_32x32x16_bf16(ah[cur][rf], f.l, acc[rf], 0, 0, 0);
+#pragma unroll
+        for (int rf = 0; rf < NRF; ++rf) acc[rf] = __builtin_amdgcn_mfma_f32_32x32x16_bf16(ah[cur][rf], f.h, acc[rf], 0, 0, 0);
       } else {
-        acc[0] = __builtin_amdgcn_mfma_f32_32x32x16_bf16(f.h, al[cur][0], acc[0], 0, 0, 0);
-        acc[1] = __builtin_amdgcn_mfma_f32_32x32x16_bf16(f.h, al[cur][1], acc[1], 0, 0, 0);
-        acc[0] = __builtin_amdgcn_mfma_f32_32x32x16_bf16(f.l, ah[cur][0], acc[0], 0, 0, 0);
-        acc[1] = __builtin_amdgcn_mfma_f32_32x32x16_bf16(f.l, ah[cur][1], acc[1], 0, 0, 0);
-        acc[0] = __builtin_amdgcn_mfma_f32_32x32x16_bf16(f.h, ah[cur][0], acc[0], 0, 0, 0);
-        acc[1] = __builtin_amdgcn_mfma_f32_32x32x16_bf16(f.h, ah[cur][1], acc[1], 0, 0, 0);
+#pragma unroll
+        for (int rf = 0; rf < NRF; ++rf) acc[rf] = __builtin_amdgcn_mfma_f32_32x32x16_bf16(f.h, al[cur][rf], acc[rf], 0, 0, 0);
+#pragma unroll
+        for (int rf = 0; rf < NRF; ++rf) acc[rf] = __builtin_amdgcn_mfma_f32_32x32x16_bf16(f.l, ah[cur][rf], acc[rf], 0, 0, 0);
+#pragma unroll
+        for (int rf = 0; rf < NRF; ++rf) acc[rf] = __builtin_amdgcn_mfma_f32_32x32x16_bf16(f.h, ah[cur][rf], acc[rf], 0, 0, 0);
       }
       __builtin_amdgcn_sched_barrier(0);
       if (u + G::DEPTH < G::U) bq[u % G::DEPTH] = load_unit(wf_hi, wf_lo, nf, u + G::DEPTH);
@@ -129,28 +136,32 @@
     }
   };
   float4* const red4 = reinterpret_cast<float4*>(red_reg);
-  auto pieces = [&](const f32x16& a0, const f32x16& a1, float4 (&v)[2]) __attribute__((always_inline)) {
+  auto pieces = [&](const f32x16 (&a)[NRF], float4 (&v)[NRF]) __attribute__((always_inline)) {
+    const f32x16& a0 = a[0];
+    const f32x16& a1 = a[NRF - 1];
     if constexpr (G::ONE) {
       __syncthreads();
 #pragma unroll
       for (int g = 0; g < 4; ++g) {
-        red4[((((cf * 4 + kq) * 2 + 0) * 4 + g) << 6) + lane] = make_float4(a0[4 * g], a0[4 * g + 1], a0[4 * g + 2], a0[4 * g + 3]);
-        red4[((((cf * 4 + kq) * 2 + 1) * 4 + g) << 6) + lane] = make_float4(a1[4 * g], a1[4 * g + 1], a1[4 * g + 2], a1[4 * g + 3]);
+        red4[((((cf * 4 + kq) * NRF + 0) * 4 + g) << 6) + lane] = make_float4(a0[4 * g], a0[4 * g + 1], a0[4 * g + 2], a0[4 * g + 3]);
+        if constexpr (NRF == 2)
+          red4[((((cf * 4 + kq) * NRF + 1) * 4 + g) << 6) + lane] = make_float4(a1[4 * g], a1[4 * g + 1], a1[4 * g + 2], a1[4 * g + 3]);
       }
       __syncthreads();
 #pragma unroll
-      for (int rf = 0; rf < 2; ++rf) {
-        float4 t = red4[((((cf * 4 + 0) * 2 + rf) * 4 + fg) << 6) + lane];
+      for (int rf = 0; rf < NRF; ++rf) {
+        float4 t = red4[((((cf * 4 + 0) * NRF + rf) * 4 + fg) << 6) + lane];
 #pragma unroll
         for (int k = 1; k < 4; ++k) {
-          const float4 w = red4[((((cf * 4 + k) * 2 + rf) * 4 + fg) << 6) + lane];
+          const float4 w = red4[((((cf * 4 + k) * NRF + rf) * 4 + fg) << 6) + lane];
           t.x += w.x; t.y += w.y; t.z += w.z; t.w += w.w;
         }
         v[rf] = t;
       }
     } else {
-#pragma unroll
-      for (int rf = 0; rf < 2; ++rf) {
+      static_assert(G::ONE || NRF == 2, "one row fragment per round: the 64-row geometry");
+#pragma unroll
+      for (int rf = 0; rf < NRF; ++rf) {
         __syncthreads();
 #pragma unroll
         for (int g = 0; g < 4; ++g)
@@ -168,7 +179,7 @@
     }
   };
   auto put_planes = [&](int j, float v0, float v1, float v2, float v3) __attribute__((always_inline)) {
-    const int ch = 4 * (r_e8 + 8 * j);
+    const int ch = 4 * (r_e8 + TPR * j);
     uint2 hw, lw;
     hw.x = pk(v0, v1); hw.y = pk(v2, v3);
     lw.x = pk(v0 - __uint_as_float(hw.x << 16), v1 - __uint_as_float(hw.x & 0xffff0000u));
@@ -180,19 +191,21 @@
 
   float4 rv[G::JT];
   const float4 b1v = *reinterpret_cast<const float4*>(p.b1 + s * BN + cf * 32 + 8 * fg + 4 * lh);
-  float4 rres[2];
-  float4 h2v[2];
+  float4 rres[NRF];
+  float4 h2v[NRF];
   if constexpr (MODE >= 1) {
     const int ncol_ = s * BN + cf * 32 + 8 * fg + 4 * lh;
 #pragma unroll
-    for (int rf = 0; rf < 2; ++rf)
+    for (int rf = 0; rf < NRF; ++rf)
       rres[rf] = p.res ? *reinterpret_cast<const float4*>(p.res + (size_t)(m0 + rf * 32 + l31) * C + ncol_) : make_float4(0.f, 0.f, 0.f, 0.f);
     const unsigned a_base = (unsigned)(size_t)a_reg;
-    const int d_row = wave * 8 + (lane >> 3), d_slot = lane & 7;
-#pragma unroll
-    for (int c = 0; c < G::A_CH; ++c) {
+    const int d_rg = G::NRG == NWV ? wave : wave % G::NRG, d_c0 = G::NRG == NWV ? 0 : wave / G::NRG;
+    const int d_row = d_rg * 8 + (lane >> 3), d_slot = lane & 7;
+#pragma unroll
+    for (int i = 0; i < G::DMA_CH; ++i) {
+      const int c = d_c0 + i * (NWV / G::NRG);
       const size_t e = (size_t)(m0 + d_row) * C + c * 64 + ((d_slot ^ swz(d_row)) << 3);
-      const unsigned dst = a_base + (unsigned)(c * CHP + wave * 1024);
+      const unsigned dst = a_base + (unsigned)(c * CHP + d_rg * 1024);
       glds16(p.a_hi + e, dst);
       glds16(p.a_lo + e, dst + G::A_PL);
     }
@@ -204,7 +217,7 @@
   {
     const float* xr = p.x + (size_t)(m0 + r_row) * C + 4 * r_e8;
 #pragma unroll
-    for (int j = 0; j < G::JT; ++j) rv[j] = *reinterpret_cast<const float4*>(xr + 32 * j);
+    for (int j = 0; j < G::JT; ++j) rv[j] = *reinterpret_cast<const float4*>(xr + 4 * TPR * j);
   }
   job_prologue(p.w1_hi, p.w1_lo, s * 2 + cf);
   DV_QTRACE(10);
@@ -252,7 +265,7 @@
   }
 #pragma unroll
   for (int j = 0; j < G::JT; ++j) {
-    const int ch = 4 * (r_e8 + 8 * j);
+    const int ch = 4 * (r_e8 + TPR * j);
     const float4 sc = *reinterpret_cast<const float4*>(s_gscale + ch);
     const float4 sh = *reinterpret_cast<const float4*>(s_gshift + ch);
     put_planes(j, fmaf(rv[j].x, sc.x, sh.x), fmaf(rv[j].y, sc.y, sh.y), fmaf(rv[j].z, sc.z, sh.z), fmaf(rv[j].w, sc.w, sh.w));
@@ -267,16 +280,16 @@
   const int ncol = s * BN + cf * 32 + 8 * fg + 4 * lh;
   {
     const float4 b4 = b1v;
-    float4 pv[2];
-    pieces(acc[0], acc[1], pv);
-#pragma unroll
-    for (int rf = 0; rf < 2; ++rf) {
+    float4 pv[NRF];
+    pieces(acc, pv);
+#pragma unroll
+    for (int rf = 0; rf < NRF; ++rf) {
       float4 v = pv[rf];
       v.x += b4.x; v.y += b4.y; v.z += b4.z; v.w += b4.w;
       if constexpr (MODE >= 1) {
-        const float4 r4 = rf == 0 ? rres[0] : rres[1];
+        const float4 r4 = rres[rf];
         v.x += r4.x; v.y += r4.y; v.z += r4.z; v.w += r4.w;
-        if (rf == 0) h2v[0] = v; else h2v[1] = v;
+        h2v[rf] = v;
       }
       float4* const dst = reinterpret_cast<float4*>(p.out1 + (size_t)(m0 + rf * 32 + l31) * C + ncol);
       if (xl) *dst = v; else st_handover16(dst, v);
@@ -346,7 +359,15 @@
   {
     const float4* hr = reinterpret_cast<const float4*>(p.out1 + (size_t)(m0 + r_row) * C + 4 * r_e8);
     if (xl) {
-      if constexpr (G::JT == 4)
+      if constexpr (TPR == 16) {
+        static_assert(TPR == 8 || G::JT == 8, "sixteen threads per row: C = 512");
+        asm volatile("global_load_dwordx4 %0, %8, off sc1\n\tglobal_load_dwordx4 %1, %8, off offset:256 sc1\n\t"
+                     "global_load_dwordx4 %2, %8, off offset:512 sc1\n\tglobal_load_dwordx4 %3, %8, off offset:768 sc1\n\t"
+                     "global_load_dwordx4 %4, %8, off offset:1024 sc1\n\tglobal_load_dwordx4 %5, %8, off offset:1280 sc1\n\t"
+                     "global_load_dwordx4 %6, %8, off offset:1536 sc1\n\tglobal_load_dwordx4 %7, %8, off offset:1792 sc1\n\t"
+                     "s_waitcnt vmcnt(0)"
+                     : "=&v"(rv[0]), "=&v"(rv[1]), "=&v"(rv[2]), "=&v"(rv[3]), "=&v"(rv[4 % G::JT]), "=&v"(rv[5 % G::JT]), "=&v"(rv[6 % G::JT]), "=&v"(rv[7 % G::JT]) : "v"(hr) : "memory");
+      } else if constexpr (G::JT == 4)
         asm volatile("global_load_dwordx4 %0, %4, off sc1\n\tglobal_load_dwordx4 %1, %4, off offset:128 sc1\n\t"
                      "global_load_dwordx4 %2, %4, off offset:256 sc1\n\tglobal_load_dwordx4 %3, %4, off offset:384 sc1\n\t"
                      "s_waitcnt vmcnt(0)"
@@ -371,12 +392,13 @@
                      : "v"(hr) : "memory");
     } else {
 #pragma unroll
-      for (int j = 0; j < G::JT; ++j) rv[j] = ld_handover16(hr + 8 * j);
+      for (int j = 0; j < G::JT; ++j) rv[j] = ld_handover16(hr + TPR * j);
     }
     float s1 = 0.f;
 #pragma unroll
     for (int j = 0; j < G::JT; ++j) s1 += (rv[j].x + rv[j].y) + (rv[j].z + rv[j].w);
     s1 += __shfl_xor(s1, 1); s1 += __shfl_xor(s1, 2); s1 += __shfl_xor(s1, 4);
+    if constexpr (TPR == 16) s1 += __shfl_xor(s1, 8);
     const float mean = s1 * (1.0f / (float)C);
     float m2 = 0.f;
 #pragma unroll
@@ -385,6 +407,7 @@
       m2 = fmaf(d0, d0, m2); m2 = fmaf(d1, d1, m2); m2 = fmaf(d2, d2, m2); m2 = fmaf(d3, d3, m2);
     }
     m2 += __shfl_xor(m2, 1); m2 += __shfl_xor(m2, 2); m2 += __shfl_xor(m2, 4);
+    if constexpr (TPR == 16) m2 += __shfl_xor(m2, 8);
     if (r_e8 == 0) s_ln[r_row] = make_float2(mean, 1.0f / sqrtf(m2 * (1.0f / (float)C) + p.ln_eps));
 #pragma unroll
     for (int j = 0; j < G::JT; ++j) put_planes(j, rv[j].x, rv[j].y, rv[j].z, rv[j].w);
@@ -392,9 +415,9 @@
   __syncthreads();
   DV_QTRACE(6);
 
-  auto finish_q = [&](const float4 (&pv)[2]) __attribute__((always_inline)) {
-#pragma unroll
-    for (int rf = 0; rf < 2; ++rf) {
+  auto finish_q = [&](const float4 (&pv)[NRF]) __attribute__((always_inline)) {
+#pragma unroll
+    for (int rf = 0; rf < NRF; ++rf) {
       const float4 v = pv[rf];
       const float2 st = s_ln[rf * 32 + l31];
       float4 o;
@@ -405,19 +428,19 @@
   };
   if constexpr (MODE == 1) {
     job_loop(p.w2_hi, p.w2_lo, nfq, std::false_type{});
-    float4 pv[2];
-    pieces(acc[0], acc[1], pv);
+    float4 pv[NRF];
+    pieces(acc, pv);
     finish_q(pv);
     DV_QTRACE(7); DV_QTRACE(8); DV_QTRACE(9);
     return;
   } else if constexpr (MODE == 2) {
     constexpr int d = C / 8, KSq = d / 16, HS = BN / d, KP = (2 * HS < NWV) ? 2 : 1;
-    static_assert(C <= 256 && 2 * HS * KP == NWV, "MODE 2 geometry");
+    static_assert(C <= 256 && 2 * HS * KP == NWV && G::RB == BM, "MODE 2 geometry");
     job_loop(p.w2_hi, p.w2_lo, nfq, std::false_type{});
     job_prologue(p.w3_hi, p.w3_lo, s * 2 + cf);
     {
-      float4 pv[2];
-      pieces(acc[0], acc[1], pv);
+      float4 pv[NRF];
+      pieces(acc, pv);
 #pragma unroll
       for (int rf = 0; rf < 2; ++rf) {
         const float4 v = pv[rf];
@@ -583,12 +606,12 @@
     DV_QTRACE(9);
     job_loop(p.w3_hi, p.w3_lo, s * 2 + cf, std::false_type{});
     {
-      float4 pv[2];
-      pieces(acc[0], acc[1], pv);
+      float4 pv[NRF];
+      pieces(acc, pv);
       __shared__ float2 s_rp[2 * 32 * 2 * 4];
 #pragma unroll
       for (int rf = 0; rf < 2; ++rf) {
-        const float4 r4 = rf == 0 ? h2v[0] : h2v[1];
+        const float4 r4 = h2v[rf];
         float4 v = pv[rf];
         v.x += b3v.x + r4.x; v.y += b3v.y + r4.y; v.z += b3v.z + r4.z; v.w += b3v.w + r4.w;
         const size_t ob = (size_t)(m0 + rf * 32 + l31) * C + ncol;
@@ -624,23 +647,23 @@
     DV_QTRACE(13);
     return;
   } else {
-    f32x16 aq[2], ak[2], av[2];
-#pragma unroll
-    for (int rf = 0; rf < 2; ++rf)
+    f32x16 aq[NRF], ak[NRF], av[NRF];
+#pragma unroll
+    for (int rf = 0; rf < NRF; ++rf)
 #pragma unroll
       for (int r = 0; r < 16; ++r) { aq[rf][r] = 0.f; ak[rf][r] = 0.f; av[rf][r] = 0.f; }
     {
-      auto read_a = [&](int u, bf16x8 (&h)[2], bf16x8 (&l)[2]) {
+      auto read_a = [&](int u, bf16x8 (&h)[NRF], bf16x8 (&l)[NRF]) {
         const int c16 = (kq * G::U + u) * 2 + lh;
 #pragma unroll
-        for (int rf = 0; rf < 2; ++rf) {
+        for (int rf = 0; rf < NRF; ++rf) {
           const int row = rf * 32 + l31;
           const int off = (c16 >> 3) * CHP + row * 128 + (((c16 & 7) ^ swz(row)) << 4);
           h[rf] = *reinterpret_cast<const bf16x8*>(a_reg + off);
           l[rf] = *reinterpret_cast<const bf16x8*>(a_reg + G::A_PL + off);
         }
       };
-      bf16x8 ah[2][2], al[2][2];
+      bf16x8 ah[2][NRF], al[2][NRF];
       read_a(0, ah[0], al[0]);
 #pragma unroll
       for (int j = 0; j < 3 * G::U; ++j) {
@@ -649,25 +672,25 @@
         const BFrag f = b3[j % G::D3];
         if (ps == 2) {
 #pragma unroll
-          for (int rf = 0; rf < 2; ++rf) av[rf] = __builtin_amdgcn_mfma_f32_32x32x16_bf16(al[cur][rf], f.h, av[rf], 0, 0, 0);
-#pragma unroll
-          for (int rf = 0; rf < 2; ++rf) av[rf] = __builtin_amdgcn_mfma_f32_32x32x16_bf16(ah[cur][rf], f.l, av[rf], 0, 0, 0);
-#pragma unroll
-          for (int rf = 0; rf < 2; ++rf) av[rf] = __builtin_amdgcn_mfma_f32_32x32x16_bf16(ah[cur][rf], f.h, av[rf], 0, 0, 0);
+          for (int rf = 0; rf < NRF; ++rf) av[rf] = __builtin_amdgcn_mfma_f32_32x32x16_bf16(al[cur][rf], f.h, av[rf], 0, 0, 0);
+#pragma unroll
+          for (int rf = 0; rf < NRF; ++rf) av[rf] = __builtin_amdgcn_mfma_f32_32x32x16_bf16(ah[cur][rf], f.l, av[rf], 0, 0, 0);
+#pragma unroll
+          for (int rf = 0; rf < NRF; ++rf) av[rf] = __builtin_amdgcn_mfma_f32_32x32x16_bf16(ah[cur][rf], f.h, av[rf], 0, 0, 0);
         } else if (ps == 1) {
 #pragma unroll
-          for (int rf = 0; rf < 2; ++rf) ak[rf] = __builtin_amdgcn_mfma_f32_32x32x16_bf16(f.h, al[cur][rf], ak[rf], 0, 0, 0);
-#pragma unroll
-          for (int rf = 0; rf < 2; ++rf) ak[rf] = __builtin_amdgcn_mfma_f32_32x32x16_bf16(f.l, ah[cur][rf], ak[rf], 0, 0, 0);
-#pragma unroll
-          for (int rf = 0; rf < 2; ++rf) ak[rf] = __builtin_amdgcn_mfma_f32_32x32x16_bf16(f.h, ah[cur][rf], ak[rf], 0, 0, 0);
+          for (int rf = 0; rf < NRF; ++rf) ak[rf] = __builtin_amdgcn_mfma_f32_32x32x16_bf16(f.h, al[cur][rf], ak[rf], 0, 0, 0);
+#pragma unroll
+          for (int rf = 0; rf < NRF; ++rf) ak[rf] = __builtin_amdgcn_mfma_f32_32x32x16_bf16(f.l, ah[cur][rf], ak[rf], 0, 0, 0);
+#pragma unroll
+          for (int rf = 0; rf < NRF; ++rf) ak[rf] = __builtin_amdgcn_mfma_f32_32x32x16_bf16(f.h, ah[cur][rf], ak[rf], 0, 0, 0);
         } else {
 #pragma unroll
-          for (int rf = 0; rf < 2; ++rf) aq[rf] = __builtin_amdgcn_mfma_f32_32x32x16_bf16(f.h, al[cur][rf], aq[rf], 0, 0, 0);
-#pragma unroll
-          for (int rf = 0; rf < 2; ++rf) aq[rf] = __builtin_amdgcn_mfma_f32_32x32x16_bf16(f.l, ah[cur][rf], aq[rf], 0, 0, 0);
-#pragma unroll
-          for (int rf = 0; rf < 2; ++rf) aq[rf] = __builtin_amdgcn_mfma_f32_32x32x16_bf16(f.h, ah[cur][rf], aq[rf], 0, 0, 0);
+          for (int rf = 0; rf < NRF; ++rf) aq[rf] = __builtin_amdgcn_mfma_f32_32x32x16_bf16(f.h, al[cur][rf], aq[rf], 0, 0, 0);
+#pragma unroll
+          for (int rf = 0; rf < NRF; ++rf) aq[rf] = __builtin_amdgcn_mfma_f32_32x32x16_bf16(f.l, ah[cur][rf], aq[rf], 0, 0, 0);
+#pragma unroll
+          for (int rf = 0; rf < NRF; ++rf) aq[rf] = __builtin_amdgcn_mfma_f32_32x32x16_bf16(f.h, ah[cur][rf], aq[rf], 0, 0, 0);
         }
         __builtin_amdgcn_sched_barrier(0);
         if (j + G::D3 < 3 * G::U) b3[j % G::D3] = load_unit3(j + G::D3);
@@ -675,12 +698,12 @@
       }
     }
     DV_QTRACE(7);
-    float4 pv[2];
-    pieces(aq[0], aq[1], pv);
+    float4 pv[NRF];
+    pieces(aq, pv);
     finish_q(pv);
-    pieces(ak[0], ak[1], pv);
-#pragma unroll
-    for (int rf = 0; rf < 2; ++rf) {
+    pieces(ak, pv);
+#pragma unroll
+    for (int rf = 0; rf < NRF; ++rf) {
       const float4 v = pv[rf];
       const float2 st = s_ln[rf * 32 + l31];
       const float o0 = st.y * (v.x - st.x * uk.x) + bk4.x, o1 = st.y * (v.y - st.x * uk.y) + bk4.y;
@@ -694,9 +717,9 @@
       dv_st8(p.sa_kf_lo + eo, lw);
     }
     DV_QTRACE(8);
-    pieces(av[0], av[1], pv);
-#pragma unroll
-    for (int rf = 0; rf < 2; ++rf) {
+    pieces(av, pv);
+#pragma unroll
+    for (int rf = 0; rf < NRF; ++rf) {
       const float4 v = pv[rf];
       const float4 s01 = *reinterpret_cast<const float4*>(&s_ln[rf * 32 + 8 * fg + 4 * lh]);
       const float4 s23 = *reinterpret_cast<const float4*>(&s_ln[rf * 32 + 8 * fg + 4 * lh + 2]);
@@ -719,6 +742,11 @@
   }
 }
 
+bool xcd_local_blocks(int row_blocks) {
+  static const bool xcd_on = [] { const char* e = getenv("DVITS_QKV_XCD"); return !(e && e[0] == '0'); }();
+  return xcd_on && row_blocks % 8 == 0;
+}
+
 template <int C>
 hipError_t qkv_init_one() {
   hipError_t e = hipFuncSetAttribute(reinterpret_cast<const void*>(k_qkv_split<C, 0>), hipFuncAttributeMaxDynamicSharedMemorySize, QGeom<C>::SMEM);
@@ -731,9 +759,10 @@
 template <int C>
 hipError_t qkv_launch_one(const ChainParams& pin, hipStream_t st) {
   ChainParams p = pin;
-  p.qs_xcd = qkv_split_xcd_local(p.M) ? 1 : 0;
-  if (p.amode == 1) hipLaunchKernelGGL((k_qkv_split<C, 0>), dim3((p.M / BM) * QGeom<C>::NSPL), dim3(NT), QGeom<C>::SMEM, st, p);
-  else if (!p.xa_kf_hi) hipLaunchKernelGGL((k_qkv_split<C, 1>), dim3((p.M / BM) * QGeom<C>::NSPL), dim3(NT), QGeom<C>::SMEM, st, p);
+  constexpr int RB = QGeom<C>::RB;
+  p.qs_xcd = xcd_local_blocks(p.M / RB) ? 1 : 0;
+  if (p.amode == 1) hipLaunchKernelGGL((k_qkv_split<C, 0>), dim3((p.M / RB) * QGeom<C>::NSPL), dim3(NT), QGeom<C>::SMEM, st, p);
+  else if (!p.xa_kf_hi) hipLaunchKernelGGL((k_qkv_split<C, 1>), dim3((p.M / RB) * QGeom<C>::NSPL), dim3(NT), QGeom<C>::SMEM, st, p);
   else {
     if constexpr (C <= 256) {
       if (!p.qs_xcd) return hipErrorInvalidValue;
@@ -745,19 +774,17 @@
 
 }
 
-bool qkv_split_xcd_local(int M) {
-  static const bool xcd_on = [] { const char* e = getenv("DVITS_QKV_XCD"); return !(e && e[0] == '0'); }();
-  return xcd_on && (M / BM) % 8 == 0;
-}
+bool qkv_split_xcd_local(int M) { return xcd_local_blocks(M / BM); }
 hipError_t qkv_split_init() {
   hipError_t e = qkv_init_one<128>();
   if (e == hipSuccess) e = qkv_init_one<256>();
-  return e != hipSuccess ? e : qkv_init_one<384>();
+  if (e == hipSuccess) e = qkv_init_one<384>();
+  return e != hipSuccess ? e : qkv_init_one<512>();
 }
 bool qkv_split_supported(const ChainParams& p, int precision) {
   if (precision != 0 || !p.out1 || (p.ldo2 & 3) != 0) return false;
-  if (p.C != 128 && p.C != 256 && p.C != 384) return false;
-  if (p.T % BM != 0 || p.M % p.T != 0 || p.Tv < 0 || p.Tv > p.T || (p.Tv > 0 && p.Tv <= p.T - 32)) return false;
+  if (p.C != 128 && p.C != 256 && p.C != 384 && p.C != 512) return false;
+  if (p.T % qrows(p.C) != 0 || p.M % p.T != 0 || p.Tv < 0 || p.Tv > p.T || (p.Tv > 0 && p.Tv <= p.T - 32)) return false;
   if (p.amode == 1) {
     if (p.passes != 3 || !p.sa_kf_hi || !p.sa_kf_lo || !p.sa_vf_hi || !p.sa_vf_lo || p.res || p.xa_kf_hi || !p.out2 || p.ldo2 < p.C) return false;
     const int G = p.groups;
@@ -765,12 +792,12 @@
     if ((p.T / 32) * (p.C / 16) > 2 * 4 * 4 * 64 * 16 / 8) return false;
     return true;
   }
-  if (p.amode != 0 || p.passes != 1 || !p.a_hi || !p.a_lo || p.sa_kf_hi) return false;
+  if (p.amode != 0 || p.passes != 1 || !p.a_hi || !p.a_lo || !p.res || p.sa_kf_hi) return false;
   if (!p.xa_kf_hi) return p.out2 && p.ldo2 >= p.C;
   return p.C <= 256 && p.xa_kf_lo && p.xa_vf_hi && p.xa_vf_lo && p.xa_bias && p.xa_nT > 0 && p.xa_d == p.C / 8 && p.w3_hi && p.w3_lo && p.b3 &&
          p.out3 && p.out3_hi && p.out3_lo && p.rowstat3 && p.qs_o_hi && p.qs_o_lo && qkv_split_xcd_local(p.M);
 }
-int qkv_split_flags(const ChainParams& p) { return (p.M / BM) * (p.C / BN) * (p.xa_kf_hi ? 2 : 1); }
+int qkv_split_flags(const ChainParams& p) { return (p.M / qrows(p.C)) * (p.C / BN) * (p.xa_kf_hi ? 2 : 1); }
 hipError_t launch_qkv_split(const ChainParams& p, int precision, hipStream_t st) {
   if (!qkv_split_supported(p, precision)) return hipErrorInvalidValue;
   if ((p.amode == 1 && (!p.x || !p.stat16 || !p.gamma || !p.beta)) || !p.w1_hi || !p.w1_lo || !p.b1 || !p.w2_hi || !p.w2_lo || !p.b2 || !p.u2 ||
@@ -778,9 +805,10 @@
     return hipErrorInvalidValue;
   if (!gemm_handover_rounds()) {
     static const int n_cu = [] { int d = 0, n = 0; (void)hipGetDevice(&d); (void)hipDeviceGetAttribute(&n, hipDeviceAttributeMultiprocessorCount, d); return n; }();
-    if ((p.M / BM) * (p.C / BN) > n_cu) return hipErrorInvalidValue;
+    if ((p.M / qrows(p.C)) * (p.C / BN) > n_cu) return hipErrorInvalidValue;
   }
   if (p.C == 128) return qkv_launch_one<128>(p, st);
   if (p.C == 256) return qkv_launch_one<256>(p, st);
-  return qkv_launch_one<384>(p, st);
-}
+  if (p.C == 384) return qkv_launch_one<384>(p, st);
+  return qkv_launch_one<512>(p, st);
+}
```

After: 68250 mel-frames/s (median of 6 runs). 1.01x the previous value.
